# pavel-paulau/query

Measured on AMD Instinct MI355X. Metric: rows/sec filter+group-by on 100M synthetic JSON docs; achieved HBM GB/s, higher is better.
Workload: dtype int64/f64 tagged scalars (u8 tag + 8 B payload), u32 dictionary codes; 1 GPU; config2: SELECT cat, SUM(price) FROM default WHERE price > 50 GROUP BY cat @ 100000000 rows, K_cat=1000, columns resident in HBM; rows_per_gpu=100000000, groups=1000, rows_selected=49401294, agg_mode=2, spec_kernel=1

## Files before the change

### query_amd/build.py

```python
from __future__ import annotations

import os
import shutil
import subprocess
import sys

HERE = os.path.dirname(os.path.abspath(__file__))
CSRC = os.path.join(HERE, "csrc")
LIB = os.path.join(HERE, "libn1k.so")
SOURCES = ["n1k_kernels.hip", "n1k_bins.hip", "n1k_jsondev.hip", "n1k_matchtable.hip", "n1k_order.hip", "n1k_rowdistinct.hip", "n1k_order.cpp", "n1k_rowdistinct.cpp", "n1k_matchtable.cpp", "n1k_like.cpp", "n1k_coll.cpp", "n1k_in.cpp", "n1k_strfn.cpp", "n1k_jsonpush.cpp", "n1k_plan.cpp", "n1k_engine.cpp", "n1k_scan.cpp", "n1k_select.cpp", "n1k_partitioned.cpp", "n1k_distinct.cpp",
           "n1k_finish.cpp", "n1k_tail.cpp", "n1k_exchange.cpp", "n1k_jit.cpp", "n1k_json.cpp"]
HEADERS = ["n1k_types.h", "n1k_device.h", "n1k_tables.h", "n1k_scatter.h", "n1k_spec.h", "n1k_like.h", "n1k_coll.h", "n1k_in.h", "n1k_strfn.h", "n1k_order.h", "n1k_rowdistinct.h", "n1k_jit.h", "n1k_kernels.h", "n1k_plan.h", os.path.join("..", "..", "include", "n1k.h")]
HOST_HEADERS = ["n1k_engine.h", "n1k_buf.h", "n1k_wire.h"]
ARCH = "gfx950"


def _hipcc() -> str:
    for c in (os.environ.get("HIPCC"), shutil.which("hipcc"), "/opt/rocm/bin/hipcc"):
        if c and os.path.exists(c):
            return c
    raise RuntimeError("hipcc not found")


OBJDIR = os.path.join(CSRC, "build")
FLAGS = ["--offload-arch=" + ARCH, "-O3", "-std=c++17", "-fPIC", "-munsafe-fp-atomics", "-Wall", "-Wno-unused-function"]


def _stale(target: str, deps) -> bool:
    if not os.path.exists(target):
        return True
    mt = os.path.getmtime(target)
    return any(os.path.getmtime(d) > mt for d in deps)


def source_hash() -> str:
    import hashlib
    h = hashlib.sha1()
    for f in sorted([x for x in SOURCES if x.endswith(".hip")] + [x for x in HEADERS if not x.startswith("..")]):
        with open(os.path.join(CSRC, f), "rb") as fh:
            h.update(f.encode() + b"\0" + fh.read())
    return h.hexdigest()[:16]


def needs_build() -> bool:
    return _stale(LIB, [os.path.join(CSRC, f) for f in SOURCES + HEADERS + HOST_HEADERS] + [os.path.abspath(__file__)])


def build(force: bool = False, verbose: bool = False) -> str:
    if not force and not needs_build():
        return LIB
    from concurrent.futures import ThreadPoolExecutor
    os.makedirs(OBJDIR, exist_ok=True)
    hipcc = _hipcc()
    headers = [os.path.join(CSRC, f) for f in HEADERS + HOST_HEADERS] + [os.path.abspath(__file__)]

    def compile_one(src: str) -> str:
        obj = os.path.join(OBJDIR, src + ".o")
        path = os.path.join(CSRC, src)
        deps = headers if not src.endswith(".hip") else [os.path.join(CSRC, f) for f in HEADERS]
        if force or _stale(obj, [path] + deps):
            cmd = [hipcc] + FLAGS + ["-c", path, "-o", obj]
            if verbose:
                print(" ".join(cmd), file=sys.stderr)
            subprocess.check_call(cmd)
        return obj

    with ThreadPoolExecutor(max_workers=min(len(SOURCES), os.cpu_count() or 1)) as ex:
        objs = list(ex.map(compile_one, SOURCES))
    cmd = [hipcc, "--offload-arch=" + ARCH, "-shared", "-fPIC", "-o", LIB] + objs + ["-lhiprtc", "-lrccl", "-ldl", "-pthread"]
    if verbose:
        print(" ".join(cmd), file=sys.stderr)
    subprocess.check_call(cmd)
    return LIB


if __name__ == "__main__":
    print(build(force="--force" in sys.argv, verbose=True))
```

### query_amd/csrc/n1k_engine.cpp

```cpp
#include "n1k_engine.h"

using namespace n1k;
using namespace n1k_eng;

namespace n1k_eng {

thread_local std::string g_create_error;

n1k_status fail(n1k_handle* h, n1k_status st, const char* fmt, ...) {
    char buf[512];
    va_list ap;
    va_start(ap, fmt);
    vsnprintf(buf, sizeof buf, fmt, ap);
    va_end(ap);
    h->last_error = buf;
    return st;
}

uint32_t intern(n1k_handle* h, const std::string& s) {
    auto it = h->dict_index.find(s);
    if (it != h->dict_index.end()) return it->second;
    uint32_t code = (uint32_t)h->dict.size();
    h->dict.push_back(s);
    h->dict_index.emplace(s, code);
// ... 373 lines not shown
        tbits = (63 - n_dict * dbits) / n_tag;
    }
    uint32_t shift = 0;
    for (uint32_t k = 0; k < P.nkeys; k++) {
        KeySpec& ks = P.keys[k];
        ks.bits = ks.mode == KEYM_DICT ? dbits : tbits;
        ks.shift = shift;
        shift += ks.bits;
        if (ks.bits < (ks.mode == KEYM_DICT ? 4u : 8u)) return fail(h, N1K_UNSUPPORTED, "group key layout does not fit 63 bits");
    }
    P.wide_int = P.wide_flt = nullptr;
    P.wide_bits = 0;
    P.wide_count = h->groups.counters.p + CTR_WIDE_VALUES;
    if (n_tag && h->opt.wide_values) {
        uint32_t wb = 4;
        while ((1ull << wb) < h->opt.wide_values * 2 && wb < 30) wb++;
        wb = std::min(wb, tbits - 4);
        const size_t n = (size_t)1 << wb;
        HIP_TRY(h, h->groups.wide_int.ensure(n));
        HIP_TRY(h, h->groups.wide_flt.ensure(n));
        HIP_TRY(h, hipMemsetAsync(h->groups.wide_int.p, 0xFF, n * 8, h->stream));
        HIP_TRY(h, hipMemsetAsync(h->groups.wide_flt.p, 0xFF, n * 8, h->stream));
        P.wide_int = h->groups.wide_int.p;
        P.wide_flt = h->groups.wide_flt.p;
        P.wide_bits = wb;
    }
    {
        uint32_t total = 0;
        for (uint32_t k = 0; k < P.nkeys; k++) total += P.keys[k].bits;
        h->distinct.nw_key_bits = P.nkeys == 0 ? 1u : (total <= 34 ? total : 24u);
        h->distinct.nw_val_bits = 61 - h->distinct.nw_key_bits;
        for (uint32_t a = 0; a < P.naggs; a++)
            if (P.aggs[a].distinct)
                h->distinct.words[P.aggs[a].log_index] = h->opt.distinct_words && P.aggs[a].kind == AGG_COUNT;
    }
    h->layout_fixed = true;
    return N1K_OK;
}

n1k_status alloc_table(n1k_handle* h, uint64_t capacity, GlobalTable& t, DevBuf<uint64_t>& keys, DevBuf<uint64_t>& acc,
                       DevBuf<uint64_t>& rep) {
    HIP_TRY(h, keys.ensure(capacity));
    HIP_TRY(h, acc.ensure(capacity * h->prog.glob_words));
    if (h->prog.want_rep_row) HIP_TRY(h, rep.ensure(capacity));
    t.keys = keys.p;
    t.acc = acc.p;
    t.rep_row = h->prog.want_rep_row ? rep.p : nullptr;
    t.capacity = capacity;
    HIP_TRY(h, launch_init_table(h->prog, t, 0, capacity, nullptr, h->stream));
    return N1K_OK;
}

static n1k_status grow_table(n1k_handle* h, uint64_t cap) {
    if (cap <= h->groups.table.capacity) return N1K_OK;
    if (!h->groups.table.capacity) return alloc_table(h, cap, h->groups.table, h->groups.keys, h->groups.acc, h->groups.rep);
    GlobalTable nt{};
    DevBuf<uint64_t> nk, na, nr;
    ST_TRY(alloc_table(h, cap, nt, nk, na, nr));
    HIP_TRY(h, launch_rehash(h->prog, h->groups.table, nt, h->groups.errp, h->groups.counters.p + CTR_REHASH_SCRATCH, h->stream));
    HIP_TRY(h, hipStreamSynchronize(h->stream));
    h->groups.keys = std::move(nk);
    h->groups.acc = std::move(na);
    h->groups.rep = std::move(nr);
    h->groups.table = nt;
    return N1K_OK;
}

n1k_status ensure_table(n1k_handle* h, uint64_t incoming_rows) {
    uint64_t want_groups = std::min<uint64_t>(h->opt.max_groups, h->row_base + h->groups.merged_bound + incoming_rows);
    if (h->prog.nkeys == 0) want_groups = 1;
    else {
        bool all_dict = true;
        long double dom = 1;
        for (uint32_t k = 0; k < h->prog.nkeys; k++) {
            all_dict &= h->prog.keys[k].mode == KEYM_DICT;
            dom *= (long double)h->dict.size() + 2;
        }
        if (all_dict && dom < (long double)want_groups) want_groups = (uint64_t)dom;
    }
    return grow_table(h, next_pow2(std::max<uint64_t>(want_groups * 2, 1024)));
}

n1k_status ensure_table_groups(n1k_handle* h, uint64_t groups) {
    if (groups > h->opt.max_groups)
        return fail(h, N1K_OOM, "group table capacity exceeded: raise the max_groups option (now %llu)", (unsigned long long)h->opt.max_groups);
    return grow_table(h, next_pow2(std::max<uint64_t>(groups * 2, 1024)));
}

n1k_status ensure_pinned_counters(n1k_handle* h) {
    HIP_TRY(h, h->res.pin_counters.ensure(kCounters + kPinScratch));
    return N1K_OK;
}

hipEvent_t get_event(n1k_handle* h) {
    if (!h->timing.event_pool.empty()) {
        hipEvent_t e = h->timing.event_pool.back();
        h->timing.event_pool.pop_back();
        return e;
    }
    hipEvent_t e = nullptr;
    (void)hipEventCreate(&e);
    return e;
}

void drain_events(n1k_handle* h) {
    for (auto& pr : h->timing.events) {
        float ms = 0.f;
        if (pr.first && pr.second && hipEventElapsedTime(&ms, pr.first, pr.second) == hipSuccess) h->timing.stats.device_ms += ms;
        if (pr.first) h->timing.event_pool.push_back(pr.first);
        if (pr.second) h->timing.event_pool.push_back(pr.second);
    }
    h->timing.events.clear();
}

n1k_status validate_batch(n1k_handle* h, const n1k_batch* b) {
    if (!b) return fail(h, N1K_INVALID, "null batch");
    if (b->ncols != (uint32_t)h->plan.paths.size()) return fail(h, N1K_INVALID, "batch has %u columns, plan needs %u", b->ncols, (uint32_t)h->plan.paths.size());
    for (uint32_t c = 0; c < b->ncols; c++) {
        const n1k_col& col = b->cols[c];
        if (col.kind == N1K_COL_DICT32) {
            if (b->nrows && !col.codes) return fail(h, N1K_INVALID, "column %u: null codes", c);
        } else if (col.kind == N1K_COL_TAGGED64) {
            if (b->nrows && (!col.tags || !col.payload)) return fail(h, N1K_INVALID, "column %u: null tags/payload", c);
        } else
            return fail(h, N1K_INVALID, "column %u: unknown kind %u", c, col.kind);
        if (h->layout_fixed && col.kind != h->col_kinds[c])
            return fail(h, N1K_INVALID, "column %u changed kind between batches", c);
    }
    return N1K_OK;
}

uint64_t batch_bytes_per_row(const n1k_handle* h) {
    uint64_t b = 0;
    for (uint32_t c = 0; c < (uint32_t)h->plan.paths.size(); c++) b += h->col_kinds[c] == N1K_COL_DICT32 ? 4 : 9;
    return b;
}

void default_value(const AggDef& d, n1k_value& v, n1k_partial& p) {
    memset(&v, 0, sizeof v);
    memset(&p, 0, sizeof p);
    p.extreme.tag = N1K_T_NULL;
    if (d.kind == AGG_COUNT || d.kind == AGG_COUNTN) {
        v.tag = N1K_T_INT;
        v.v.i = 0;
    } else
        v.tag = N1K_T_NULL;
}

n1k_status reset_handle(n1k_handle* h, bool clear_stop) {
    if (clear_stop) h->stop_flag.store(0);
    h->failure_global = false;
    h->row_base = 0;
    h->groups.merged_bound = 0;
    h->filter.selected.clear();
    h->filter.has_sel32 = false;
    h->res.keys.clear();
    h->res.aggs.clear();
    h->res.parts.clear();
    h->res.rep.clear();
    memset(&h->timing.stats, 0, sizeof h->timing.stats);
    if (h->device_ready) {
        HIP_TRY(h, hipSetDevice(h->device));
        if (!h->timing.events.empty()) {
            HIP_TRY(h, hipStreamSynchronize(h->stream));
            drain_events(h);
        }
        h->timing.stats.device_ms = 0;
        h->part.groups_seen = 0;
        h->res.out_count_dirty = false;
        h->part.pending.count = 0;
        if (!h->timing.ev_q0) {
            (void)hipEventCreate(&h->timing.ev_q0);
            (void)hipEventCreate(&h->timing.ev_q1);
        }
        h->timing.q1_recorded = false;
        h->timing.q0_recorded = h->timing.ev_q0 && hipEventRecord(h->timing.ev_q0, h->stream) == hipSuccess;
        if (h->device_clean) return N1K_OK;
        h->device_clean = true;
        if (h->groups.table.capacity) HIP_TRY(h, launch_init_table(h->prog, h->groups.table, 0, h->groups.table.capacity, h->groups.counters.p, h->stream));
        else HIP_TRY(h, hipMemsetAsync(h->groups.counters.p, 0, kCounters * sizeof(unsigned long long), h->stream));
        if (h->distinct.word_hist.p) HIP_TRY(h, hipMemsetAsync(h->distinct.word_hist.p, 0, kMaxDistinct * 256 * sizeof(unsigned long long), h->stream));
        if (h->distinct.wcursor.p) HIP_TRY(h, hipMemsetAsync(h->distinct.wcursor.p, 0, kMaxDistinct * kWordSubs * kCursorStride * sizeof(unsigned long long), h->stream));
        h->distinct.wregion_used = false;
        if (h->prog.wide_int) {
            const size_t n = (size_t)1 << h->prog.wide_bits;
            HIP_TRY(h, hipMemsetAsync(h->groups.wide_int.p, 0xFF, n * 8, h->stream));
            HIP_TRY(h, hipMemsetAsync(h->groups.wide_flt.p, 0xFF, n * 8, h->stream));
        }
    }
    return N1K_OK;
}

}



extern "C" {

int n1k_abi_version(void) { return N1K_ABI_VERSION; }

int n1k_device_count(void) {
    int n = 0;
    if (hipGetDeviceCount(&n) != hipSuccess) return 0;
    return n;
}

const char* n1k_create_error(void) { return g_create_error.c_str(); }

uint64_t n1k_device_bytes_live(void) { return g_device_bytes_live.load(std::memory_order_relaxed); }

n1k_status n1k_create(const char* plan_json, size_t len, n1k_handle** out) {
    return guarded(nullptr, [&]() -> n1k_status {
    if (out) *out = nullptr;
    if (!plan_json || !out) {
        g_create_error = "null argument";
        return N1K_INVALID;
    }
    auto* h = new n1k_handle();
    PlanError err;
    if (!parse_plan_json(plan_json, len, h->plan, err) || !compile_plan(h, err)) {
        g_create_error = err.msg;
        n1k_status st = err.unsupported ? N1K_UNSUPPORTED : N1K_INVALID;
        delete h;
        return st;
    }
    if (h->plan.has_having) {
        std::string cond = h->plan.having_text;
        std::vector<std::pair<std::string, std::string>> subst;
        for (size_t a = 0; a < h->plan.aggs.size(); a++) subst.emplace_back(h->plan.aggs[a].text, "(`$g`.`a" + std::to_string(a) + "`)");
        for (size_t k = 0; k < h->plan.key_texts.size(); k++) subst.emplace_back(h->plan.key_texts[k], "(`$g`.`k" + std::to_string(k) + "`)");
        std::stable_sort(subst.begin(), subst.end(), [](const auto& x, const auto& y) { return x.first.size() > y.first.size(); });
        for (auto& sb : subst) {
            if (sb.first.empty()) continue;
            for (size_t pos = 0; (pos = cond.find(sb.first, pos)) != std::string::npos; pos += sb.second.size())
                cond.replace(pos, sb.first.size(), sb.second);
        }
        std::string js = "{\"#operator\":\"Filter\",\"condition\":\"";
        for (char c : cond) {
            if (c == '"' || c == '\\') js.push_back('\\');
            if ((unsigned char)c < 0x20) {
                char b[8];
                snprintf(b, sizeof b, "\\u%04x", (unsigned)c);
                js += b;
            } else
                js.push_back(c);
        }
        js += "\"}";
        n1k_status hst = n1k_create(js.c_str(), js.size(), &h->tail.having);
        if (hst != N1K_OK) {
            g_create_error = "HAVING: " + g_create_error;
            delete h;
            return hst;
        }
        for (const std::string& p : h->tail.having->plan.paths) {
            int idx = -1;
            char kind = 0;
            if (sscanf(p.c_str(), "(`$g`.`%c%d`)", &kind, &idx) != 2 || (kind != 'k' && kind != 'a') || idx < 0 ||
                (size_t)idx >= (kind == 'k' ? h->plan.key_texts.size() : h->plan.aggs.size())) {
                g_create_error = "HAVING refers to " + p + ", which is neither a group key nor an aggregate of the plan";
                n1k_destroy(h->tail.having);
                delete h;
                return N1K_UNSUPPORTED;
            }
            h->tail.having_cols.push_back(kind == 'k' ? idx : -idx - 1);
        }
    }
    if (h->plan.has_project) {
        n1k_status pst = build_projection(h);
        if (pst != N1K_OK) {
            if (h->tail.having) n1k_destroy(h->tail.having);
            h->tail.having = nullptr;
            delete h;
            return pst;
        }
    }
    g_create_error.clear();
    *out = h;
    return N1K_OK;
    });
}

static void destroy_handle(n1k_handle* h);
void n1k_destroy(n1k_handle* h) {
    if (!h) return;
    try {
        destroy_handle(h);
    } catch (...) {
    }
}
static void destroy_handle(n1k_handle* h) {
    if (h->timing.host_us[5] > 0)
        fprintf(stderr, "n1k host trace: %.0f one-call executions; per call: reset %.1f us, push %.1f us, finish %.1f us (of which waiting %.1f us, after the wait %.1f us)\n",
                h->timing.host_us[5], h->timing.host_us[0] / h->timing.host_us[5], h->timing.host_us[1] / h->timing.host_us[5], h->timing.host_us[2] / h->timing.host_us[5],
                h->timing.host_us[3] / h->timing.host_us[5], h->timing.host_us[4] / h->timing.host_us[5]);
    if (h->tail.having) n1k_destroy(h->tail.having);
    h->tail.having = nullptr;
    if (h->tail.project) n1k_destroy(h->tail.project);
    h->tail.project = nullptr;
    if (h->device_ready) {
        (void)hipSetDevice(h->device);
        if (h->stream) (void)hipStreamSynchronize(h->stream);
        if (h->stage.copy_stream) (void)hipStreamSynchronize(h->stage.copy_stream);
        drain_events(h);
        for (auto e : h->timing.event_pool) (void)hipEventDestroy(e);
        if (h->timing.ev_q0) (void)hipEventDestroy(h->timing.ev_q0);
        if (h->timing.ev_q1) (void)hipEventDestroy(h->timing.ev_q1);
// ... 36 lines not shown
}
const char* n1k_projection_alias(const n1k_handle* h, uint32_t i) {
    if (h && i < h->plan.row_distinct.size()) return h->plan.row_distinct[i].as.c_str();
    return (h && i < h->plan.project.size()) ? h->plan.project[i].as.c_str() : nullptr;
}

n1k_status n1k_dict_intern(n1k_handle* h, uint32_t n, const uint64_t* offsets, const char* bytes, uint32_t* out_codes) {
    return guarded(h, [&]() -> n1k_status {
    if (!h || (n && (!offsets || !bytes || !out_codes))) return N1K_INVALID;
    for (uint32_t i = 0; i < n; i++) {
        if (offsets[i + 1] < offsets[i]) return fail(h, N1K_INVALID, "dictionary offsets are not monotone");
        out_codes[i] = intern(h, std::string(bytes + offsets[i], (size_t)(offsets[i + 1] - offsets[i])));
    }
    if (h->dict.size() >= 0xFFFFFFF0ull) return fail(h, N1K_OOM, "dictionary too large");
    return N1K_OK;
    });
}

uint32_t n1k_dict_size(const n1k_handle* h) { return h ? (uint32_t)h->dict.size() : 0; }

n1k_status n1k_dict_get(const n1k_handle* h, uint32_t code, const char** ptr, size_t* len) {
    return guarded(h, [&]() -> n1k_status {
    if (!h || !ptr || !len || code >= h->dict.size()) return N1K_INVALID;
    *ptr = h->dict[code].data();
    *len = h->dict[code].size();
    return N1K_OK;
    });
}

n1k_status n1k_set_option(n1k_handle* h, const char* name, int64_t value) {
    return guarded(h, [&]() -> n1k_status {
    if (!h || !name) return N1K_INVALID;
    std::string n = name;
    if (n == "agg_mode") h->opt.agg_mode = value;
    else if (n == "max_groups") h->opt.max_groups = value > 0 ? (uint64_t)value : 1;
    else if (n == "grid_blocks") h->opt.grid_blocks = (uint32_t)std::max<int64_t>(0, value);
    else if (n == "fast") h->opt.fast = value ? 1 : 0;
    else if (n == "spec") h->opt.spec = value ? 1 : 0;
    else if (n == "wide") h->opt.wide = value ? 1 : 0;
    else if (n == "fuse_arith") h->opt.fuse_arith = value ? 1 : 0;
    else if (n == "lean_topk") h->opt.lean_topk = value ? 1 : 0;
    else if (n == "topk_sample") h->opt.topk_sample = value ? 1 : 0;
    else if (n == "distinct_fill_pct") h->opt.distinct_fill_pct = (uint32_t)std::min<int64_t>(std::max<int64_t>(value, 1), 75);
    else if (n == "dedupe_unroll") h->opt.dedupe_unroll = (uint32_t)value;
    else if (n == "agg_spec") h->opt.agg_spec = value ? 1 : 0;
    else if (n == "merge_chunks") h->opt.merge_chunks = (uint32_t)std::min<int64_t>(std::max<int64_t>(value, 0), 16);
    else if (n == "inject_failure") h->opt.inject_failure = (uint32_t)std::min<int64_t>(std::max<int64_t>(value, 0), 3);
    else if (n == "part_block") h->opt.part_block = value == 256 ? 256 : 512;
    else if (n == "part_subs") h->opt.part_subs = (uint32_t)std::min<int64_t>(std::max<int64_t>(value, 0), 2);
    else if (n == "part_per_cu") h->opt.part_per_cu = (uint32_t)std::min<int64_t>(std::max<int64_t>(value, 0), 8);
    else if (n == "jit") h->opt.jit = (uint32_t)std::min<int64_t>(std::max<int64_t>(value, 0), 2);
    else if (n == "jit_min_rows") h->opt.jit_min_rows = (uint64_t)std::max<int64_t>(value, 0);
    else if (n == "distinct_words") {
        if (h->layout_fixed) return fail(h, N1K_INVALID, "distinct_words must be set before the first batch");
        h->opt.distinct_words = value ? 1 : 0;
    } else if (n == "distinct_set_slots") {
        uint32_t v = 64;
        while (v < (uint32_t)std::min<int64_t>(std::max<int64_t>(value, 64), 8192)) v <<= 1;
        h->opt.distinct_set_slots = v;
    } else if (n == "records") {
        h->opt.records = value ? 1 : 0;
    } else if (n == "rec_slots") {
        h->opt.rec_slots = (uint32_t)std::min<int64_t>(std::max<int64_t>(value, 0), 8192);
    } else if (n == "rec_bins") {
        uint32_t v = 0;
        if (value > 0) for (v = 1; v < (uint32_t)std::min<int64_t>(value, 256); v <<= 1) {}
        h->opt.rec_bins = v;
    } else if (n == "rec_slices") {
        h->opt.rec_slices = (uint32_t)std::min<int64_t>(std::max<int64_t>(value, 0), 64);
    } else if (n == "rec_scan_per_cu") {
        h->opt.rec_scan_per_cu = (uint32_t)std::min<int64_t>(std::max<int64_t>(value, 0), 8);
    } else if (n == "rec_block") {
        h->opt.rec_block = value <= 0 ? 0u : (value <= 256 ? 256u : 512u);
    } else if (n == "rec_unroll") {
        h->opt.rec_unroll = (uint32_t)std::min<int64_t>(std::max<int64_t>(value, 0), 8);
    } else if (n == "distinct_region_cap") {
        h->opt.region_cap = (uint64_t)std::max<int64_t>(value, 0);
    } else if (n == "dedupe_block") {
        if ((value | 1) != 257 && (value | 1) != 513 && (value | 1) != 1025) return fail(h, N1K_INVALID, "dedupe_block must be 256, 512 or 1024 (+1: probe word by word)");
        h->opt.dedupe_block = (uint32_t)value;
    } else if (n == "json_device") {
        h->opt.json_device = value ? 1 : 0;
    } else if (n == "json_device_left_pct") {
        h->opt.json_device_left_pct = (uint32_t)std::min<int64_t>(std::max<int64_t>(value, 0), 100);
    } else if (n == "json_device_min_docs") {
        h->opt.json_device_min_docs = (uint64_t)std::max<int64_t>(value, 0);
    } else if (n == "json_threads") {
        h->opt.json_threads = (uint32_t)std::min<int64_t>(std::max<int64_t>(value, 0), 64);
    } else if (n == "partition_min_rows") {
        h->opt.partition_min_rows = (uint64_t)std::max<int64_t>(value, 1);
    } else if (n == "partition_probe_rows") {
        h->opt.partition_probe_rows = (uint64_t)std::max<int64_t>(value, 1);
    } else if (n == "partition_min_groups") {
        h->opt.partition_min_groups = (uint64_t)std::max<int64_t>(value, 1);
    } else if (n == "partition_sticky") {
        h->opt.partition_sticky = value ? 1 : 0;
        h->part.sticky.valid = false;
    } else if (n == "partition_levels") {
        h->opt.partition_levels = (int32_t)std::min<int64_t>(std::max<int64_t>(value, -1), 2);
    } else if (n == "topk_min_groups") {
        h->opt.topk_min_groups = (uint64_t)std::max<int64_t>(value, 1);
    } else if (n == "distinct_levels") {
        h->opt.distinct_levels = (int32_t)std::min<int64_t>(std::max<int64_t>(value, -1), 2);
    } else if (n == "wide_values") {
        if (h->layout_fixed) return fail(h, N1K_INVALID, "wide_values must be set before the first batch");
        h->opt.wide_values = (uint64_t)std::max<int64_t>(value, 0);
    }
    else if (n == "slabs") h->opt.slabs = (uint32_t)std::min<int64_t>(std::max<int64_t>(value, 0), 2);
    else if (n == "block") {
        if (value != 0 && value != 256 && value != 512 && value != 1024) return fail(h, N1K_INVALID, "block must be 0 (auto), 256, 512 or 1024");
        h->opt.block = (uint32_t)value;
    } else if (n == "rows_per_lane") {
        if (value != 2 && value != 4) return fail(h, N1K_INVALID, "rows_per_lane must be 2 or 4");
        h->opt.rows_per_lane = (uint32_t)value;
    }
    else if (n == "lds_bytes") h->opt.lds_bytes = (uint32_t)std::min<int64_t>(std::max<int64_t>(value, 1024), 64 * 1024);
    else if (n == "device") {
        if (h->device_ready) return fail(h, N1K_INVALID, "device must be chosen before the first push");
        h->device = (int)value;
    } else if (n == "stream") {
        if (h->device_ready) return fail(h, N1K_INVALID, "stream must be chosen before the first push");
        h->stream = (hipStream_t)(uintptr_t)value;
        h->own_stream = false;
    } else if (n == "rep_row") {
        if (h->layout_fixed) return fail(h, N1K_INVALID, "rep_row must be chosen before the first push");
        h->opt.rep_row = value ? 1 : 0;
        PlanError err;
        h->agg_names.clear();
        h->has_distinct = false;
        h->n_distinct = 0;
        if (!compile_plan(h, err)) return fail(h, N1K_INVALID, "%s", err.msg.c_str());
    } else if (!rowdistinct_option(h, n, value))
        return fail(h, N1K_INVALID, "unknown option %s", name);
    return N1K_OK;
    });
}

n1k_status n1k_push_device_batch(n1k_handle* h, const n1k_batch* batch) {
    return guarded(h, [&]() -> n1k_status {
    if (!h) return N1K_INVALID;
    ST_TRY(refuse_ordered_rows(h, "n1k_push_device_batch"));
    return push_device(h, batch);
    });
}

n1k_status n1k_run_device_batch(n1k_handle* h, const n1k_batch* batch, n1k_result* out) {
    if (!h || !batch || !out) return N1K_INVALID;
    if (h->plan.ordered_rows() || h->plan.has_row_distinct) return guarded(h, [&]() -> n1k_status { return refuse_ordered_rows(h, "n1k_run_device_batch"); });
    static const bool trace = getenv("N1K_HOST_TRACE") != nullptr;
    auto now = [] { return std::chrono::duration<double, std::micro>(std::chrono::steady_clock::now().time_since_epoch()).count(); };
    const double t0 = trace ? now() : 0;
    n1k_status st = n1k_reset(h);
    const double t1 = trace ? now() : 0;
    if (st == N1K_OK) st = n1k_push_device_batch(h, batch);
    const double t2 = trace ? now() : 0;
    if (st == N1K_OK) {
        h->clear_on_finish = true;
        st = n1k_finish(h, out);
        h->clear_on_finish = false;
    }
    if (trace) {
        h->timing.host_us[0] += t1 - t0;
        h->timing.host_us[1] += t2 - t1;
        h->timing.host_us[2] += now() - t2;
        h->timing.host_us[5] += 1;
    }
    return st;
}

n1k_status n1k_extract_json(n1k_handle* h, uint64_t ndocs, const uint64_t* offsets, const char* bytes, n1k_batch* out) {
    return guarded(h, [&]() -> n1k_status {
    if (!h || !out || (ndocs && (!offsets || !bytes))) return N1K_INVALID;
    if (h->json.paths_state == 0) {
        h->json.paths.resize(h->plan.paths.size());
        h->json.paths_state = 1;
        for (size_t c = 0; c < h->plan.paths.size(); c++)
            if (!parse_leaf_path(h->plan.paths[c], h->json.paths[c])) h->json.paths_state = -1;
    }
    if (h->json.paths_state < 0)
        return fail(h, N1K_UNSUPPORTED, "a leaf path of the plan is not a chain of field names: extract the columns yourself");
    const size_t np = h->json.paths.size();
    uint32_t nthreads = h->opt.json_threads ? h->opt.json_threads : std::min(16u, std::max(1u, std::thread::hardware_concurrency()));
    nthreads = (uint32_t)std::max<uint64_t>(1, std::min<uint64_t>(nthreads, ndocs / 2048 + 1));
    std::vector<JsonColumns> part(nthreads);
    std::vector<std::string> errs(nthreads);
    std::vector<long long> bad(nthreads, -1);
    std::vector<std::thread> workers;
    auto range = [&](uint32_t t) { return std::make_pair(ndocs * t / nthreads, ndocs * (t + 1) / nthreads); };
    std::vector<char> threw(nthreads, 0);
    auto work = [&](uint32_t t) {
        try {
            auto r = range(t);
            bad[t] = extract_json_range(h->json.paths, offsets, bytes, r.first, r.second, part[t], errs[t]);
        } catch (...) {
            threw[t] = 1;
        }
    };
    workers.reserve(nthreads);
    std::vector<uint32_t> inline_ranges{0};
    for (uint32_t t = 1; t < nthreads; t++) {
        try {
            workers.emplace_back(work, t);
        } catch (...) {
            inline_ranges.push_back(t);
        }
    }
    for (uint32_t t : inline_ranges) work(t);
    for (auto& w : workers) w.join();
    for (uint32_t t = 0; t < nthreads; t++)
        if (threw[t]) return fail(h, N1K_OOM, "out of host memory while scanning the documents");
    for (uint32_t t = 0; t < nthreads; t++)
        if (bad[t] >= 0) {
            if (errs[t].find("nested deeper than 256") != std::string::npos)
                return fail(h, N1K_UNSUPPORTED_DATA, "document %lld: %s", bad[t], errs[t].c_str());
            return fail(h, N1K_INVALID, "document %lld is not valid JSON: %s", bad[t], errs[t].c_str());
        }
    h->json.tags.assign(np, std::vector<uint8_t>());
    h->json.payload.assign(np, std::vector<uint64_t>());
    for (size_t c = 0; c < np; c++) {
        h->json.tags[c].resize(ndocs);
        h->json.payload[c].resize(ndocs);
    }
    for (uint32_t t = 0; t < nthreads; t++) {
        auto r = range(t);
        std::vector<uint64_t> code(part[t].strings.size());
        for (size_t i = 0; i < code.size(); i++) code[i] = intern(h, part[t].strings[i]);
        for (size_t c = 0; c < np; c++) {
            const size_t n = (size_t)(r.second - r.first);
            memcpy(h->json.tags[c].data() + r.first, part[t].tags[c].data(), n);
            uint64_t* dst = h->json.payload[c].data() + r.first;
            const uint64_t* src = part[t].payload[c].data();
            const uint8_t* tg = part[t].tags[c].data();
            for (size_t i = 0; i < n; i++) dst[i] = tg[i] >= N1K_T_STRING ? code[src[i]] : src[i];
        }
    }
    h->json.cols.assign(np, n1k_col{});
    for (size_t c = 0; c < np; c++) {
        h->json.cols[c].kind = N1K_COL_TAGGED64;
        h->json.cols[c].tags = h->json.tags[c].data();
        h->json.cols[c].payload = h->json.payload[c].data();
    }
    out->nrows = ndocs;
    out->ncols = (uint32_t)np;
    out->cols = h->json.cols.data();
    return N1K_OK;
    });
}

n1k_status n1k_push_json(n1k_handle* h, uint64_t ndocs, const uint64_t* offsets, const char* bytes) {
    return guarded(h, [&]() -> n1k_status {
    if (!h || (ndocs && (!offsets || !bytes))) return N1K_INVALID;
    ST_TRY(refuse_ordered_rows(h, "n1k_push_json"));
    if (h->stop_flag.load()) return fail(h, N1K_STOPPED, "operator was stopped");
    if (h->json.paths_state == 0) {
        h->json.paths.resize(h->plan.paths.size());
        h->json.paths_state = 1;
        for (size_t c = 0; c < h->plan.paths.size(); c++)
            if (!parse_leaf_path(h->plan.paths[c], h->json.paths[c])) h->json.paths_state = -1;
    }
    if (h->json.paths_state > 0 && ndocs) {
        bool done = false;
        n1k_status dst = push_json_device(h, ndocs, offsets, bytes, &done);
        if (dst != N1K_OK || done) return dst;
    }
    n1k_batch b{};
    n1k_status st = n1k_extract_json(h, ndocs, offsets, bytes, &b);
    if (st != N1K_OK) return st;
    return n1k_push_batch(h, &b);
    });
}

n1k_status n1k_push_batch(n1k_handle* h, const n1k_batch* batch) {
    return guarded(h, [&]() -> n1k_status {
    if (!h) return N1K_INVALID;
    ST_TRY(refuse_ordered_rows(h, "n1k_push_batch"));
    if (h->stop_flag.load()) return fail(h, N1K_STOPPED, "operator was stopped");
    n1k_status st = ensure_device(h);
    if (st != N1K_OK) return st;
    st = validate_batch(h, batch);
    if (st != N1K_OK) return st;
    std::vector<n1k_col> dcols;
    st = stage_host_batch(h, batch, dcols);
    if (st != N1K_OK) return st;
    n1k_batch db = *batch;
    db.cols = dcols.data();
    st = push_device(h, &db);
    n1k_status st2 = staged_batch_issued(h);
    return st != N1K_OK ? st : st2;
    });
}

n1k_status n1k_sync(n1k_handle* h) {
    return guarded(h, [&]() -> n1k_status {
    if (!h) return N1K_INVALID;
    if (!h->device_ready) return N1K_OK;
    HIP_TRY(h, hipSetDevice(h->device));
    unsigned long long counters[kCounters] = {0};
    HIP_TRY(h, hipMemcpyAsync(counters, h->groups.counters.p, sizeof counters, hipMemcpyDeviceToHost, h->stream));
    HIP_TRY(h, hipStreamSynchronize(h->stream));
    drain_events(h);
    if (h->plan.has_group && !h->device_clean) {
        h->timing.stats.rows_selected = counters[CTR_ROWS_SELECTED];
        h->timing.stats.groups_out = h->part.pending.count ? h->part.pending.count : counters[CTR_GROUPS];
    }
    if (!h->device_clean) h->timing.stats.wide_key_values = counters[CTR_WIDE_VALUES];
    return N1K_OK;
    });
}

n1k_status n1k_jit_check(n1k_handle* h, const uint32_t* col_kinds, uint32_t ncols, char* log, size_t loglen) {
    return guarded(h, [&]() -> n1k_status {
    if (!h || !col_kinds) return N1K_INVALID;
    if (log && loglen) log[0] = 0;
// ... 192 lines not shown
```

### query_amd/csrc/n1k_engine.h

```cpp
#pragma once
#include <hip/hip_runtime.h>

#include <algorithm>
#include <atomic>
#include <chrono>
#include <cmath>
#include <cstdarg>
#include <cstdio>
#include <cstring>
#include <functional>
#include <numeric>
#include <string>
#include <condition_variable>
#include <mutex>
#include <thread>
#include <unordered_map>
#include <vector>

#include "../../include/n1k.h"
#include "n1k_buf.h"
#include "n1k_jit.h"
#include "n1k_json.h"
#include "n1k_kernels.h"
#include "n1k_coll.h"
#include "n1k_in.h"
#include "n1k_like.h"
#include "n1k_order.h"
#include "n1k_plan.h"
#include "n1k_rowdistinct.h"
#include "n1k_strfn.h"


using namespace n1k;

static_assert(sizeof(n1k_value) == 16, "n1k_value layout");
static_assert(sizeof(OutValue) == sizeof(n1k_value), "OutValue must alias n1k_value");
static_assert(sizeof(Program) + sizeof(ScanArgs) + sizeof(GlobalTable) + 64 <= 4096, "kernel arguments exceed 4 KiB");

namespace n1k_eng {

extern thread_local std::string g_create_error;

struct MatchScratch {
    DevBuf<uint8_t> bytes;
    DevBuf<uint64_t> off;
    DevBuf<uint8_t> left;
    DevBuf<uint8_t> bits;
    DevBuf<uint8_t> progs;
    DevBuf<uint8_t> sprogs;
};

enum MatchKind { MK_LIKE, MK_COLL, MK_IN, MK_STRFN, MK_COUNT };

struct MatchTable {
    std::vector<LikePattern> patterns;
    std::vector<CollPred> preds;
    std::vector<InList> lists;
    uint32_t string_lists = 0;
    std::vector<StrFnPred> strfns;
    uint32_t strfn_first = 0;
    uint32_t coll_top = kMatchBits - 1;
    std::vector<double> in_numbers;
    InTableHost in_table;
    DevBuf<uint8_t> d_in_table;
    DevBuf<double> d_in_nums;
    bool in_uploaded = false;
    DevBuf<uint8_t> d_bits;
    size_t built_for = 0;
    MatchScratch scratch;
    struct { uint64_t dev = 0, host = 0; } counts[MK_COUNT];

    int add_like(const std::string& pattern, PlanError& err);
    int add_coll(const Expr* e, PlanError& err);
    int add_in(const Expr* e, PlanError& err);
    int add_strfn(const Expr* e, const Expr*& path, PlanError& err);
    void finalize_bits(Program& P);
    void clear_plan() {
        patterns.clear();
        preds.clear();
        lists.clear();
        strfns.clear();
        in_numbers.clear();
        string_lists = strfn_first = 0;
    }
};

inline uint32_t match_lds_bytes(const FastArgs& F) {
    for (uint32_t t = 0; t < F.nterms; t++)
        if (term_is_table_bit(F.terms[t].op)) return kMatchLdsBytes;
    return 0;
}

inline uint64_t next_pow2(uint64_t x) {
    uint64_t p = 1;
    while (p < x) p <<= 1;
    return p;
}
inline uint32_t ceil_log2(uint64_t x) {
    uint32_t b = 0;
    while ((1ull << b) < x) b++;
    return b;
}

n1k_status fail(n1k_handle* h, n1k_status st, const char* fmt, ...);

#define HIP_TRY(h, expr)                                                                                  \
    do {                                                                                                  \
        hipError_t _e = (expr);                                                                           \
        if (_e != hipSuccess)                                                                             \
            return fail(h, _e == hipErrorOutOfMemory ? N1K_OOM : N1K_DEVICE_ERROR, "%s failed: %s", #expr, \
                        hipGetErrorString(_e));                                                           \
    } while (0)

#define ST_TRY(expr) do { n1k_status _st = (expr); if (_st != N1K_OK) return _st; } while (0)

constexpr uint32_t kPinScratch = 16;
constexpr uint64_t kWordSubs = 256ull * kRecSubs;


struct Options {
    int64_t agg_mode = N1K_MODE_AUTO;
    uint64_t max_groups = 1ull << 26;
    uint32_t grid_blocks = 0;
    uint32_t fast = 1, spec = 1, wide = 1;
    uint32_t fuse_arith = 1;
    uint32_t lean_topk = 1;
    uint32_t topk_sample = 1;
    uint32_t distinct_fill_pct = 25;
    uint32_t dedupe_unroll = 0;
    uint32_t agg_spec = 1;
    uint32_t merge_chunks = 0;
    uint32_t inject_failure = 0;
    uint32_t part_block = 256;
    uint32_t part_subs = 1;
    uint32_t part_per_cu = 0;
    uint32_t jit = 1;
    uint64_t jit_min_rows = 4u << 20;
    uint32_t distinct_words = 1;
    uint32_t distinct_set_slots = 8192;
    uint32_t records = 1;
    uint32_t rec_slots = 0, rec_bins = 0, rec_slices = 0, rec_scan_per_cu = 0, rec_block = 0, rec_unroll = 0;
    uint64_t region_cap = 0;
    uint32_t dedupe_block = 1025;
    uint32_t json_device = 1;
    uint32_t json_device_left_pct = 12;
    uint64_t json_device_min_docs = 4096;
    uint32_t json_threads = 0;
    uint64_t partition_min_rows = 8u << 20, partition_probe_rows = 512u << 10, partition_min_groups = 4096;
    uint32_t partition_sticky = 1;
    int32_t partition_levels = -1;
    uint64_t topk_min_groups = 65536;
    int32_t distinct_levels = -1;
    uint64_t wide_values = 1u << 20;
    uint32_t slabs = 1;
    uint32_t block = 0, rows_per_lane = 4;
    uint32_t lds_bytes = 64 * 1024;
    uint32_t rep_row = 0;
    uint64_t rowdistinct_slots = 0;
    uint32_t rowdistinct_lds_slots = 0;
};

enum Counter : uint32_t {
    CTR_ROWS_SELECTED = 0,
    CTR_GROUPS = 1,
    CTR_OUT_COUNT = 2,
    CTR_FILTER_TOTAL = 3,
    CTR_REHASH_SCRATCH = 4,
    CTR_DISTINCT_REGION_WORDS = 5,
    CTR_PAIR_LOG_CURSORS = 8,
    CTR_ERR_FLAGS = 12,
    CTR_WIDE_VALUES = 13,
    CTR_WORD_LOG_CURSORS = 16,
    CTR_OPTIMISTIC_OVERFLOW = 20,
    CTR_PART_RECORDS = 21,
    CTR_SINGLETONS = 22,
    CTR_EXACT_OVERFLOW = 24,
    CTR_SAVED_ROWS_SELECTED = 25,
    CTR_REGION_GROUPS = 26,
    CTR_PEER_STATUS = 27,
    CTR_ROWDISTINCT_COUNT = 28,
    CTR_ROWDISTINCT_REACHED = 29
};
static_assert(CTR_ERR_FLAGS + kPeerStatusFromErr == CTR_PEER_STATUS, "the verdict kernel writes the peer status this far behind the flags");
static_assert(CTR_ROWDISTINCT_REACHED < kCounters && CTR_ROWDISTINCT_REACHED == CTR_ROWDISTINCT_COUNT + 1, "every counter word lies inside the buffer (CTR_ROWDISTINCT_REACHED is the last)");
static_assert(CTR_PAIR_LOG_CURSORS + kMaxDistinct <= CTR_ERR_FLAGS && CTR_WORD_LOG_CURSORS + kMaxDistinct <= CTR_OPTIMISTIC_OVERFLOW, "cursor words overlap their neighbours");

struct GroupTable {
    GlobalTable table{};
    DevBuf<uint64_t> keys, acc, rep;
    DevBuf<uint64_t> slabs;
    DevBuf<unsigned long long> block_sel;
    uint32_t* errp = nullptr;
    DevBuf<unsigned long long> counters;
    DevBuf<uint64_t> wide_int, wide_flt;
    uint64_t merged_bound = 0;
};
uint32_t intern(n1k_handle* h, const std::string& s);
uint32_t lookup_code(const n1k_handle* h, const char* s);
bool to_operand(n1k_handle* h, const Expr* e, Operand& o, PlanError& err);
bool compile_plan(n1k_handle* h, PlanError& err);
n1k_status ensure_device(n1k_handle* h);
n1k_status reset_handle(n1k_handle* h, bool clear_stop);
n1k_status ensure_rank(n1k_handle* h);
n1k_status fix_layout(n1k_handle* h, const n1k_batch* b);
n1k_status ensure_table(n1k_handle* h, uint64_t incoming_rows);
n1k_status ensure_table_groups(n1k_handle* h, uint64_t groups);
hipEvent_t get_event(n1k_handle* h);
n1k_status ensure_pinned_counters(n1k_handle* h);
void drain_events(n1k_handle* h);
n1k_status validate_batch(n1k_handle* h, const n1k_batch* b);
uint64_t batch_bytes_per_row(const n1k_handle* h);
void default_value(const AggDef& d, n1k_value& v, n1k_partial& p);

struct Timing {
    double host_us[6] = {0, 0, 0, 0, 0, 0};
    hipEvent_t ev_q0 = nullptr, ev_q1 = nullptr;
    bool q0_recorded = false, q1_recorded = false;
    n1k_stats stats{};
    std::vector<std::pair<hipEvent_t, hipEvent_t>> events;
    std::vector<hipEvent_t> event_pool;
};

struct Json {
    std::vector<JsonPath> paths;
    int paths_state = 0;
    std::vector<std::vector<uint8_t>> tags;
    std::vector<std::vector<uint64_t>> payload;
    std::vector<n1k_col> cols;
    DevBuf<char> d_bytes;
    DevBuf<uint64_t> d_offsets, d_new_first, d_patch_docs, d_patch_pay, d_tab;
    DevBuf<uint8_t> d_status, d_patch_tags;
    DevBuf<uint32_t> d_new_list, d_code_of, d_codes;
    std::vector<DevBuf<uint8_t>> d_tags;
    std::vector<DevBuf<uint64_t>> d_payload;
    std::vector<uint8_t> host_status;
};
n1k_status push_json_device(n1k_handle* h, uint64_t ndocs, const uint64_t* offsets, const char* bytes, bool* done);

n1k_status ensure_match_table(n1k_handle* h);

struct Staging {
    std::vector<DevBuf<uint8_t>> tags[2];
    std::vector<DevBuf<uint64_t>> payload[2];
    std::vector<DevBuf<uint32_t>> codes[2];
    hipStream_t copy_stream = nullptr;
    hipEvent_t free_ev[2] = {nullptr, nullptr};
    bool busy[2] = {false, false};
    hipEvent_t copied = nullptr;
    int cur = 0;
};
struct FilterOnly {
    DevBuf<uint64_t> tile_off, sel;
    std::vector<uint64_t> selected;
    DevBuf<uint32_t> sel32;
    bool has_sel32 = false;
    uint64_t sel32_count = 0, sel32_rows = 0;
    const uint32_t* sel32_out = nullptr;
};

struct RowOrder {
    DevBuf<uint64_t> key[kOrdHists];
    DevBuf<uint16_t> res[kOrdMaxTerms];
    DevBuf<uint64_t> kbuf[2];
    DevBuf<uint32_t> vbuf[2];
    DevBuf<uint32_t> hist, tile_hist;
    DevBuf<uint32_t> cand;
    DevBuf<char> state;
    DevBuf<uint32_t> rows_out;
    PinBuf<uint32_t> pin_hist;
    uint32_t passes = 0;
};
n1k_status order_selection(n1k_handle* h, const uint32_t* sel, uint64_t total, const uint32_t** out_rows, uint64_t* out_count);
n1k_status refuse_ordered_rows(n1k_handle* h, const char* call);

struct RowDistinct {
    DevBuf<uint32_t> table;
    DevBuf<uint32_t> slot_of;
    DevBuf<uint32_t> tile_count;
    DevBuf<uint32_t> rows_out;
    uint64_t stats[4] = {0, 0, 0, 0};
};
n1k_status distinct_selection(n1k_handle* h, const uint32_t* sel, uint64_t total, const uint32_t** out_rows, uint64_t* out_count);
bool rowdistinct_option(n1k_handle* h, const std::string& name, int64_t value);
bool filter_stream_fast(const n1k_handle* h);
uint32_t filter_stream_grid(const n1k_handle* h, uint64_t ntiles, bool fast);
bool build_fast_args(n1k_handle* h, uint32_t max_slots, FastArgs& F, bool fuse = false, bool partition_only = false);
template <class Col> inline void advance_cols(Col* cols, uint32_t n, uint64_t off) {
    for (uint32_t c = 0; c < n; c++) {
        if (cols[c].tags) cols[c].tags += off;
        if (cols[c].payload) cols[c].payload += off;
        if (cols[c].codes) cols[c].codes += off;
    }
}
template <class Col> inline bool cols_wide_aligned(const Col* cols, uint32_t n) {
    for (uint32_t c = 0; c < n; c++)
        if ((uintptr_t)cols[c].tags % 2 || (uintptr_t)cols[c].payload % 16 || (uintptr_t)cols[c].codes % 8) return false;
    return true;
}
enum class ShapeUse { Scan, Records, Partition };
struct ShapeKernel {
    const SpecEntry* spec = nullptr;
    const JitKernel* jit = nullptr;
    uint32_t stat = 0;
    explicit operator bool() const { return spec || jit; }
};
ShapeKernel shape_kernel(n1k_handle* h, const FastArgs& F, ShapeUse use, uint64_t nrows, size_t table_bytes = 0);
bool shape_compiles(const n1k_handle* h, const FastArgs& F, ShapeUse use, std::string* log);
n1k_status run_group_batch(n1k_handle* h, const n1k_batch* b);
n1k_status run_filter_batch(n1k_handle* h, const n1k_batch* b);
n1k_status bind_columns(n1k_handle* h, const n1k_batch* b, bool defer = false);
n1k_status materialize_derived(n1k_handle* h, const n1k_batch* b);
n1k_status push_device(n1k_handle* h, const n1k_batch* b);
n1k_status stage_host_batch(n1k_handle* h, const n1k_batch* batch, std::vector<n1k_col>& dcols);
n1k_status staged_batch_issued(n1k_handle* h);

struct Partitioned {
    DevBuf<uint64_t> rec_key[3], rec_pay[3][kRecOperands];
    DevBuf<uint8_t> rec_tag[3][kRecOperands];
    DevBuf<uint64_t> emit;
    DevBuf<uint64_t> rregion, rbins;
    DevBuf<unsigned long long> rcursor;
    struct { uint64_t count = 0, cap = 0; } pending;
    struct { bool valid = false; uint64_t rows = 0, groups_est = 0; } sticky;
    uint64_t groups_seen = 0;
};
struct PartitionPlan {
    Operand src[kRecOperands];
    uint32_t nsrc = 0;
    uint32_t agg_src[kMaxAggs];
};
bool partition_eligible(n1k_handle* h, PartitionPlan& pp);
bool small_key_domain(const n1k_handle* h);
n1k_status flush_pending(n1k_handle* h);
n1k_status run_group_partitioned(n1k_handle* h, const n1k_batch* b, const PartitionPlan& pp, uint64_t groups_est, bool may_keep_region);
n1k_status run_group_records(n1k_handle* h, const n1k_batch* b, const PartitionPlan& pp, uint64_t groups_est, bool may_keep_region, bool* done);

struct Distinct {
    DevBuf<uint64_t> log_key[kMaxDistinct], log_val[kMaxDistinct], regions, set_table;
    DevBuf<uint8_t> log_cls[kMaxDistinct];
    DevBuf<uint64_t> log_word[kMaxDistinct], part[2], seg[3], wtable;
    DevBuf<unsigned long long> hist, cursor, dcounts, word_hist;
    DevBuf<uint64_t> wregion[kMaxDistinct], woff, wgather;
    DevBuf<unsigned long long> wcursor;
    uint64_t wregion_cap = 0;
    bool wregion_used = false;
    uint32_t nw_key_bits = 0, nw_val_bits = 0;
    bool words[kMaxDistinct] = {false, false, false, false};
    uint32_t path = 0;
    uint64_t log_capacity = 0;
};
n1k_status distinct_grow_logs(n1k_handle* h, uint64_t nrows, ScanArgs& A);
n1k_status distinct_grow_regions(n1k_handle* h, const Program& P, uint64_t nrows, const ScanArgs& A, uint32_t dcache_slots, WordLogArgs& L);
n1k_status distinct_words_finish(n1k_handle* h, const AggSpec& ag, uint64_t nwords, bool hist_counted = true, const uint64_t* log = nullptr);
n1k_status distinct_regions_finish(n1k_handle* h, const AggSpec& ag, uint64_t nover, bool force_exact, bool* deferred);

struct TopK {
    DevBuf<uint64_t> images;
    DevBuf<uint32_t> cand;
    DevBuf<char> state, out2;
};
struct Results {
    std::vector<n1k_value> keys, aggs;
    std::vector<n1k_partial> parts;
    std::vector<uint64_t> rep;
    DevBuf<char> d_out;
    std::vector<char> out_host;
    std::vector<char> export_blob;
    bool out_count_dirty = true;
    PinBuf<char> pin_out;
    PinBuf<unsigned long long> pin_counters;
    PinBuf<char> pin_rows;
};

struct Tail {
    n1k_handle* project = nullptr;
    std::vector<int> project_cols;
    std::vector<Operand> project_ops;
    std::vector<n1k_value> r_proj;
    n1k_handle* having = nullptr;
    std::vector<int> having_cols;
    std::vector<uint32_t> having_codes;
};
n1k_status build_projection(n1k_handle* h);
n1k_status having_groups(n1k_handle* h, uint64_t& ng);
n1k_status project_groups(n1k_handle* h, uint64_t ng);
n1k_status order_groups(n1k_handle* h, uint64_t& ng);
n1k_status array_agg_groups(n1k_handle* h, uint64_t ng, const unsigned long long* counters);
void publish_result(n1k_handle* h, uint64_t ng, bool partials, n1k_result* out);

}

using namespace n1k_eng;

struct n1k_handle {
    ParsedPlan plan;
    std::string last_error;
    std::atomic<int> stop_flag{0};
    Options opt;
    bool failure_global = false;
    bool device_clean = false, clear_on_finish = false;
    std::string jit_log;
    int device = -1;
    bool device_ready = false;
    hipStream_t stream = nullptr;
    bool own_stream = false;
    int num_cus = 256;

    std::vector<std::string> dict;
    std::unordered_map<std::string, uint32_t> dict_index;
    bool need_rank = false;
    size_t rank_built_for = (size_t)-1;
    DevBuf<uint32_t> d_rank;

    MatchTable match;

    Program prog{};
    bool layout_fixed = false;
    uint32_t col_kinds[kMaxCols]{};
    std::vector<std::string> agg_names;
    bool has_distinct = false, has_minmax = false, has_array_agg = false;
    uint32_t n_distinct = 0;
    struct Derived { uint32_t op, nops; Operand ops[4]; };
    std::vector<Derived> derived;
    std::vector<std::string> const_strings;
    std::vector<DevBuf<uint8_t>> dv_tags;
    std::vector<DevBuf<uint64_t>> dv_payload;
    bool derived_ready = true;

    uint64_t row_base = 0;
    const unsigned long long* push_nrows_dev = nullptr;
    const unsigned long long* push_seg_counts = nullptr;
    uint32_t push_nseg = 0;
    uint64_t push_seg_rows = 0;

    GroupTable groups;
    Distinct distinct;
    Partitioned part;
    TopK topk;
    Tail tail;
    Json json;
    Staging stage;
    FilterOnly filter;
    RowDistinct rowdistinct;
    RowOrder order;
    Results res;
    Timing timing;
};

namespace n1k_eng {

template <class F>
n1k_status guarded(const n1k_handle* ch, F&& f) noexcept {
    n1k_handle* h = const_cast<n1k_handle*>(ch);
    try {
        return f();
    } catch (const std::bad_alloc&) {
        try { if (h) h->last_error = "out of host memory"; else g_create_error = "out of host memory"; } catch (...) {}
        return N1K_OOM;
    } catch (const std::exception& e) {
        try { if (h) h->last_error = std::string("internal error: ") + e.what(); else g_create_error = e.what(); } catch (...) {}
        return N1K_DEVICE_ERROR;
    } catch (...) {
        return N1K_DEVICE_ERROR;
    }
}

}
```

### query_amd/csrc/n1k_finish.cpp

```cpp
#include "n1k_engine.h"

using namespace n1k;
using namespace n1k_eng;

static void mark_query_end(n1k_handle* h) {
    if (h->timing.q0_recorded && h->timing.ev_q1 && hipEventRecord(h->timing.ev_q1, h->stream) == hipSuccess) h->timing.q1_recorded = true;
}

struct OutLayout {
    size_t aggs, parts, rep, total;
    OutLayout(uint64_t groups = 0, size_t nk = 0, size_t na = 0)
        : aggs(groups * nk * sizeof(OutValue)), parts(aggs + groups * na * sizeof(OutValue)), rep(parts + groups * na * sizeof(OutPartial)), total(rep + groups * 8) {}
    OutValue* k(char* b) const { return (OutValue*)b; }
    OutValue* a(char* b) const { return (OutValue*)(b + aggs); }
    OutPartial* p(char* b) const { return (OutPartial*)(b + parts); }
    uint64_t* r(char* b) const { return (uint64_t*)(b + rep); }
};

struct Finish {
    unsigned long long counters[kCounters] = {0};
    uint32_t err_flags = 0;
    uint64_t ng = 0;
    uint64_t spec_groups = 0;
    char* d_rows = nullptr;
    char* rows = nullptr;
    OutLayout lay;
    bool sets_exact = false;
    bool sets_deferred = false, vetoed = false;
    std::chrono::steady_clock::time_point wait_end{};
};

enum : uint32_t { PIN_NCAND = kCounters, PIN_ERR_FLAGS, PIN_VETO };

static uint64_t speculative_groups(const n1k_handle* h) {
    const ParsedPlan& pl = h->plan;
    const bool topk_forced = pl.has_order && pl.limit >= 0 && !pl.has_having && h->opt.topk_min_groups < 4096;
    if (!pl.has_group || h->has_distinct || !h->groups.table.capacity || h->groups.table.capacity > (1u << 20) || topk_forced || h->part.pending.count)
        return 0;
    return std::min<uint64_t>(h->groups.table.capacity, 4096);
}

static n1k_status zero_out_count(n1k_handle* h) {
    if (h->res.out_count_dirty) HIP_TRY(h, hipMemsetAsync(h->groups.counters.p + CTR_OUT_COUNT, 0, sizeof(unsigned long long), h->stream));
    h->res.out_count_dirty = true;
    return N1K_OK;
}

static n1k_status read_counters(n1k_handle* h, Finish& F) {
    if (!h->device_ready) return h->timing.stats.rows_in == 0 ? ensure_device(h) : N1K_OK;
    HIP_TRY(h, hipSetDevice(h->device));
    ST_TRY(ensure_pinned_counters(h));
    F.spec_groups = speculative_groups(h);
    if (F.spec_groups) {
        F.lay = OutLayout(F.spec_groups, h->plan.keys.size(), h->plan.aggs.size());
        HIP_TRY(h, h->res.pin_out.ensure(F.lay.total + kCounters * sizeof(unsigned long long)));
        char* d = F.rows = h->res.pin_out.p;
        unsigned long long* host_counters = (unsigned long long*)(d + F.lay.total);
        if (h->groups.table.capacity <= 8192) {
            const bool clear = h->clear_on_finish && !h->prog.wide_int;
            HIP_TRY(h, launch_finalize_small(h->prog, h->groups.table, F.lay.k(d), F.lay.a(d), F.lay.p(d), F.lay.r(d), h->groups.counters.p,
                                             host_counters, F.spec_groups, h->groups.errp, clear, h->stream));
            h->res.out_count_dirty = !clear;
            h->device_clean = clear;
        } else {
            ST_TRY(zero_out_count(h));
            HIP_TRY(h, launch_finalize(h->prog, h->groups.table, F.lay.k(d), F.lay.a(d), F.lay.p(d), F.lay.r(d),
                                       h->groups.counters.p + CTR_OUT_COUNT, F.spec_groups, h->groups.errp, h->stream));
            HIP_TRY(h, launch_publish_counters(h->groups.counters.p, host_counters, kCounters, h->stream));
        }
        mark_query_end(h);
        const auto w0 = std::chrono::steady_clock::now();
        HIP_TRY(h, hipStreamSynchronize(h->stream));
        F.wait_end = std::chrono::steady_clock::now();
        h->timing.host_us[3] += std::chrono::duration<double, std::micro>(F.wait_end - w0).count();
        memcpy(F.counters, host_counters, sizeof F.counters);
    } else {
        HIP_TRY(h, hipMemcpyAsync(h->res.pin_counters.p, h->groups.counters.p, sizeof F.counters, hipMemcpyDeviceToHost, h->stream));
        mark_query_end(h);
        HIP_TRY(h, hipStreamSynchronize(h->stream));
        memcpy(F.counters, h->res.pin_counters.p, sizeof F.counters);
    }
    F.err_flags = (uint32_t)F.counters[CTR_ERR_FLAGS];
    drain_events(h);
    return N1K_OK;
}

static n1k_status build_distinct_sets(n1k_handle* h, Finish& F) {
    h->distinct.path = 0;
    if (h->distinct.wregion_used) HIP_TRY(h, hipMemsetAsync(h->groups.counters.p + CTR_OPTIMISTIC_OVERFLOW, 0, 8, h->stream));
    for (size_t a = 0; a < h->plan.aggs.size(); a++) {
        const AggSpec& ag = h->prog.aggs[a];
        if (!ag.distinct || ag.kind == AGG_ARRAY) continue;
        const uint64_t npairs = std::min<uint64_t>(F.counters[CTR_PAIR_LOG_CURSORS + ag.log_index], h->distinct.log_capacity);
        const uint64_t nwords = h->distinct.words[ag.log_index] ? std::min<uint64_t>(F.counters[CTR_WORD_LOG_CURSORS + ag.log_index], h->distinct.log_capacity) : 0;
        DistinctArgs D{};
        D.log_key = h->distinct.log_key[ag.log_index].p;
        D.log_val = h->distinct.log_val[ag.log_index].p;
        D.log_cls = h->distinct.log_cls[ag.log_index].p;
        D.npairs = npairs;
        D.glob_off = ag.glob_off;
        D.kind = ag.kind;
        D.total_words = h->groups.counters.p + CTR_DISTINCT_REGION_WORDS;
        HIP_TRY(h, h->distinct.regions.ensure(h->groups.table.capacity * 6));
        D.regions = h->distinct.regions.p;
        HIP_TRY(h, hipMemsetAsync(D.total_words, 0, sizeof(unsigned long long), h->stream));
        HIP_TRY(h, launch_distinct_layout(h->prog, h->groups.table, D, h->stream));
        if (npairs) {
            unsigned long long words = 0;
            HIP_TRY(h, hipMemcpyAsync(&words, D.total_words, sizeof words, hipMemcpyDeviceToHost, h->stream));
            HIP_TRY(h, hipStreamSynchronize(h->stream));
            HIP_TRY(h, h->distinct.set_table.ensure(std::max<uint64_t>(words, 1)));
            D.set_table = h->distinct.set_table.p;
            if (words) HIP_TRY(h, hipMemsetAsync(h->distinct.set_table.p, 0xFF, words * 8, h->stream));
            HIP_TRY(h, launch_distinct_insert(h->prog, h->groups.table, D, h->groups.errp, h->stream));
            h->distinct.path |= 1u;
        }
        if (h->distinct.wregion_used && h->distinct.words[ag.log_index]) ST_TRY(distinct_regions_finish(h, ag, nwords, F.sets_exact, &F.sets_deferred));
        else if (nwords) ST_TRY(distinct_words_finish(h, ag, nwords));
    }
    h->timing.stats.distinct_path = h->distinct.path;
    return N1K_OK;
}

struct TopKPlan { bool on = false, lean = false; uint64_t keep = 0; };

static TopKPlan plan_topk(const n1k_handle* h, uint64_t ng) {
    const ParsedPlan& pl = h->plan;
    TopKPlan t;
    t.keep = pl.limit >= 0 ? (uint64_t)pl.offset + (uint64_t)pl.limit : ng;
    t.on = pl.has_order && pl.limit >= 0 && !pl.has_having && pl.order[0].proj_index < 0 && t.keep > 0 && t.keep < ng &&
           ng >= h->opt.topk_min_groups && ng < (1ull << 32);
    t.lean = t.on && h->part.pending.count && h->opt.lean_topk;
    return t;
}

static n1k_status sized_final_group(n1k_handle* h, Finish& F, bool lean) {
    F.lay = OutLayout(F.ng, h->plan.keys.size(), h->plan.aggs.size());
    HIP_TRY(h, h->res.d_out.ensure((lean ? F.ng * sizeof(OutValue) : F.lay.total) + 16));
    char* d = F.d_rows = h->res.d_out.p;
    ST_TRY(zero_out_count(h));
    if (lean) {
        const OrderTerm& t0 = h->plan.order[0];
        HIP_TRY(h, h->topk.images.ensure(F.ng));
        ST_TRY(ensure_rank(h));
        HIP_TRY(h, launch_finalize_region(h->prog, h->part.emit.p, h->part.pending.cap, F.ng, nullptr, nullptr, nullptr, nullptr, h->groups.errp,
                                          h->stream, nullptr, nullptr, t0.key_index >= 0,
                                          (uint32_t)(t0.key_index >= 0 ? t0.key_index : t0.agg_index), h->topk.images.p, t0.desc));
    } else if (h->part.pending.count)
        HIP_TRY(h, launch_finalize_region(h->prog, h->part.emit.p, h->part.pending.cap, F.ng, F.lay.k(d), F.lay.a(d), F.lay.p(d), F.lay.r(d),
                                          h->groups.errp, h->stream));
    else
        HIP_TRY(h, launch_finalize(h->prog, h->groups.table, F.lay.k(d), F.lay.a(d), F.lay.p(d), F.lay.r(d), h->groups.counters.p + CTR_OUT_COUNT,
                                   F.ng, h->groups.errp, h->stream));
    return N1K_OK;
}

static n1k_status select_topk(n1k_handle* h, Finish& F, const TopKPlan& tk) {
    const OrderTerm& t0 = h->plan.order[0];
    const uint32_t nk = (uint32_t)h->plan.keys.size(), na = (uint32_t)h->plan.aggs.size();
    HIP_TRY(h, h->topk.images.ensure(F.ng));
    HIP_TRY(h, h->topk.cand.ensure(topk_cand_entries(F.ng)));
    HIP_TRY(h, h->topk.state.ensure(topk_state_bytes()));
    ST_TRY(ensure_rank(h));
    char* d = F.d_rows;
    const OutLayout all = F.lay;
    const bool by_key = t0.key_index >= 0;
    const OutValue* vals = tk.lean || by_key ? all.k(d) : all.a(d);
    const uint32_t stride = tk.lean ? 1u : (by_key ? nk : na), index = tk.lean ? 0u : (uint32_t)(by_key ? t0.key_index : t0.agg_index);
    const bool sampled = h->opt.topk_sample && topk_can_sample(F.ng, tk.keep);
    unsigned long long ncand = 0;
    for (int attempt = sampled ? 0 : 1; attempt < 2; attempt++) {
        HIP_TRY(h, launch_topk_select(h->prog, vals, stride, index, F.ng, t0.desc, tk.keep, h->topk.images.p, h->topk.state.p, h->topk.cand.p,
                                      h->stream, attempt == 0, tk.lean || (attempt == 1 && sampled)));
        HIP_TRY(h, hipMemcpyAsync(h->res.pin_counters.p + PIN_NCAND, h->topk.state.p + topk_ncand_offset(), sizeof ncand, hipMemcpyDeviceToHost, h->stream));
        HIP_TRY(h, hipStreamSynchronize(h->stream));
        ncand = h->res.pin_counters.p[PIN_NCAND];
        if (ncand >= tk.keep) break;
    }
    F.lay = OutLayout(ncand, nk, na);
    HIP_TRY(h, h->topk.out2.ensure(F.lay.total + 16));
    char* c = F.d_rows = h->topk.out2.p;
    if (tk.lean)
        HIP_TRY(h, launch_finalize_region(h->prog, h->part.emit.p, h->part.pending.cap, ncand, F.lay.k(c), F.lay.a(c), F.lay.p(c), F.lay.r(c),
                                          h->groups.errp, h->stream, h->topk.cand.p));
    else
        HIP_TRY(h, launch_topk_compact(h->topk.cand.p, ncand, nk, na, all.k(d), all.a(d), all.p(d), all.r(d), F.lay.k(c), F.lay.a(c), F.lay.p(c),
                                       F.lay.r(c), h->stream));
    h->timing.stats.topk_candidates = ncand;
    F.ng = ncand;
    return N1K_OK;
}

static n1k_status land_rows(n1k_handle* h, Finish& F) {
    const size_t bytes = F.lay.total;
    const bool pinned_rows = bytes <= (8u << 20);
    if (pinned_rows && h->res.pin_rows.n < bytes) HIP_TRY(h, h->res.pin_rows.ensure(std::max<size_t>(bytes, 64u << 10)));
    if (!pinned_rows) h->res.out_host.resize(bytes);
    F.rows = pinned_rows ? h->res.pin_rows.p : h->res.out_host.data();
    unsigned long long* const pin = h->res.pin_counters.p;
    HIP_TRY(h, hipMemcpyAsync(F.rows, F.d_rows, bytes, hipMemcpyDeviceToHost, h->stream));
    HIP_TRY(h, hipMemcpyAsync(pin + PIN_ERR_FLAGS, h->groups.errp, 4, hipMemcpyDeviceToHost, h->stream));
    if (F.sets_deferred) HIP_TRY(h, hipMemcpyAsync(pin + PIN_VETO, h->groups.counters.p + CTR_OPTIMISTIC_OVERFLOW, 8, hipMemcpyDeviceToHost, h->stream));
    mark_query_end(h);
    HIP_TRY(h, hipStreamSynchronize(h->stream));
    memcpy(&F.err_flags, pin + PIN_ERR_FLAGS, 4);
    F.vetoed = F.sets_deferred && pin[PIN_VETO] != 0;
    return N1K_OK;
}

static void unpack_rows(n1k_handle* h, const Finish& F) {
    const size_t nk = h->plan.keys.size(), na = h->plan.aggs.size(), ng = F.ng;
    h->res.keys.assign((const n1k_value*)F.lay.k(F.rows), (const n1k_value*)F.lay.k(F.rows) + ng * nk);
    h->res.aggs.assign((const n1k_value*)F.lay.a(F.rows), (const n1k_value*)F.lay.a(F.rows) + ng * na);
    h->res.rep.assign(F.lay.r(F.rows), F.lay.r(F.rows) + ng);
    const OutPartial* parts = F.lay.p(F.rows);
    h->res.parts.resize(ng * na);
    for (size_t i = 0; i < ng * na; i++) {
        n1k_partial& p = h->res.parts[i];
        memset(&p, 0, sizeof p);
        p.count = parts[i].count;
        p.isum = parts[i].isum;
        p.fsum = parts[i].fsum;
        p.int_exact = parts[i].flags & 1u;
        p.has_float = (parts[i].flags >> 1) & 1u;
        p.extreme.tag = (uint8_t)parts[i].ext_tag;
        p.extreme.v.code = parts[i].ext_payload;
        p.distinct = parts[i].distinct;
    }
// ... 104 lines not shown
```

### query_amd/csrc/n1k_kernels.h

```cpp
#pragma once
#include <hip/hip_runtime.h>
#include <vector>
#include "n1k_types.h"

namespace n1k {

constexpr int kFilterStreamTile = 8192;

struct OutValue {
    uint64_t tag;
    uint64_t payload;
};

struct OutPartial {
    int64_t count;
    int64_t isum;
    double fsum;
    uint32_t flags;
    uint32_t ext_tag;
    uint64_t ext_payload;
    int64_t distinct;
};

struct SynthArgs {
    uint64_t seed, first_row, nrows, total_rows;
    uint32_t k_cat, pad;
    const double* cat_cdf;
    uint32_t* cat_codes;
    uint8_t* price_tags;
    uint64_t* price_payload;
    uint8_t* user_tags;
    uint64_t* user_payload;
    uint8_t* region_tags;
    uint64_t* region_payload;
};

hipError_t launch_init_table(const Program& P, const GlobalTable& G, uint64_t first, uint64_t count,
                             unsigned long long* counters, hipStream_t st);
hipError_t launch_restamp_ranks(const Program& P, const GlobalTable& G, hipStream_t st);
hipError_t launch_rehash(const Program& P, const GlobalTable& oldt, const GlobalTable& newt, uint32_t* err_flags,
                         unsigned long long* ngroups_scratch, hipStream_t st);
hipError_t launch_scan_group(const Program& P, const ScanArgs& A, const GlobalTable& G, unsigned long long* ngroups,
                             uint32_t grid, uint32_t block, uint32_t rows_per_lane, bool direct, hipStream_t st);
hipError_t launch_scan_fast(const Program& P, const FastArgs& F, const GlobalTable& G, unsigned long long* ngroups,
                            uint32_t grid, uint32_t block, uint32_t rows_per_lane, hipStream_t st);
hipError_t launch_merge_slabs(const Program& P, const FastArgs& F, const GlobalTable& G, uint32_t nblocks,
                              unsigned long long* ngroups, hipStream_t st, uint32_t ychunks_opt = 0);
hipError_t launch_finalize_region(const Program& P, const uint64_t* region, uint64_t cap, uint64_t count, OutValue* out_keys,
                                  OutValue* out_aggs, OutPartial* out_parts, uint64_t* out_rep, uint32_t* err_flags, hipStream_t st,
                                  const uint32_t* cand = nullptr, OutValue* ord = nullptr, bool ord_is_key = false, uint32_t ord_index = 0,
                                  uint64_t* images = nullptr, bool desc = false);
hipError_t launch_add_counter(unsigned long long* p, unsigned long long v, hipStream_t st);
hipError_t launch_probe_keys(const Program& P, uint64_t nrows, const GlobalTable& G, uint32_t* err_flags, unsigned long long* ngroups,
                             uint32_t grid, hipStream_t st);
hipError_t launch_project_records(const Program& P, const ProjectArgs& A, uint32_t grid, hipStream_t st);
hipError_t launch_agg_bins(const Program& P, const BinAggArgs& A, const GlobalTable& G, unsigned long long* ngroups, uint32_t grid,
                           hipStream_t st);
size_t topk_state_bytes();
size_t topk_ncand_offset();
hipError_t launch_topk_select(const Program& P, const OutValue* vals, uint32_t stride, uint32_t index, uint64_t n, bool desc,
                              uint64_t keep, uint64_t* images, void* state, uint32_t* cand, hipStream_t st, bool sampled = false, bool images_done = false);
hipError_t launch_topk_select_images(const uint64_t* images, uint64_t n, uint64_t keep, void* state, uint32_t* cand, hipStream_t st, bool sampled);
bool topk_can_sample(uint64_t n, uint64_t keep);
uint64_t topk_cand_entries(uint64_t n);
hipError_t launch_topk_compact(const uint32_t* cand, uint64_t ncand, uint32_t nk, uint32_t na, const OutValue* keys,
                               const OutValue* aggs, const OutPartial* parts, const uint64_t* rep, OutValue* okeys, OutValue* oaggs,
                               OutPartial* oparts, uint64_t* orep, hipStream_t st);
hipError_t launch_distinct_layout(const Program& P, const GlobalTable& G, const DistinctArgs& D, hipStream_t st);
hipError_t launch_radix_pass(const RadixArgs& A, uint32_t slices, hipStream_t st, bool have_hist = false);
hipError_t launch_distinct_dedupe(const Program& P, const GlobalTable& G, const DedupeArgs& D, uint32_t grid, uint32_t block, hipStream_t st);
size_t distinct_dedupe_lds(const DedupeArgs& D);
hipError_t launch_compact_regions(const uint64_t* region, uint32_t nreg, uint64_t cap, const unsigned long long* count, const uint64_t* off,
                                  uint64_t* dst, hipStream_t st);
hipError_t launch_regrow_regions(const uint64_t* src, uint32_t nreg, uint64_t src_cap, uint64_t* dst, uint64_t dst_cap,
                                 unsigned long long* count, hipStream_t st);
hipError_t launch_distinct_words_global(const GlobalTable& G, const uint64_t* words, uint64_t n, uint64_t* table, uint64_t mask,
                                        uint32_t key_shift, unsigned long long* counts, uint32_t* err_flags, uint32_t grid,
                                        hipStream_t st);
hipError_t launch_distinct_add_counts(const Program& P, const GlobalTable& G, const unsigned long long* counts, uint32_t glob_off,
                                      hipStream_t st, const uint32_t* veto = nullptr);
hipError_t launch_distinct_insert(const Program& P, const GlobalTable& G, const DistinctArgs& D, uint32_t* err_flags,
                                  hipStream_t st);
hipError_t launch_export_partials(const Program& P, const GlobalTable& G, uint32_t nparts, uint64_t cap, uint64_t* out,
                                  uint64_t region_words, uint32_t* err_flags, hipStream_t st);
hipError_t launch_merge_partials(const Program& P, const GlobalTable& G, uint32_t nregions, uint64_t cap, const uint64_t* in,
                                 uint64_t region_words, uint32_t* err_flags, unsigned long long* ngroups, hipStream_t st,
                                 uint64_t limit = 0, bool unique_keys = false);
hipError_t launch_arith(const ArithArgs& A, hipStream_t st);
hipError_t launch_publish_counters(const unsigned long long* src, unsigned long long* dst, uint32_t n, hipStream_t st);
hipError_t launch_partition(const Program& P, const PartArgs& A, uint32_t grid, hipStream_t st);
struct HeaderList { unsigned long long* h[kMaxParts]; };
hipError_t launch_exchange_verdict(const HeaderList& H, uint32_t nregions, uint32_t* err_flags, hipStream_t st);
hipError_t launch_stamp_verdict(unsigned long long* headers, uint32_t nregions, uint64_t stride_words, const uint32_t* err_flags,
                                uint32_t host_status, hipStream_t st);
hipError_t launch_dense_to_segments(unsigned long long* headers, uint32_t nregions, uint64_t stride_words, uint64_t sub_rows, hipStream_t st,
                                    const uint32_t* dest_cap = nullptr);
struct SpecEntry {
    const char* name;
    SpecSig sig;
    hipError_t (*launch)(const Program& P, const FastArgs& F, const GlobalTable& G, unsigned long long* ngroups,
                         uint32_t grid, uint32_t block, bool wide, const WordLogArgs& L, hipStream_t st);
    hipError_t (*launch_records)(const Program& P, const FastArgs& F, uint32_t grid, bool wide, const WordLogArgs& L, hipStream_t st);
};
size_t spec_records_lds_bytes();
hipError_t launch_radix_scatter16(const RadixArgs& A, uint32_t wpr, uint32_t bins_per_region, hipStream_t st);
hipError_t launch_radix_scatter_words(const RadixArgs& A, uint32_t wpr, uint32_t bins_per_region, hipStream_t st);
size_t agg_bins16_lds_bytes(const Program& P, uint32_t slots);
hipError_t launch_agg_bins16(const Program& P, const BinAggArgs& A, uint32_t grid, uint32_t block, uint32_t per_thread, hipStream_t st,
                             bool specialise = true);
const std::vector<SpecEntry>& spec_registry();
hipError_t launch_finalize(const Program& P, const GlobalTable& G, OutValue* out_keys, OutValue* out_aggs,
                           OutPartial* out_parts, uint64_t* out_rep, unsigned long long* out_count, uint64_t max_out,
                           uint32_t* err_flags, hipStream_t st);
hipError_t launch_finalize_small(const Program& P, const GlobalTable& G, OutValue* out_keys, OutValue* out_aggs, OutPartial* out_parts,
                                 uint64_t* out_rep, unsigned long long* counters, unsigned long long* host_counters, uint64_t max_out,
                                 uint32_t* err_flags, bool clear, hipStream_t st);
hipError_t launch_filter_stream(const Program& P, uint64_t nrows, uint64_t row_base, uint64_t* out_rows, unsigned long long* tile_state,
                                unsigned long long* tile_counter, unsigned long long* total, uint32_t* err_flags, uint32_t grid,
                                hipStream_t st, bool fast = false);
hipError_t launch_filter_stream(const Program& P, uint64_t nrows, uint32_t* out_rows, unsigned long long* tile_state,
                                unsigned long long* tile_counter, unsigned long long* total, uint32_t* err_flags, uint32_t grid,
                                hipStream_t st, bool fast);
constexpr uint32_t kGatherMaxCols = 16;
struct GatherCol {
    uint32_t kind, pad;
    const uint8_t* src_tags;
    const uint64_t* src_payload;
    const uint32_t* src_codes;
    uint8_t* dst_tags;
    uint64_t* dst_payload;
    uint32_t* dst_codes;
};
struct GatherArgs {
    const uint32_t* rows;
    uint64_t n;
    uint32_t ncols, pad;
    GatherCol cols[kGatherMaxCols];
};
hipError_t launch_gather_rows(const GatherArgs& A, hipStream_t st);
constexpr uint32_t kJsonMaxSteps = 4;
struct JsonDevPath {
    uint32_t nsteps;
    uint32_t name_off[kJsonMaxSteps], name_len[kJsonMaxSteps];
};
struct JsonDevArgs {
    const uint8_t* bytes;
    const uint64_t* offsets;
    uint64_t base, ndocs;
    uint32_t npaths, tab_bits;
    JsonDevPath paths[kMaxCols];
    char names[1024];
    uint8_t* out_tags[kMaxCols];
    uint64_t* out_payload[kMaxCols];
    uint8_t* status;
    unsigned long long* tab_hash;
    unsigned long long* tab_first;
    uint32_t* new_list;
    unsigned long long* new_count;
    uint32_t new_cap;
};
hipError_t launch_json_extract(const JsonDevArgs& A, uint32_t num_cus, hipStream_t st);
hipError_t launch_json_remap(const JsonDevArgs& A, const uint32_t* code_of, hipStream_t st);
hipError_t launch_json_gather_first(const JsonDevArgs& A, uint64_t n, unsigned long long* out, hipStream_t st);
hipError_t launch_json_scatter_codes(const uint32_t* new_list, const uint32_t* codes, uint64_t n, uint32_t* code_of, hipStream_t st);
hipError_t launch_json_patch(const JsonDevArgs& A, const uint64_t* docs, const uint8_t* tags, const uint64_t* payload, uint64_t n, hipStream_t st);
hipError_t launch_synth(const SynthArgs& a, hipStream_t st);

}
```

### query_amd/csrc/n1k_kernels.hip

```cpp
#include <hip/hip_runtime.h>
#include "n1k_device.h"
#include "n1k_tables.h"
#include "n1k_scatter.h"
#include "n1k_kernels.h"
#include <algorithm>
#include <vector>

namespace n1k {


template <int R>
N1K_DEV void load_operand(const Program& P, const Operand& o, const uint64_t (&row)[R], const bool (&valid)[R],
                          uint32_t (&tag)[R], uint64_t (&pay)[R]) {
    if (o.is_const) {
#pragma unroll
        for (int j = 0; j < R; j++) {
            tag[j] = o.ctag;
            pay[j] = o.cpayload;
        }
        return;
    }
    const DevCol& c = P.cols[o.col];
    if (c.kind == COLK_DICT32) {
        const uint32_t* codes = c.codes;
#pragma unroll
        for (int j = 0; j < R; j++) {
            uint32_t code = valid[j] ? codes[row[j]] : 0xFFFFFFFFu;
            tag[j] = code == 0xFFFFFFFFu ? T_MISSING : (code == 0xFFFFFFFEu ? T_NULL : T_STRING);
            pay[j] = code;
        }
    } else {
        const uint8_t* tags = c.tags;
        const uint64_t* payload = c.payload;
#pragma unroll
        for (int j = 0; j < R; j++) {
            tag[j] = valid[j] ? (uint32_t)tags[row[j]] : (uint32_t)T_MISSING;
            pay[j] = valid[j] ? payload[row[j]] : 0ull;
        }
    }
}

template <int R>
N1K_DEV void eval_term(const Program& P, const Term& t, const uint64_t (&row)[R], const bool (&valid)[R],
                       uint32_t (&out)[R], uint32_t& unsupported) {
    uint32_t ta[R];
    uint64_t pa[R];
    load_operand<R>(P, t.a, row, valid, ta, pa);
    switch (t.op) {
        case TERM_EQ:
        case TERM_LT:
        case TERM_LE: {
            uint32_t tb[R];
            uint64_t pb[R];
            load_operand<R>(P, t.b, row, valid, tb, pb);
#pragma unroll
            for (int j = 0; j < R; j++) {
                if (t.op == TERM_EQ) {
                    out[j] = equals_l(ta[j], pa[j], tb[j], pb[j], &unsupported);
                } else {
                    int c = compare(ta[j], pa[j], tb[j], pb[j], P.str_rank, &unsupported);
                    out[j] = c == CMP_MISSING ? L_MISSING
                                              : (c == CMP_NULL ? L_NULL : ((t.op == TERM_LT ? c < 0 : c <= 0) ? L_TRUE : L_FALSE));
                }
            }
            break;
        }
        case TERM_BETWEEN: {
            uint32_t tb[R], tc[R];
            uint64_t pb[R], pc[R];
            load_operand<R>(P, t.b, row, valid, tb, pb);
            load_operand<R>(P, t.c, row, valid, tc, pc);
#pragma unroll
            for (int j = 0; j < R; j++) {
                int lo = compare(ta[j], pa[j], tb[j], pb[j], P.str_rank, &unsupported);
                int hi = compare(ta[j], pa[j], tc[j], pc[j], P.str_rank, &unsupported);
                uint32_t r;
                if (lo == CMP_MISSING || hi == CMP_MISSING) r = L_MISSING;
                else if (lo == CMP_NULL || hi == CMP_NULL) r = L_NULL;
                else r = (lo >= 0 && hi <= 0) ? L_TRUE : L_FALSE;
                out[j] = r;
            }
            break;
        }
        case TERM_IS_NULL:
#pragma unroll
            for (int j = 0; j < R; j++) out[j] = ta[j] == T_NULL ? L_TRUE : (ta[j] == T_MISSING ? L_MISSING : L_FALSE);
            break;
        case TERM_IS_NOT_NULL:
#pragma unroll
            for (int j = 0; j < R; j++) out[j] = ta[j] == T_NULL ? L_FALSE : (ta[j] == T_MISSING ? L_MISSING : L_TRUE);
            break;
        case TERM_IS_MISSING:
#pragma unroll
            for (int j = 0; j < R; j++) out[j] = ta[j] == T_MISSING ? L_TRUE : L_FALSE;
            break;
        case TERM_IS_NOT_MISSING:
#pragma unroll
            for (int j = 0; j < R; j++) out[j] = ta[j] == T_MISSING ? L_FALSE : L_TRUE;
            break;
        case TERM_IS_VALUED:
#pragma unroll
            for (int j = 0; j < R; j++) out[j] = ta[j] <= T_NULL ? L_FALSE : L_TRUE;
            break;
        case TERM_IS_NOT_VALUED:
#pragma unroll
            for (int j = 0; j < R; j++) out[j] = ta[j] <= T_NULL ? L_TRUE : L_FALSE;
            break;
        case TERM_TRUTH:
#pragma unroll
            for (int j = 0; j < R; j++) out[j] = truth_l(ta[j], pa[j], P.empty_str_code, P.empty_arr_code, P.empty_obj_code);
            break;
        case TERM_LIKE:
        case TERM_STRFN:
        case TERM_COLL: {
            const uint32_t bit = 1u << (uint32_t)t.b.cpayload;
            const uint32_t want = term_table_tag(t.op);
#pragma unroll
            for (int j = 0; j < R; j++) {
                const uint32_t code = (uint32_t)pa[j];
                const bool hit = ta[j] == want && code < P.match_n && (P.match_bits[code] & bit) != 0;
                out[j] = ta[j] == T_MISSING ? L_MISSING : (ta[j] != want ? L_NULL : (hit ? L_TRUE : L_FALSE));
            }
            break;
        }
        case TERM_IN: {
            const uint32_t flags = (uint32_t)t.b.cpayload, mask = flags & 0xFFu;
            const uint32_t begin = (uint32_t)t.c.cpayload, end = (uint32_t)(t.c.cpayload >> 32);
#pragma unroll
            for (int j = 0; j < R; j++) {
                const uint32_t code = (uint32_t)pa[j];
                const bool str_hit = ta[j] == T_STRING && mask && code < P.match_n && (P.match_bits[code] & mask) != 0;
                out[j] = in_term_l(flags, P.in_nums + begin, end - begin, ta[j], pa[j], str_hit);
            }
            break;
        }
        default: {
            const uint32_t ct = t.b.ctag;
            const uint64_t cp = t.b.cpayload;
            const double cf = num_actual(ct, cp);
#pragma unroll
            for (int j = 0; j < R; j++) {
                uint32_t tg = ta[j];
                int c;
                if (tg == T_INT && ct == T_INT) {
                    int64_t x = (int64_t)pa[j], y = (int64_t)cp;
                    c = x < y ? -1 : (x > y ? 1 : 0);
                } else if (tg == T_INT || tg == T_FLOAT) {
                    c = collate_f64(num_actual(tg, pa[j]), cf);
                } else {
                    c = tg < T_INT ? -1 : 1;
                }
                bool r = t.op == TERM_NUM_LT ? c < 0 : t.op == TERM_NUM_LE ? c <= 0 : t.op == TERM_NUM_GT ? c > 0
                         : t.op == TERM_NUM_GE ? c >= 0 : (c == 0 && (tg == T_INT || tg == T_FLOAT));
                out[j] = tg == T_MISSING ? L_MISSING : (tg == T_NULL ? L_NULL : (r ? L_TRUE : L_FALSE));
            }
// ... 1004 lines not shown

template <class Spec>
static hipError_t launch_spec_records(const Program& P, const FastArgs& F, uint32_t grid, bool wide, const WordLogArgs& L, hipStream_t st) {
    const size_t shmem = sizeof(ScatterLds<Rec16, 512, 4>);
    if (wide) {
        auto k = scan_spec_records_kernel<Spec, 2, 512, true>;
        (void)hipFuncSetAttribute((const void*)k, hipFuncAttributeMaxDynamicSharedMemorySize, (int)shmem);
        hipLaunchKernelGGL(k, dim3(grid), dim3(512), shmem, st, P, F, L);
    } else {
        auto k = scan_spec_records_kernel<Spec, 4, 512, false>;
        (void)hipFuncSetAttribute((const void*)k, hipFuncAttributeMaxDynamicSharedMemorySize, (int)shmem);
        hipLaunchKernelGGL(k, dim3(grid), dim3(512), shmem, st, P, F, L);
    }
    return hipGetLastError();
}
size_t spec_records_lds_bytes() { return sizeof(ScatterLds<Rec16, 512, 4>); }

const std::vector<SpecEntry>& spec_registry() {
    static const std::vector<SpecEntry> reg = {
#define N1K_REG(S) SpecEntry{#S, make_sig<S>(), &launch_spec<S>, &launch_spec_records<S>}
        N1K_REG(Spec_gt_sum), N1K_REG(Spec_lt_sum), N1K_REG(Spec_gtf_sum), N1K_REG(Spec_gt_all), N1K_REG(Spec_gt_count),
        N1K_REG(Spec_sum), N1K_REG(Spec_avg), N1K_REG(Spec_count), N1K_REG(Spec_gt_nokey_count), N1K_REG(Spec_2k_sum),
        N1K_REG(Spec_ik_count), N1K_REG(Spec_ik_sum), N1K_REG(Spec_dik_sum), N1K_REG(Spec_cd_avg), N1K_REG(Spec_cd),
#undef N1K_REG
    };
    return reg;
}

__global__ void init_table_kernel(const Program P, const GlobalTable G, uint64_t first, uint64_t count,
                                  unsigned long long* counters) {
    uint64_t i = (uint64_t)blockIdx.x * blockDim.x + threadIdx.x;
    if (counters && i < kCounters) counters[i] = 0;
    if (i >= count) return;
    uint64_t s = first + i;
    G.keys[s] = kEmptyKey;
    if (G.rep_row) G.rep_row[s] = ~0ull;
    glob_row_init(P, &G.acc[(size_t)s * P.glob_words]);
}

template <int R, int BLOCK>
__global__ __launch_bounds__(BLOCK) void partition_kernel(const Program P, const PartArgs A) {
    const uint32_t tid = threadIdx.x, lane = tid & 63;
    uint32_t unsupported = 0, unpackable = 0;
    __shared__ uint32_t s_cnt[kMaxParts];
    __shared__ unsigned long long s_base[kMaxParts];
    for (uint32_t d = tid; d < kMaxParts; d += BLOCK) s_cnt[d] = 0;
    __syncthreads();
    const uint64_t tile_rows = (uint64_t)BLOCK * R;
    const uint64_t ntiles = (A.nrows + tile_rows - 1) / tile_rows;
    for (uint64_t tile = blockIdx.x; tile < ntiles; tile += gridDim.x) {
        uint64_t row[R];
        bool valid[R], pass[R];
#pragma unroll
        for (int j = 0; j < R; j++) {
            row[j] = tile * tile_rows + (uint64_t)j * BLOCK + tid;
            valid[j] = row[j] < A.nrows;
        }
        eval_predicate<R>(P, row, valid, pass, unsupported);
        uint64_t key[R];
#pragma unroll
        for (int j = 0; j < R; j++) key[j] = 0;
        for (uint32_t k = 0; k < P.nkeys; k++) {
            const KeySpec& ks = P.keys[k];
            uint32_t kt[R];
            uint64_t kp[R];
            load_operand<R>(P, ks.src, row, pass, kt, kp);
#pragma unroll
            for (int j = 0; j < R; j++) {
                uint64_t f = 0, canon = 0;
                if (pass[j] && !pack_key_field(P, ks, kt[j], kp[j], f, canon)) {
                    unpackable = 1;
                    pass[j] = false;
                }
                key[j] = mix64(key[j] ^ canon) + k;
            }
        }
        uint64_t pos[R];
        uint32_t dest[R];
#pragma unroll
        for (int j = 0; j < R; j++) {
            dest[j] = (uint32_t)(((key[j] >> 32) * (uint64_t)A.nparts) >> 32);
            pos[j] = 0;
            for (uint32_t d = 0; d < A.nparts; d++) {
                unsigned long long m = __ballot(pass[j] && dest[j] == d);
                if (m == 0ull) continue;
                int leader = __ffsll((long long)m) - 1;
                uint32_t base = 0;
                if ((int)lane == leader) base = atomicAdd(&s_cnt[d], (uint32_t)__popcll(m));
                base = __shfl(base, leader, 64);
                if (pass[j] && dest[j] == d) pos[j] = base + (uint32_t)__popcll(m & ((1ull << lane) - 1ull));
            }
        }
        __syncthreads();
        for (uint32_t d = tid; d < A.nparts; d += BLOCK) {
            uint32_t n = s_cnt[d];
            s_base[d] = n ? atomicAdd(&A.counts[(size_t)d * (A.count_stride ? A.count_stride : 1u)], (unsigned long long)n) : 0ull;
        }
        __syncthreads();
#pragma unroll
        for (int j = 0; j < R; j++) {
            if (!pass[j]) continue;
            uint64_t r = s_base[dest[j]] + pos[j];
            if (r >= (A.per_dest ? (uint64_t)A.dest_cap[dest[j]] : A.capacity)) {
                if (!(atomicOr(A.err_flags, (uint32_t)ERR_TABLE_FULL) & ERR_TABLE_FULL) && A.region_bytes)
                    for (uint32_t q = 0; q < A.nparts; q++)
                        atomicOr(&A.counts[(size_t)q * A.count_stride + 1], 1ull);
                pass[j] = false;
            }
            pos[j] = A.region_bytes ? r : (uint64_t)dest[j] * A.capacity + r;
        }
        __syncthreads();
        for (uint32_t d = tid; d < A.nparts; d += BLOCK) s_cnt[d] = 0;
        uint64_t roff[R];
#pragma unroll
        for (int j = 0; j < R; j++) roff[j] = A.hdr_bytes;
        for (uint32_t c = 0; c < A.ncopy; c++) {
            Operand o{};
            o.is_const = 0;
            o.col = c;
            uint32_t vt[R];
            uint64_t vp[R];
            load_operand<R>(P, o, row, pass, vt, vp);
#pragma unroll
            for (int j = 0; j < R; j++) {
                if (!pass[j]) continue;
                if (A.per_dest) {
                    char* const reg = (char*)A.counts + (size_t)dest[j] * A.region_bytes;
                    const uint64_t capd = A.dest_cap[dest[j]];
                    if (P.cols[c].kind == COLK_DICT32) {
                        ((uint32_t*)(reg + roff[j]))[pos[j]] = (uint32_t)vp[j];
                        roff[j] = part_region_next(roff[j], capd, 4);
                    } else {
                        ((uint64_t*)(reg + roff[j]))[pos[j]] = vp[j];
                        roff[j] = part_region_next(roff[j], capd, 8);
                        ((uint8_t*)(reg + roff[j]))[pos[j]] = (uint8_t)vt[j];
                        roff[j] = part_region_next(roff[j], capd, 1);
                    }
                    continue;
                }
                const size_t shift = (size_t)dest[j] * A.region_bytes;
                if (P.cols[c].kind == COLK_DICT32) {
                    ((uint32_t*)((char*)A.out_codes[c] + shift))[pos[j]] = (uint32_t)vp[j];
                } else {
                    ((uint8_t*)((char*)A.out_tags[c] + shift))[pos[j]] = (uint8_t)vt[j];
                    ((uint64_t*)((char*)A.out_payload[c] + shift))[pos[j]] = vp[j];
                }
            }
        }
    }
    if (unsupported) atomicOr(A.err_flags, (uint32_t)ERR_UNSUPPORTED_VALUE);
    if (unpackable) atomicOr(A.err_flags, (uint32_t)ERR_UNPACKABLE_KEY);
}

enum { RED_ADD_U64, RED_ADD_F64, RED_OR, RED_MIN_I64, RED_MAX_I64, RED_MIN_U64, RED_MAX_U64 };

template <int OP>
N1K_DEV uint64_t reduce_over_y(uint64_t (*red)[64], uint64_t v) {
    const uint32_t tx = threadIdx.x, ty = threadIdx.y;
    red[ty][tx] = v;
    __syncthreads();
    for (uint32_t off = 8; off > 0; off >>= 1) {
        if (ty < off) {
            uint64_t a = red[ty][tx], b = red[ty + off][tx], r;
            if (OP == RED_ADD_U64) r = a + b;
            else if (OP == RED_ADD_F64) r = f64_bits(as_f64(a) + as_f64(b));
            else if (OP == RED_OR) r = a | b;
            else if (OP == RED_MIN_I64) r = (int64_t)a < (int64_t)b ? a : b;
            else if (OP == RED_MAX_I64) r = (int64_t)a > (int64_t)b ? a : b;
            else if (OP == RED_MIN_U64) r = a < b ? a : b;
            else r = a > b ? a : b;
            red[ty][tx] = r;
        }
        __syncthreads();
    }
    uint64_t out = red[0][tx];
    __syncthreads();
    return out;
}

__global__ __launch_bounds__(1024) void merge_slabs_kernel(const Program P, const FastArgs F, const GlobalTable G,
                                                          uint32_t nblocks_total, unsigned long long* ngroups) {
    __shared__ uint64_t red[16][64];
    const uint32_t S = F.lds_slots;
    const uint32_t s = blockIdx.x * 64 + threadIdx.x;
    const bool in_range = s < S;
    if (blockIdx.x == 0 && blockIdx.y == 0 && threadIdx.y == 0) {
        unsigned long long c = 0;
        for (uint32_t b = threadIdx.x; b < nblocks_total; b += 64) c += F.block_selected[b];
        for (int off = 32; off > 0; off >>= 1) c += __shfl_down(c, off, 64);
        if (threadIdx.x == 0 && c) atomicAdd(F.rows_selected, c);
    }
    const uint32_t Y = 16 * gridDim.y, y = blockIdx.y * 16 + threadIdx.y;
    const size_t slab_words = (size_t)P.lds_words * S * Y;
    const uint32_t nblocks = (in_range && y < nblocks_total) ? (nblocks_total - y + Y - 1) / Y : 0;
    const uint64_t* base = F.slabs + (size_t)y * P.lds_words * S + (in_range ? s : 0);
    uint64_t touched = 0;
#pragma unroll 8
    for (uint32_t b = 0; b < nblocks; b++) touched |= base[b * slab_words] ^ kEmptyKey;
    touched = reduce_over_y<RED_OR>(red, touched);
    const bool leader = threadIdx.y == 0 && in_range && touched != 0;
    long long g = -1;
    if (leader) g = global_find_or_insert(G, fast_slot_key(F, s), F.err_flags, ngroups);
    uint64_t* grow = g >= 0 ? &G.acc[(size_t)g * P.glob_words] : nullptr;
    for (uint32_t a = 0; a < P.naggs; a++) {
        const AggSpec& ag = P.aggs[a];
        if (ag.distinct) continue;
        const uint64_t* l = base + (size_t)ag.lds_off * S;
        unsigned long long* w = grow ? (unsigned long long*)(grow + ag.glob_off) : nullptr;
        switch (ag.kind) {
            case AGG_COUNT:
            case AGG_COUNTN: {
                unsigned long long c = 0;
#pragma unroll 8
                for (uint32_t b = 0; b < nblocks; b++) c += l[b * slab_words];
                c = reduce_over_y<RED_ADD_U64>(red, c);
                if (w && c) atomicAdd(&w[0], c);
                break;
            }
            case AGG_SUM:
            case AGG_AVG: {
                unsigned long long lo = 0, hi = 0, fl = 0, n = 0;
                double fs = 0.0;
                const bool avg = ag.kind == AGG_AVG;
#pragma unroll 4
                for (uint32_t b = 0; b < nblocks; b++) {
                    const uint64_t* lb = l + b * slab_words;
                    int64_t x = (int64_t)lb[0];
                    double f = as_f64(lb[(size_t)S]);
                    fl |= lb[2 * (size_t)S];
                    lo += (unsigned long long)(uint32_t)x;
                    hi += (unsigned long long)(x >> 32);
                    fs += f;
                    if (avg) n += lb[3 * (size_t)S];
                }
                lo = reduce_over_y<RED_ADD_U64>(red, lo);
                hi = reduce_over_y<RED_ADD_U64>(red, hi);
                fs = as_f64(reduce_over_y<RED_ADD_F64>(red, f64_bits(fs)));
                fl = reduce_over_y<RED_OR>(red, fl);
                if (avg) n = reduce_over_y<RED_ADD_U64>(red, n);
                if (!w || !fl) break;
                if (fl & (SF_NONNEG_INT | SF_NEG_INT)) { atomicAdd(&w[0], lo); atomicAdd(&w[1], hi); }
                if (fl & SF_FLOAT) atomicAdd((double*)&w[2], fs);
                atomicOr(&w[3], fl);
                if (avg) atomicAdd(&w[4], n);
                break;
            }
            default: {
                const bool mn = ag.kind == AGG_MIN;
                unsigned long long fl = 0;
                long long iv = mn ? INT64_MAX : INT64_MIN;
                unsigned long long fv = mn ? ~0ull : 0ull, sv = mn ? ~0ull : 0ull;
#pragma unroll 4
                for (uint32_t b = 0; b < nblocks; b++) {
                    const uint64_t* lb = l + b * slab_words;
                    fl |= lb[0];
                    long long x = (long long)lb[(size_t)S];
                    unsigned long long yv = lb[2 * (size_t)S], z = lb[3 * (size_t)S];
                    iv = mn ? (x < iv ? x : iv) : (x > iv ? x : iv);
                    fv = mn ? (yv < fv ? yv : fv) : (yv > fv ? yv : fv);
                    sv = mn ? (z < sv ? z : sv) : (z > sv ? z : sv);
                }
                fl = reduce_over_y<RED_OR>(red, fl);
                if (mn) {
                    iv = (long long)reduce_over_y<RED_MIN_I64>(red, (uint64_t)iv);
                    fv = reduce_over_y<RED_MIN_U64>(red, fv);
                    sv = reduce_over_y<RED_MIN_U64>(red, sv);
                } else {
                    iv = (long long)reduce_over_y<RED_MAX_I64>(red, (uint64_t)iv);
                    fv = reduce_over_y<RED_MAX_U64>(red, fv);
                    sv = reduce_over_y<RED_MAX_U64>(red, sv);
                }
                if (!w || !fl) break;
                atomicOr(&w[0], fl);
                if (fl & MM_INT) { if (mn) atomicMin((long long*)&w[1], iv); else atomicMax((long long*)&w[1], iv); }
                if (fl & MM_FLOAT) { if (mn) atomicMin(&w[2], fv); else atomicMax(&w[2], fv); }
                if (fl & MM_STRING) { if (mn) atomicMin(&w[3], sv); else atomicMax(&w[3], sv); }
                break;
            }
        }
    }
}

__global__ void export_partials_kernel(const Program P, const GlobalTable G, uint32_t nparts, uint64_t cap,
                                       uint64_t* out, uint64_t region_words, uint32_t* err_flags) {
    uint64_t s = (uint64_t)blockIdx.x * blockDim.x + threadIdx.x;
    if (s == 0 && P.wide_count && *P.wide_count)
        for (uint32_t r = 0; r < nparts; r++) atomicOr((unsigned long long*)&out[(size_t)r * region_words + 1], 2ull);
    const uint64_t key = s < G.capacity ? G.keys[s] : kEmptyKey;
    const bool used = key != kEmptyKey;
    const uint32_t d = used ? (uint32_t)(((mix64(key) >> 32) * (uint64_t)nparts) >> 32) : 0xFFFFFFFFu;
    unsigned long long pos = 0;
    unsigned long long todo = __ballot(used);
    const uint32_t lane = threadIdx.x & 63;
    while (todo) {
        const int leader = __ffsll((long long)todo) - 1;
        const uint32_t dl = __shfl(d, leader, 64);
        const unsigned long long same = __ballot(used && d == dl);
        unsigned long long base = 0;
        if ((int)lane == leader) base = atomicAdd((unsigned long long*)&out[(size_t)dl * region_words], (unsigned long long)__popcll(same));
        base = __shfl(base, leader, 64);
        if (used && d == dl) pos = base + (unsigned long long)__popcll(same & ((1ull << lane) - 1ull));
        todo &= ~same;
    }
    if (!used) return;
    uint64_t* region = out + (size_t)d * region_words;
    if (pos >= cap) {
        if (!(atomicOr(err_flags, (uint32_t)ERR_TABLE_FULL) & ERR_TABLE_FULL))
            for (uint32_t r = 0; r < nparts; r++) atomicOr((unsigned long long*)&out[(size_t)r * region_words + 1], 1ull);
        return;
    }
    region[2 + pos] = key;
    uint64_t* acc = region + 2 + cap + pos * P.glob_words;
    for (uint32_t w = 0; w < P.glob_words; w++) acc[w] = G.acc[(size_t)s * P.glob_words + w];
}

N1K_DEV void merge_partial_record(const Program& P, const GlobalTable& G, uint64_t key, const uint64_t* l, uint32_t* err_flags,
                                  bool& fresh, bool unique_keys) {
    long long g = global_find_or_insert_quiet(G, key, err_flags, fresh);
    if (g < 0) return;
    if (fresh && unique_keys) {
        uint64_t* w = &G.acc[(size_t)g * P.glob_words];
        for (uint32_t i = 0; i < P.glob_words; i++) w[i] = l[i];
        return;
    }
    for (uint32_t a = 0; a < P.naggs; a++) {
        const AggSpec& ag = P.aggs[a];
        const uint64_t* p = l + ag.glob_off;
        unsigned long long* w = (unsigned long long*)&G.acc[(size_t)g * P.glob_words + ag.glob_off];
        if (ag.distinct) {
            atomicOr(err_flags, (uint32_t)ERR_UNSUPPORTED_VALUE);
            continue;
        }
        switch (ag.kind) {
            case AGG_COUNT:
            case AGG_COUNTN:
                if (p[0]) atomicAdd(&w[0], (unsigned long long)p[0]);
                break;
            case AGG_SUM:
            case AGG_AVG:
                if (!p[3]) break;
                atomicAdd(&w[0], (unsigned long long)p[0]);
                atomicAdd(&w[1], (unsigned long long)p[1]);
                if (p[3] & SF_FLOAT) atomicAdd((double*)&w[2], as_f64(p[2]));
                atomicOr(&w[3], (unsigned long long)p[3]);
                if (ag.kind == AGG_AVG) atomicAdd(&w[4], (unsigned long long)p[4]);
                break;
            default: {
                if (!p[0]) break;
                bool mn = ag.kind == AGG_MIN;
                atomicOr(&w[0], (unsigned long long)p[0]);
                if (p[0] & MM_INT) { if (mn) atomicMin((long long*)&w[1], (long long)p[1]); else atomicMax((long long*)&w[1], (long long)p[1]); }
                if (p[0] & MM_FLOAT) { if (mn) atomicMin(&w[2], (unsigned long long)p[2]); else atomicMax(&w[2], (unsigned long long)p[2]); }
                if (p[0] & MM_STRING) { if (mn) atomicMin(&w[3], (unsigned long long)p[3]); else atomicMax(&w[3], (unsigned long long)p[3]); }
                break;
            }
        }
    }
}

N1K_DEV void raise_verdict(uint64_t verdict, uint32_t* err_flags) {
    uint32_t f = 0;
    if (verdict & VD_OVERFLOW) f |= ERR_EXCHANGE_OVERFLOW;
    if (verdict & VD_WIDE) f |= ERR_EXCHANGE_WIDE;
    if (verdict & VD_UNPACKABLE) f |= ERR_PEER_UNPACKABLE;
    if (verdict & VD_UNSUPPORTED) f |= ERR_PEER_UNSUPPORTED;
    if (verdict >> VD_STATUS_SHIFT) f |= ERR_PEER_FAILED;
    atomicOr(err_flags, f);
}

__global__ void merge_partials_kernel(const Program P, const GlobalTable G, uint32_t nregions, uint64_t cap,
                                      const uint64_t* in, uint64_t region_words, uint32_t* err_flags,
                                      unsigned long long* ngroups, uint32_t unique_keys) {
    uint64_t i = (uint64_t)blockIdx.x * blockDim.x + threadIdx.x;
    uint32_t r = (uint32_t)(i / cap);
    uint64_t pos = i % cap;
    if (r >= nregions) return;
    uint64_t verdict = 0, status = 0;
    for (uint32_t q = 0; q < nregions; q++) {
        const uint64_t v = in[(size_t)q * region_words + 1];
        verdict |= v;
        status = (v >> VD_STATUS_SHIFT) > status ? (v >> VD_STATUS_SHIFT) : status;
    }
    if (verdict) {
        if (i == 0) {
            raise_verdict(verdict, err_flags);
            if (status) atomicMax((unsigned long long*)err_flags + kPeerStatusFromErr, (unsigned long long)(status & 0xFF));
        }
        return;
    }
    const uint64_t* region = in + (size_t)r * region_words;
    uint64_t count = region[0] < cap ? region[0] : cap;
    bool fresh = false;
    if (pos < count) merge_partial_record(P, G, region[2 + pos], region + 2 + cap + pos * P.glob_words, err_flags, fresh, unique_keys != 0);
    const unsigned long long m = __ballot(fresh);
    if ((threadIdx.x & 63) == 0 && m) atomicAdd(ngroups, (unsigned long long)__popcll(m));
}

__global__ void restamp_ranks_kernel(const Program P, const GlobalTable G) {
    uint64_t s = (uint64_t)blockIdx.x * blockDim.x + threadIdx.x;
    if (s >= G.capacity || G.keys[s] == kEmptyKey) return;
    for (uint32_t a = 0; a < P.naggs; a++) {
        const AggSpec& ag = P.aggs[a];
        if (ag.distinct || (ag.kind != AGG_MIN && ag.kind != AGG_MAX)) continue;
        uint64_t* w = &G.acc[s * P.glob_words + ag.glob_off];
        if (w[0] & MM_STRING) {
            const uint32_t code = (uint32_t)w[3];
            w[3] = ((uint64_t)P.str_rank[code] << 32) | code;
        }
    }
}

hipError_t launch_restamp_ranks(const Program& P, const GlobalTable& G, hipStream_t st) {
    if (!G.capacity) return hipSuccess;
    hipLaunchKernelGGL(restamp_ranks_kernel, dim3((uint32_t)((G.capacity + 255) / 256)), dim3(256), 0, st, P, G);
    return hipGetLastError();
}

__global__ void rehash_kernel(const Program P, const GlobalTable oldt, const GlobalTable newt, uint32_t* err_flags,
                              unsigned long long* scratch) {
    uint64_t s = (uint64_t)blockIdx.x * blockDim.x + threadIdx.x;
    if (s >= oldt.capacity) return;
    uint64_t key = oldt.keys[s];
    if (key == kEmptyKey) return;
    bool fresh = false;
    long long g = global_find_or_insert_quiet(newt, key, err_flags, fresh);
    if (g < 0) return;
    for (uint32_t w = 0; w < P.glob_words; w++) newt.acc[(size_t)g * P.glob_words + w] = oldt.acc[(size_t)s * P.glob_words + w];
    if (newt.rep_row && oldt.rep_row) newt.rep_row[g] = oldt.rep_row[s];
}


// ... 11 lines not shown
        put_value(fin, T_NULL, 0);
        *part = pt;
        return;
    }
    if (ag.distinct) {
        pt.distinct = (int64_t)w[0];
        if (ag.kind == AGG_COUNT || ag.kind == AGG_COUNTN) {
            put_value(fin, T_INT, w[0]);
        } else if (w[0] == 0) {
            put_value(fin, T_NULL, 0);
        } else {
            uint64_t fl = w[8];
            __int128 tot = ((__int128)(int64_t)w[6] << 32) + (__int128)(unsigned __int128)w[5];
            bool fits = tot >= (__int128)INT64_MIN && tot <= (__int128)INT64_MAX;
            bool int_exact = !(fl & SF_FLOAT) && !(fl & SF_NEG_INT) && fits;
            double itot = fits ? (double)(int64_t)tot : (double)(int64_t)w[6] * 4294967296.0 + (double)w[5];
            double fsum = as_f64(w[7]);
            pt.isum = int_exact ? (int64_t)tot : 0;
            pt.fsum = int_exact ? 0.0 : fsum + itot;
            pt.flags = (int_exact ? 1u : 0u) | ((fl & SF_FLOAT) ? 2u : 0u);
            if (ag.kind == AGG_SUM) {
                if (int_exact) put_value(fin, T_INT, (uint64_t)(int64_t)tot);
                else put_value(fin, T_FLOAT, f64_bits(fsum + itot));
            } else {
                double avg = (int_exact ? (double)(int64_t)tot : fsum + itot) / (double)w[0];
                if (is_int_f64(avg)) put_value(fin, T_INT, (uint64_t)go_f2i(avg));
                else put_value(fin, T_FLOAT, f64_bits(avg));
            }
        }
        *part = pt;
        return;
    }
    switch (ag.kind) {
        case AGG_COUNT:
        case AGG_COUNTN:
            pt.count = (int64_t)w[0];
            put_value(fin, T_INT, w[0]);
            break;
        case AGG_SUM:
        case AGG_AVG: {
            uint64_t fl = w[3];
            bool has_nn = fl & SF_NONNEG_INT, has_ng = fl & SF_NEG_INT, has_f = fl & SF_FLOAT;
            __int128 tot = ((__int128)(int64_t)w[1] << 32) + (__int128)(unsigned __int128)w[0];
            bool fits = tot >= (__int128)INT64_MIN && tot <= (__int128)INT64_MAX;
            bool int_exact = !has_f && !(has_nn && has_ng) && fits;
            double itot = (double)(int64_t)w[1] * 4294967296.0 + (double)w[0];
            if (fits) itot = (double)(int64_t)tot;
            double fsum = as_f64(w[2]);
            uint64_t n = ag.kind == AGG_AVG ? w[4] : 0;
            pt.count = (int64_t)n;
            pt.isum = int_exact ? (int64_t)tot : 0;
            pt.fsum = int_exact ? fsum : fsum + itot;
            pt.flags = (int_exact ? 1u : 0u) | (has_f ? 2u : 0u);
            if (fl == 0) {
                put_value(fin, T_NULL, 0);
            } else if (ag.kind == AGG_SUM) {
                if (int_exact) put_value(fin, T_INT, (uint64_t)(int64_t)tot);
                else put_value(fin, T_FLOAT, f64_bits(fsum + itot));
            } else {
                double sm = int_exact ? (double)(int64_t)tot : fsum + itot;
                double avg = sm / (double)n;
                if (is_int_f64(avg)) put_value(fin, T_INT, (uint64_t)go_f2i(avg));
                else put_value(fin, T_FLOAT, f64_bits(avg));
            }
            break;
        }
        default: {
            uint64_t fl = w[0];
            bool mn = ag.kind == AGG_MIN;
            uint32_t tag = T_NULL;
            uint64_t p = 0;
            bool has_num = fl & (MM_INT | MM_FLOAT);
            bool has_bool = fl & (MM_FALSE | MM_TRUE);
            int which = 0;
            if (mn) which = has_bool ? 1 : (has_num ? 2 : ((fl & MM_STRING) ? 3 : ((fl & MM_OTHER) ? 4 : 0)));
            else which = (fl & MM_OTHER) ? 4 : ((fl & MM_STRING) ? 3 : (has_num ? 2 : (has_bool ? 1 : 0)));
            if (which == 1) {
                tag = mn ? ((fl & MM_FALSE) ? T_FALSE : T_TRUE) : ((fl & MM_TRUE) ? T_TRUE : T_FALSE);
            } else if (which == 2) {
                bool hi = fl & MM_INT, hf = fl & MM_FLOAT;
                double f = f64_unsortable(w[2]);
                int64_t iv = (int64_t)w[1];
                bool pick_int = hi;
                if (hi && hf) {
                    int c = collate_f64((double)iv, f);
                    pick_int = mn ? c <= 0 : c >= 0;
                }
                if (pick_int) { tag = T_INT; p = (uint64_t)iv; }
                else { tag = T_FLOAT; p = f64_bits(f); }
            } else if (which == 3) {
                tag = T_STRING;
                p = w[3] & 0xFFFFFFFFull;
            } else if (which == 4) {
                atomicOr(err_flags, (uint32_t)ERR_UNSUPPORTED_VALUE);
            }
            pt.ext_tag = tag;
            pt.ext_payload = p;
            put_value(fin, tag, p);
            break;
        }
    }
    *part = pt;
}

constexpr uint32_t kFinalizeChunkMax = 16384;
__global__ __launch_bounds__(256) void finalize_kernel(const Program P, const GlobalTable G, OutValue* out_keys, OutValue* out_aggs,
                                                       OutPartial* out_parts, uint64_t* out_rep, unsigned long long* out_count,
                                                       uint64_t max_out, uint32_t* err_flags, uint32_t chunk) {
    __shared__ uint32_t wave_cnt[4];
    __shared__ unsigned long long chunk_base;
    const uint32_t tid = threadIdx.x, lane = tid & 63, wave = tid >> 6;
    const uint64_t lo = (uint64_t)blockIdx.x * chunk;
    const uint64_t hi = lo + chunk < G.capacity ? lo + chunk : G.capacity;
    uint32_t mine = 0;
    for (uint64_t s = lo + tid; s < hi; s += 256) mine += G.keys[s] != kEmptyKey ? 1u : 0u;
    for (int off = 32; off > 0; off >>= 1) mine += __shfl_down(mine, off, 64);
    if (lane == 0) wave_cnt[wave] = mine;
    __syncthreads();
    if (tid == 0) {
        const uint32_t total = wave_cnt[0] + wave_cnt[1] + wave_cnt[2] + wave_cnt[3];
        chunk_base = total ? atomicAdd(out_count, (unsigned long long)total) : 0ull;
    }
    __syncthreads();
    unsigned long long next = chunk_base;
    for (uint64_t s0 = lo; s0 < hi; s0 += 256) {
        const uint64_t s = s0 + tid;
        const uint64_t key = s < hi ? G.keys[s] : kEmptyKey;
        const bool used = key != kEmptyKey;
        const unsigned long long m = __ballot(used);
        __syncthreads();
        if (lane == 0) wave_cnt[wave] = (uint32_t)__popcll(m);
        __syncthreads();
        uint32_t before = 0;
        for (uint32_t w = 0; w < wave; w++) before += wave_cnt[w];
        const uint32_t step_total = wave_cnt[0] + wave_cnt[1] + wave_cnt[2] + wave_cnt[3];
        const unsigned long long idx = next + before + (uint32_t)__popcll(m & ((1ull << lane) - 1ull));
        next += step_total;
        if (!used || idx >= max_out) continue;
        for (uint32_t k = 0; k < P.nkeys; k++) {
            const KeySpec& ks = P.keys[k];
            uint64_t field = ks.bits >= 64 ? key : ((key >> ks.shift) & ((1ull << ks.bits) - 1ull));
            uint32_t tag;
            uint64_t p;
            unpack_key_field(P, ks.mode, field, tag, p);
            put_value(&out_keys[idx * P.nkeys + k], tag, p);
        }
        const uint64_t* g = &G.acc[(size_t)s * P.glob_words];
        for (uint32_t a = 0; a < P.naggs; a++)
            finalize_agg(P, P.aggs[a], g, &out_aggs[idx * P.naggs + a], &out_parts[idx * P.naggs + a], err_flags);
        if (out_rep) out_rep[idx] = P.emit_packed_key ? key : (G.rep_row ? G.rep_row[s] : ~0ull);
    }
}

constexpr uint32_t kFinalizeSmallMax = 8192;
__global__ __launch_bounds__(1024) void finalize_small_kernel(const Program P, const GlobalTable G, OutValue* out_keys, OutValue* out_aggs,
                                                             OutPartial* out_parts, uint64_t* out_rep, unsigned long long* counters,
                                                             unsigned long long* host_counters, uint64_t max_out, uint32_t* err_flags,
                                                             uint32_t clear) {
    __shared__ uint32_t wave_cnt[16];
    const uint32_t tid = threadIdx.x, lane = tid & 63, wave = tid >> 6;
    unsigned long long next = 0;
    for (uint64_t s0 = 0; s0 < G.capacity; s0 += 1024) {
        const uint64_t s = s0 + tid;
        const uint64_t key = s < G.capacity ? G.keys[s] : kEmptyKey;
        const bool used = key != kEmptyKey;
        const unsigned long long m = __ballot(used);
        __syncthreads();
        if (lane == 0) wave_cnt[wave] = (uint32_t)__popcll(m);
        __syncthreads();
        uint32_t before = 0, step_total = 0;
        for (uint32_t w = 0; w < 16; w++) {
            before += w < wave ? wave_cnt[w] : 0u;
            step_total += wave_cnt[w];
        }
        const unsigned long long idx = next + before + (uint32_t)__popcll(m & ((1ull << lane) - 1ull));
        next += step_total;
        if (!used) continue;
        uint64_t* g = &G.acc[(size_t)s * P.glob_words];
        if (idx < max_out) {
            for (uint32_t k = 0; k < P.nkeys; k++) {
                const KeySpec& ks = P.keys[k];
                uint64_t field = ks.bits >= 64 ? key : ((key >> ks.shift) & ((1ull << ks.bits) - 1ull));
                uint32_t tag;
                uint64_t p;
                unpack_key_field(P, ks.mode, field, tag, p);
                put_value(&out_keys[idx * P.nkeys + k], tag, p);
            }
            for (uint32_t a = 0; a < P.naggs; a++)
                finalize_agg(P, P.aggs[a], g, &out_aggs[idx * P.naggs + a], &out_parts[idx * P.naggs + a], err_flags);
            if (out_rep) out_rep[idx] = P.emit_packed_key ? key : (G.rep_row ? G.rep_row[s] : ~0ull);
        }
        if (clear) {
            G.keys[s] = kEmptyKey;
            if (G.rep_row) G.rep_row[s] = ~0ull;
            glob_row_init(P, g);
        }
    }
    __syncthreads();
    if (tid == 0) counters[2] = next;
    __syncthreads();
    if (tid < kCounters) {
        host_counters[tid] = __hip_atomic_load(&counters[tid], __ATOMIC_RELAXED, __HIP_MEMORY_SCOPE_AGENT);
        if (clear) counters[tid] = 0;
    }
}

hipError_t launch_finalize_small(const Program& P, const GlobalTable& G, OutValue* out_keys, OutValue* out_aggs, OutPartial* out_parts,
                                 uint64_t* out_rep, unsigned long long* counters, unsigned long long* host_counters, uint64_t max_out,
                                 uint32_t* err_flags, bool clear, hipStream_t st) {
    if (G.capacity > kFinalizeSmallMax) return hipErrorInvalidValue;
    hipLaunchKernelGGL(finalize_small_kernel, dim3(1), dim3(1024), 0, st, P, G, out_keys, out_aggs, out_parts, out_rep, counters,
                       host_counters, max_out, err_flags, clear ? 1u : 0u);
    return hipGetLastError();
}

N1K_DEV uint64_t order_image(const Program& P, uint64_t tag, uint64_t p, bool desc);
__global__ void finalize_region_kernel(const Program P, const uint64_t* region, uint64_t cap, uint64_t count, OutValue* out_keys,
                                       OutValue* out_aggs, OutPartial* out_parts, uint64_t* out_rep, uint32_t* err_flags,
                                       const uint32_t* cand, OutValue* ord, uint32_t ord_is_key, uint32_t ord_index, uint64_t* images,
                                       uint32_t desc) {
    const uint64_t j = (uint64_t)blockIdx.x * blockDim.x + threadIdx.x;
    if (j >= count) return;
    const uint64_t i = cand ? (uint64_t)cand[j] : j;
    const uint64_t key = region[2 + i];
    const uint64_t* g = region + 2 + cap + i * P.glob_words;
    if (ord || images) {
        OutValue v, term;
        OutPartial part;
        term.tag = T_MISSING;
        term.payload = 0;
        for (uint32_t a = 0; a < P.naggs; a++) {
            finalize_agg(P, P.aggs[a], g, &v, &part, err_flags);
            if (!ord_is_key && a == ord_index) term = v;
        }
        if (ord_is_key) {
            const KeySpec& ks = P.keys[ord_index];
            uint64_t field = ks.bits >= 64 ? key : ((key >> ks.shift) & ((1ull << ks.bits) - 1ull));
            uint32_t tag;
            uint64_t p;
            unpack_key_field(P, ks.mode, field, tag, p);
            put_value(&term, tag, p);
        }
        if (images) images[i] = order_image(P, term.tag, term.payload, desc != 0);
        else ord[i] = term;
        return;
    }
    for (uint32_t k = 0; k < P.nkeys; k++) {
        const KeySpec& ks = P.keys[k];
        uint64_t field = ks.bits >= 64 ? key : ((key >> ks.shift) & ((1ull << ks.bits) - 1ull));
        uint32_t tag;
        uint64_t p;
        unpack_key_field(P, ks.mode, field, tag, p);
        put_value(&out_keys[j * P.nkeys + k], tag, p);
    }
    for (uint32_t a = 0; a < P.naggs; a++)
        finalize_agg(P, P.aggs[a], g, &out_aggs[j * P.naggs + a], &out_parts[j * P.naggs + a], err_flags);
    if (out_rep) out_rep[j] = ~0ull;
}

template <int R, int BLOCK>
__global__ __launch_bounds__(BLOCK) void project_records_kernel(const Program P, const ProjectArgs A) {
    __shared__ uint32_t wave_cnt[BLOCK / 64];
    __shared__ unsigned long long tile_base;
    __shared__ uint32_t s_hist[256];
    const uint32_t tid = threadIdx.x;
    for (uint32_t i = tid; i < 256; i += BLOCK) s_hist[i] = 0;
    __syncthreads();
    uint32_t unsupported = 0, unpackable = 0;
    const uint64_t tile_rows = (uint64_t)BLOCK * R;
    const uint64_t ntiles = (A.nrows + tile_rows - 1) / tile_rows;
    for (uint64_t tile = blockIdx.x; tile < ntiles; tile += gridDim.x) {
        uint64_t row[R];
        bool valid[R], pass[R];
#pragma unroll
        for (int j = 0; j < R; j++) {
            row[j] = tile * tile_rows + (uint64_t)j * BLOCK + tid;
            valid[j] = row[j] < A.nrows;
        }
        eval_predicate<R>(P, row, valid, pass, unsupported);
        uint64_t key[R];
#pragma unroll
        for (int j = 0; j < R; j++) key[j] = 0;
        for (uint32_t k = 0; k < P.nkeys; k++) {
            const KeySpec& ks = P.keys[k];
            uint32_t kt[R];
            uint64_t kp[R];
            load_operand<R>(P, ks.src, row, pass, kt, kp);
#pragma unroll
            for (int j = 0; j < R; j++) {
                uint64_t f = 0, canon = 0;
                if (pass[j] && !pack_key_field(P, ks, kt[j], kp[j], f, canon)) {
                    unpackable = 1;
                    pass[j] = false;
                }
                key[j] |= f << ks.shift;
            }
        }
        uint32_t mine = 0;
#pragma unroll
        for (int j = 0; j < R; j++) {
            mine += pass[j] ? 1u : 0u;
            if (pass[j] && A.hist) atomicAdd(&s_hist[radix_bin(key[j], 56)], 1u);
        }
        unsigned long long pos = tile_reserve<BLOCK>(mine, A.cursor, wave_cnt, &tile_base, tid);
        unsigned long long q = pos;
#pragma unroll
        for (int j = 0; j < R; j++)
            if (pass[j] && q < A.capacity) A.out.key[q++] = key[j];
        for (uint32_t e = 0; e < A.nsrc; e++) {
            uint32_t vt[R];
            uint64_t vp[R];
            load_operand<R>(P, A.src[e], row, pass, vt, vp);
            q = pos;
#pragma unroll
            for (int j = 0; j < R; j++)
                if (pass[j] && q < A.capacity) {
                    A.out.pay[e][q] = vp[j];
                    A.out.tag[e][q] = (uint8_t)vt[j];
                    q++;
                }
        }
        if (pos + mine > A.capacity) atomicOr(A.err_flags, (uint32_t)ERR_TABLE_FULL);
        __syncthreads();
    }
    if (unsupported) atomicOr(A.err_flags, (uint32_t)ERR_UNSUPPORTED_VALUE);
    if (unpackable) atomicOr(A.err_flags, (uint32_t)ERR_UNPACKABLE_KEY);
    __syncthreads();
    if (A.hist)
        for (uint32_t i = tid; i < 256; i += BLOCK)
            if (s_hist[i]) atomicAdd(&A.hist[i], (unsigned long long)s_hist[i]);
}

template <int R, int BLOCK>
__global__ __launch_bounds__(BLOCK) void probe_keys_kernel(const Program P, uint64_t nrows, const GlobalTable G, uint32_t* err_flags,
                                                          unsigned long long* ngroups) {
    const uint32_t tid = threadIdx.x;
    uint32_t unsupported = 0, fresh = 0;
    const uint64_t tile_rows = (uint64_t)BLOCK * R;
    const uint64_t ntiles = (nrows + tile_rows - 1) / tile_rows;
    for (uint64_t tile = blockIdx.x; tile < ntiles; tile += gridDim.x) {
        uint64_t row[R];
        bool valid[R], pass[R];
#pragma unroll
        for (int j = 0; j < R; j++) {
            row[j] = tile * tile_rows + (uint64_t)j * BLOCK + tid;
            valid[j] = row[j] < nrows;
        }
        eval_predicate<R>(P, row, valid, pass, unsupported);
        uint64_t key[R];
#pragma unroll
        for (int j = 0; j < R; j++) key[j] = 0;
        for (uint32_t k = 0; k < P.nkeys; k++) {
            const KeySpec& ks = P.keys[k];
            uint32_t kt[R];
            uint64_t kp[R];
            load_operand<R>(P, ks.src, row, pass, kt, kp);
#pragma unroll
            for (int j = 0; j < R; j++) {
                uint64_t f = 0, canon = 0;
                if (pass[j] && !pack_key_field(P, ks, kt[j], kp[j], f, canon)) pass[j] = false;
                key[j] |= f << ks.shift;
            }
        }
#pragma unroll
        for (int j = 0; j < R; j++) {
// ... 1138 lines not shown
```

### query_amd/csrc/n1k_scan.cpp

```cpp
#include "n1k_engine.h"

using namespace n1k;
using namespace n1k_eng;

namespace n1k_eng {

bool build_fast_args(n1k_handle* h, uint32_t max_slots, FastArgs& F, bool fuse, bool partition_only) {
    const Program& P = h->prog;
    memset(&F, 0, sizeof F);
    const uint32_t ni = (uint32_t)h->plan.paths.size(), nd = (uint32_t)h->derived.size();
    if (fuse) {
        if (nd == 0 || nd > (uint32_t)kFastDerived || ni == 0 || ni > (uint32_t)kFastCols) return false;
        for (uint32_t d = 0; d < nd; d++)
            for (uint32_t k = 0; k < h->derived[d].nops; k++) {
                const Operand& o = h->derived[d].ops[k];
                if (h->derived[d].op >= AR_GREATEST) return false;
                if (!o.is_const && o.col >= ni + d) return false;
                if (o.is_const) F.dconst[d][k] = o.cpayload;
            }
        F.nderived = nd;
    }
    if (h->opt.fast == 0 || P.want_rep_row || P.ncols == 0 || (!fuse && P.ncols > (uint32_t)kFastCols)) return false;
    if (P.nkeys > (uint32_t)kFastKeys || (!partition_only && (P.naggs > (uint32_t)kFastAggs || P.naggs == 0))) return false;
    uint32_t term_ix[2] = {0, 0};
// ... 76 lines not shown
}

static SpecSig make_plan_sig(const n1k_handle* h, const FastArgs& F, ShapeUse use) {
    const Program& P = h->prog;
    SpecSig g{};
    g.ncols = (int)F.ncols; g.nterms = (int)F.nterms; g.nkeys = (int)F.nkeys; g.naggs = (int)F.naggs;
    g.hashed = (int)F.hashed;
    for (uint32_t c = 0; c < F.ncols; c++) g.col_kind[c] = F.cols[c].kind;
    for (uint32_t t = 0; t < F.nterms; t++) {
        g.terms[t].op = F.terms[t].op;
        g.terms[t].col = F.terms[t].col;
        bool num = F.terms[t].op >= TERM_NUM_LT && F.terms[t].op <= TERM_NUM_EQ;
        g.terms[t].const_int = num && F.terms[t].ctag == T_INT ? 1u : 0u;
    }
    for (uint32_t k = 0; k < F.nkeys; k++) g.key_col[k] = F.keys[k].col;
    for (uint32_t a = 0; a < F.naggs; a++) {
        g.aggs[a].kind = P.aggs[a].kind;
        g.aggs[a].has_operand = P.aggs[a].has_operand;
        g.aggs[a].col = P.aggs[a].has_operand ? F.agg_col[a] : 0u;
        g.aggs[a].distinct = P.aggs[a].distinct ? 1u : 0u;
    }
    g.nderived = (int)F.nderived;
    for (uint32_t d = 0; d < F.nderived; d++) {
        g.derived[d].op = h->derived[d].op;
        g.derived[d].nops = h->derived[d].nops;
        for (uint32_t k = 0; k < h->derived[d].nops; k++) {
            const Operand& o = h->derived[d].ops[k];
            g.derived[d].ops[k].is_const = o.is_const ? 1u : 0u;
            g.derived[d].ops[k].v = o.is_const ? o.ctag : o.col;
        }
    }
    if (use == ShapeUse::Scan) g.seg = h->push_nseg > 1 ? 1 : 0;
    if (use == ShapeUse::Partition) {
        g.mode = 1;
        g.hashed = 0;
    }
    return g;
}

bool shape_compiles(const n1k_handle* h, const FastArgs& F, ShapeUse use, std::string* log) {
    return jit_compile_check(make_plan_sig(h, F, use), log);
}

ShapeKernel shape_kernel(n1k_handle* h, const FastArgs& F, ShapeUse use, uint64_t nrows, size_t table_bytes) {
    if (!h->opt.spec) return {};
    const SpecSig g = make_plan_sig(h, F, use);
    if (use != ShapeUse::Partition && !g.seg)
        for (const SpecEntry& e : spec_registry())
            if (memcmp(&e.sig, &g, sizeof g) == 0) return {&e, nullptr, 1u};
    bool build = h->opt.jit && (use == ShapeUse::Records || h->opt.jit == 2 || nrows >= h->opt.jit_min_rows);
    if (use == ShapeUse::Scan) {
        bool key_kinds_hashed = false;
        for (uint32_t k = 0; k < F.nkeys; k++) key_kinds_hashed |= F.keys[k].col >= F.ncols || F.cols[F.keys[k].col].kind != COLK_DICT32;
        build = build && table_bytes <= 64 * 1024 && key_kinds_hashed == (F.hashed != 0);
    } else if (use == ShapeUse::Partition) {
        size_t lds = 2048 + 2048 + 4096;
        for (uint32_t c = 0; c < F.ncols; c++) lds += 2048u * (F.cols[c].kind == COLK_DICT32 ? 4u : 9u);
        build = build && lds + match_lds_bytes(F) <= 60 * 1024;
    }
    if (!build) return {};
    const JitKernel* k = jit_get(g);
    if (k->failed || !(use == ShapeUse::Scan ? k->wide : (use == ShapeUse::Records ? k->rec_wide : k->part_wide))) {
        h->jit_log = k->log;
        return {};
    }
    return {nullptr, k, F.nderived ? 3u : 2u};
}

struct ScanChoice {
    bool interpreter = true;
    bool shaped = false;
    bool fuse = false;
    ShapeKernel kernel;
    FastArgs F;
    uint32_t ndist = 0;
    Program compact;
    uint32_t fblock = 0, per_cu = 0, grid_cap = 0;
    bool use_slabs = false;
    uint32_t table_bytes = 0, scatter_bytes = 0, match_lds = 0, dcache_slots = 0, lds_total = 0;
    uint32_t max_slots = 0, slots = 0, block = 0, rpl = 0, direct_stride[kMaxKeys] = {}, direct_radix[kMaxKeys] = {};
    bool direct = false;
};

static ScanChoice choose_scan(n1k_handle* h, uint64_t nrows) {
    const Program& P = h->prog;
    ScanChoice c;
    FastArgs& F = c.F;
    c.block = h->opt.block ? h->opt.block : 1024;
    c.rpl = c.block == 1024 ? h->opt.rows_per_lane : 4;
    c.max_slots = (uint32_t)std::min<uint64_t>(h->opt.lds_bytes / (P.lds_words * 8), 1u << 15);
    if (c.max_slots < 2) return c;
    const uint32_t direct_max_slots = (uint32_t)std::min<uint64_t>((156u * 1024u) / (P.lds_words * 8), 1u << 15);
    for (uint32_t a = 0; a < P.naggs; a++) c.ndist += P.aggs[a].distinct ? 1u : 0u;
    if (c.ndist) {
        c.compact = P;
        uint32_t w = 1;
        for (uint32_t a = 0; a < c.compact.naggs; a++) {
            AggSpec& ag = c.compact.aggs[a];
            ag.lds_off = w;
            if (ag.distinct) ag.lds_n = 0;
            else w += (ag.kind == AGG_COUNT || ag.kind == AGG_COUNTN) ? 1u : (ag.kind == AGG_SUM ? kLdsWordsSum : (ag.kind == AGG_AVG ? kLdsWordsAvg : kWordsMinMax));
        }
        c.compact.lds_words = w;
    }
    const uint32_t ndist = c.ndist, lds_words = ndist ? c.compact.lds_words : P.lds_words;
    if (h->opt.agg_mode != N1K_MODE_LDS_HASH) {
        if (!h->derived_ready && h->opt.fuse_arith && build_fast_args(h, direct_max_slots, F, true)) {
            c.kernel = shape_kernel(h, F, ShapeUse::Scan, nrows, (size_t)F.lds_slots * P.lds_words * 8);
            c.fuse = c.shaped = (bool)c.kernel;
        }
        if (!c.fuse && (c.shaped = build_fast_args(h, direct_max_slots, F, false)))
            c.kernel = shape_kernel(h, F, ShapeUse::Scan, nrows, (size_t)F.lds_slots * lds_words * 8);
    }
    c.interpreter = !c.shaped || (!c.kernel && (F.hashed || ndist || h->push_nrows_dev || h->push_nseg));
    if (c.interpreter) {
        c.direct = h->opt.agg_mode != N1K_MODE_LDS_HASH;
        uint64_t domain = 1;
        for (uint32_t k = 0; k < P.nkeys && c.direct; k++) {
            if (P.keys[k].mode != KEYM_DICT) c.direct = false;
            uint64_t radix = (uint64_t)h->dict.size() + 2;
            c.direct_stride[k] = (uint32_t)domain;
            c.direct_radix[k] = (uint32_t)std::min<uint64_t>(radix, 0xFFFFFFFFull);
            domain *= radix;
            if (domain > c.max_slots) c.direct = false;
        }
        c.slots = c.direct ? (uint32_t)std::max<uint64_t>(domain, 2) : c.max_slots;
        if (P.nkeys == 0) c.slots = 2;
        return c;
    }
    c.table_bytes = F.lds_slots * lds_words * 8;
    c.match_lds = match_lds_bytes(F);
    c.scatter_bytes = ndist * (2048u * 8u + 2u * 256u * 4u + 256u * 4u + 256u * 8u + 2048u) + (ndist ? 64u : 0u);
    if (ndist) {
        const uint32_t without = c.table_bytes + c.scatter_bytes + c.match_lds;
        const uint32_t share = 160u * 1024u / std::max(1u, std::min(3u, 160u * 1024u / (without + 512u)));
        for (uint32_t sl = 4096; sl >= 64; sl >>= 1)
            if (without + ndist * sl * 8u + 512u <= share) { c.dcache_slots = sl; break; }
    }
    c.lds_total = c.table_bytes + c.scatter_bytes + ndist * c.dcache_slots * 8u + c.match_lds;
    c.fblock = h->opt.block == 1024 || h->opt.block == 512 ? h->opt.block : (c.table_bytes <= 72 * 1024 ? 512u : 1024u);
    if (ndist) c.fblock = 512;
    c.per_cu = c.fblock == 512 ? (c.lds_total <= 48 * 1024 ? 3u : (c.lds_total <= 72 * 1024 ? 2u : 1u))
                               : (c.lds_total <= 72 * 1024 ? 2u : 1u);
    if (ndist) c.per_cu = std::max(1u, std::min(3u, 160u * 1024u / (c.lds_total + 512u)));
    if (c.kernel.jit && c.fblock != 512) {
        c.fblock = 512;
        c.per_cu = c.table_bytes + c.match_lds <= 48 * 1024 ? 3u : 2u;
    }
    c.grid_cap = h->opt.grid_blocks ? h->opt.grid_blocks : (uint32_t)(h->num_cus * c.per_cu);
    c.use_slabs = !F.hashed && (h->opt.slabs == 1 ? c.table_bytes >= 4096 : h->opt.slabs == 2);
    return c;
}

static n1k_status launch_chunk(n1k_handle* h, const ScanChoice& c, const Program& P, FastArgs& F, const WordLogArgs& L, uint64_t off, uint64_t n) {
    unsigned long long* ngroups = h->groups.counters.p + CTR_GROUPS;
    auto launch = [&](uint32_t g, bool wide) {
        if (c.kernel.spec) return c.kernel.spec->launch(P, F, h->groups.table, ngroups, g, c.fblock, wide, L, h->stream);
        if (c.kernel.jit) return jit_launch(c.kernel.jit, P, F, h->groups.table, ngroups, g, wide, L, c.ndist, h->stream);
        return launch_scan_fast(P, F, h->groups.table, ngroups, g, c.fblock, h->opt.rows_per_lane, h->stream);
    };
    F.row_base = h->row_base + off;
    std::copy_n(P.cols, F.ncols, F.cols);
    advance_cols(F.cols, F.ncols, off);
    const bool wide = c.kernel && cols_wide_aligned(F.cols, F.ncols) && h->opt.wide && n >= 2;
    const uint64_t n_main = wide && !h->push_nrows_dev && !h->push_nseg ? (n & ~1ull) : n;
    F.nrows = (uint32_t)n_main;
    const uint64_t items = wide ? (n_main + 1) / 2 : n_main;
    const uint32_t rpl = !c.kernel ? h->opt.rows_per_lane : (wide ? 2 : 4);
    uint64_t tiles = (items + (uint64_t)c.fblock * rpl - 1) / ((uint64_t)c.fblock * rpl);
    if (c.ndist) tiles = (tiles + 3) / 4;
    const uint32_t g = (uint32_t)std::max<uint64_t>(1, std::min<uint64_t>(c.grid_cap, tiles));
    if (c.use_slabs && g > 1) {
        HIP_TRY(h, h->groups.slabs.ensure((size_t)g * P.lds_words * F.lds_slots));
        HIP_TRY(h, h->groups.block_sel.ensure(g));
        F.slabs = h->groups.slabs.p;
        F.block_selected = h->groups.block_sel.p;
    }
    HIP_TRY(h, launch(g, wide));
    if (F.slabs) HIP_TRY(h, launch_merge_slabs(P, F, h->groups.table, g, ngroups, h->stream, h->opt.merge_chunks));
    F.slabs = nullptr;
    if (n_main < n) {
        advance_cols(F.cols, F.ncols, n_main);
        F.nrows = (uint32_t)(n - n_main);
        F.row_base += n_main;
        HIP_TRY(h, launch(1, false));
    }
    return N1K_OK;
}

static n1k_status run_shaped(n1k_handle* h, ScanChoice& c, const ScanArgs& A, uint64_t nrows) {
    const Program& P = c.ndist ? c.compact : h->prog;
    FastArgs& F = c.F;
    F.err_flags = h->groups.errp;
    F.rows_selected = h->groups.counters.p + CTR_ROWS_SELECTED;
    F.nrows_dev = h->push_nrows_dev;
    if (h->push_nseg > 1) {
        if (h->push_nseg > kMaxSegments || nrows >= (1ull << 31)) return fail(h, N1K_INVALID, "segmented batch too large");
        F.nseg = h->push_nseg;
        F.seg_rows = (uint32_t)h->push_seg_rows;
        F.seg_count_stride = kCursorStride;
        F.seg_counts = h->push_seg_counts;
    }
    WordLogArgs L{};
    if (c.ndist) {
        n1k_status st = distinct_grow_regions(h, P, nrows, A, c.dcache_slots, L);
        if (st != N1K_OK) return st;
    }
    hipEvent_t e0 = get_event(h), e1 = get_event(h);
    if (e0) (void)hipEventRecord(e0, h->stream);
    const uint64_t chunk = 1ull << 31;
    for (uint64_t off = 0; off < nrows; off += chunk) {
        n1k_status st = launch_chunk(h, c, P, F, L, off, std::min<uint64_t>(chunk, nrows - off));
        if (st != N1K_OK) return st;
    }
    if (e1) (void)hipEventRecord(e1, h->stream);
    h->timing.events.emplace_back(e0, e1);
    h->timing.stats.agg_mode = F.hashed ? N1K_MODE_LDS_HASH : N1K_MODE_LDS_DIRECT;
    return N1K_OK;
}

static n1k_status run_interpreter(n1k_handle* h, const ScanChoice& c, ScanArgs& A, uint64_t nrows) {
    const Program& P = h->prog;
    memcpy(A.direct_stride, c.direct_stride, sizeof A.direct_stride);
    memcpy(A.direct_radix, c.direct_radix, sizeof A.direct_radix);
    A.lds_slots = c.slots;
    A.lds_max_fill = std::max(1u, (uint32_t)((uint64_t)c.slots * 5 / 8));
    A.err_flags = h->groups.errp;
    A.rows_selected = h->groups.counters.p + CTR_ROWS_SELECTED;
    uint64_t tile_rows = (uint64_t)c.block * c.rpl;
    uint64_t ntiles = (nrows + tile_rows - 1) / tile_rows;
    uint32_t per_cu = c.block == 1024 ? 1 : (c.block == 512 ? 2 : 4);
    uint32_t grid = h->opt.grid_blocks ? h->opt.grid_blocks : (uint32_t)(h->num_cus * per_cu);
    grid = (uint32_t)std::max<uint64_t>(1, std::min<uint64_t>(grid, ntiles));
    hipEvent_t e0 = get_event(h), e1 = get_event(h);
    if (e0) (void)hipEventRecord(e0, h->stream);
    if (h->push_nseg > 1) {
        Program Ps = P;
        for (uint32_t sg = 0; sg < h->push_nseg; sg++) {
            std::copy_n(P.cols, P.ncols, Ps.cols);
            advance_cols(Ps.cols, P.ncols, (uint64_t)sg * h->push_seg_rows);
            ScanArgs As = A;
            As.nrows = h->push_seg_rows;
            As.nrows_dev = h->push_seg_counts + (size_t)sg * kCursorStride;
            const uint64_t nt = (h->push_seg_rows + tile_rows - 1) / tile_rows;
            const uint32_t g = (uint32_t)std::max<uint64_t>(1, std::min<uint64_t>(grid, nt));
            HIP_TRY(h, launch_scan_group(Ps, As, h->groups.table, h->groups.counters.p + CTR_GROUPS, g, c.block, c.rpl, c.direct, h->stream));
        }
    } else
        HIP_TRY(h, launch_scan_group(P, A, h->groups.table, h->groups.counters.p + CTR_GROUPS, grid, c.block, c.rpl, c.direct, h->stream));
    if (e1) (void)hipEventRecord(e1, h->stream);
    h->timing.events.emplace_back(e0, e1);
    h->timing.stats.agg_mode = c.direct ? N1K_MODE_LDS_DIRECT : N1K_MODE_LDS_HASH;
    return N1K_OK;
}

n1k_status run_group_batch(n1k_handle* h, const n1k_batch* b) {
    n1k_status st = ensure_table(h, b->nrows);
    if (st != N1K_OK) return st;
    ScanArgs A{};
    A.nrows = b->nrows;
    A.nrows_dev = h->push_nrows_dev;
    A.row_base = h->row_base;
    if (h->has_distinct) {
        st = distinct_grow_logs(h, b->nrows, A);
        if (st != N1K_OK) return st;
    }
    ScanChoice c = choose_scan(h, b->nrows);
    if (c.max_slots < 2) return fail(h, N1K_UNSUPPORTED, "accumulator row too wide for LDS");
    if (!c.fuse) {
        st = materialize_derived(h, b);
        if (st != N1K_OK) return st;
        if (c.ndist) std::copy_n(h->prog.cols, h->prog.ncols, c.compact.cols);
    }
    if (c.shaped) h->timing.stats.spec_kernel = c.kernel.stat;
    return c.interpreter ? run_interpreter(h, c, A, b->nrows) : run_shaped(h, c, A, b->nrows);
}

bool filter_stream_fast(const n1k_handle* h) {
    const Program& P = h->prog;
    if (!(h->opt.wide && P.nlogic == 1 && P.logic[0].op == LOGIC_PUSH)) return false;
    const Term& t = P.terms[P.logic[0].arg];
    return t.op >= TERM_NUM_LT && t.op <= TERM_NUM_EQ && !t.a.is_const && t.a.col < (uint32_t)h->plan.paths.size() &&
           P.cols[t.a.col].kind == COLK_TAGGED64 && (uintptr_t)P.cols[t.a.col].payload % 16 == 0 && (uintptr_t)P.cols[t.a.col].tags % 2 == 0;
}

uint32_t filter_stream_grid(const n1k_handle* h, uint64_t ntiles, bool fast) {
    if (fast)
        return (uint32_t)std::min<uint64_t>(ntiles, (uint64_t)h->num_cus * (h->opt.grid_blocks ? h->opt.grid_blocks : 5));
    return (uint32_t)std::min<uint64_t>(ntiles, (uint64_t)h->num_cus * 4);
}

n1k_status run_filter_batch(n1k_handle* h, const n1k_batch* b) {
    Program& P = h->prog;
    if (b->nrows == 0) return N1K_OK;
    hipEvent_t e0 = get_event(h), e1 = get_event(h);
    unsigned long long total = 0;
    const uint64_t ntiles = (b->nrows + kFilterStreamTile - 1) / kFilterStreamTile;
    HIP_TRY(h, h->filter.tile_off.ensure(ntiles + 1));
    HIP_TRY(h, h->filter.sel.ensure(b->nrows));
    const bool fast = filter_stream_fast(h);
    const uint32_t grid = filter_stream_grid(h, ntiles, fast);
    if (e0) (void)hipEventRecord(e0, h->stream);
    HIP_TRY(h, launch_filter_stream(P, b->nrows, h->row_base, h->filter.sel.p, (unsigned long long*)h->filter.tile_off.p,
                                    (unsigned long long*)h->filter.tile_off.p + ntiles, h->groups.counters.p + CTR_FILTER_TOTAL, h->groups.errp, grid, h->stream, fast));
    h->timing.stats.spec_kernel = fast ? 1u : 0u;
    if (e1) (void)hipEventRecord(e1, h->stream);
    HIP_TRY(h, hipMemcpyAsync(&total, h->groups.counters.p + CTR_FILTER_TOTAL, sizeof total, hipMemcpyDeviceToHost, h->stream));
    HIP_TRY(h, hipStreamSynchronize(h->stream));
    if (total) {
        size_t old = h->filter.selected.size();
        h->filter.selected.resize(old + total);
        HIP_TRY(h, hipMemcpyAsync(h->filter.selected.data() + old, h->filter.sel.p, total * 8, hipMemcpyDeviceToHost, h->stream));
    }
    h->timing.events.emplace_back(e0, e1);
    HIP_TRY(h, hipStreamSynchronize(h->stream));
    h->timing.stats.rows_selected += total;
    return N1K_OK;
}

n1k_status bind_columns(n1k_handle* h, const n1k_batch* b, bool defer) {
    Program& P = h->prog;
    auto resolve = [&](Operand& o) {
        if (o.is_const && o.ctag == T_STRING && o.pad == 1) {
            o.cpayload = intern(h, h->const_strings[(size_t)o.cpayload]);
            o.pad = 0;
        }
    };
    for (uint32_t t = 0; t < P.nterms; t++) { resolve(P.terms[t].a); resolve(P.terms[t].b); resolve(P.terms[t].c); }
    for (uint32_t k = 0; k < P.nkeys; k++) resolve(P.keys[k].src);
    for (uint32_t a = 0; a < P.naggs; a++) resolve(P.aggs[a].src);
    for (auto& d : h->derived)
        for (uint32_t k = 0; k < d.nops; k++) resolve(d.ops[k]);
    const uint32_t ni = (uint32_t)h->plan.paths.size();
    for (uint32_t c = 0; c < ni; c++) {
        P.cols[c].kind = b->cols[c].kind == N1K_COL_DICT32 ? COLK_DICT32 : COLK_TAGGED64;
        P.cols[c].tags = b->cols[c].tags;
        P.cols[c].payload = b->cols[c].payload;
        P.cols[c].codes = b->cols[c].codes;
    }
    bool tagged_key = false;
    for (uint32_t k = 0; k < P.nkeys; k++) tagged_key |= P.keys[k].mode == KEYM_TAGGED;
    if (tagged_key) {
        P.nan_code = intern(h, "NaN");
        P.pinf_code = intern(h, "+Infinity");
        P.ninf_code = intern(h, "-Infinity");
    }
    P.dict_size = (uint32_t)h->dict.size();
    P.empty_str_code = lookup_code(h, "");
    P.empty_arr_code = lookup_code(h, "[]");
    P.empty_obj_code = lookup_code(h, "{}");
    h->derived_ready = h->derived.empty();
    if (h->derived_ready) return N1K_OK;
    for (size_t i = 0; i < h->derived.size(); i++) {
        DevCol& d = P.cols[ni + i];
        d.kind = COLK_TAGGED64;
        d.tags = nullptr;
        d.payload = nullptr;
        d.codes = nullptr;
    }
    return defer ? N1K_OK : materialize_derived(h, b);
}

n1k_status materialize_derived(n1k_handle* h, const n1k_batch* b) {
    Program& P = h->prog;
    if (h->derived_ready) return N1K_OK;
    const uint32_t ni = (uint32_t)h->plan.paths.size();
    for (const auto& d : h->derived)
        if (d.op >= AR_GREATEST) {
            n1k_status rst = ensure_rank(h);
            if (rst != N1K_OK) return rst;
            break;
        }
    h->dv_tags.resize(h->derived.size());
    h->dv_payload.resize(h->derived.size());
    for (size_t i = 0; i < h->derived.size(); i++) {
        if (h->dv_tags[i].n < b->nrows) HIP_TRY(h, hipStreamSynchronize(h->stream));
        HIP_TRY(h, h->dv_tags[i].ensure(std::max<uint64_t>(b->nrows, 1)));
        HIP_TRY(h, h->dv_payload[i].ensure(std::max<uint64_t>(b->nrows, 1)));
        ArithArgs A{};
        A.op = h->derived[i].op;
        A.nops = h->derived[i].nops;
        for (uint32_t k = 0; k < A.nops; k++) A.ops[k] = h->derived[i].ops[k];
        for (uint32_t c = 0; c < ni + i; c++) A.cols[c] = P.cols[c];
        A.nrows = b->nrows;
        A.out_tags = h->dv_tags[i].p;
        A.out_payload = h->dv_payload[i].p;
        A.str_rank = h->d_rank.p;
        A.err_flags = h->groups.errp;
        HIP_TRY(h, launch_arith(A, h->stream));
        DevCol& d = P.cols[ni + i];
        d.kind = COLK_TAGGED64;
        d.tags = A.out_tags;
        d.payload = A.out_payload;
        d.codes = nullptr;
    }
    h->derived_ready = true;
    return N1K_OK;
}

n1k_status push_device(n1k_handle* h, const n1k_batch* b) {
    if (h->stop_flag.load()) return fail(h, N1K_STOPPED, "operator was stopped");
    h->device_clean = false;
    n1k_status st = ensure_device(h);
    if (st != N1K_OK) return st;
    st = validate_batch(h, b);
    if (st != N1K_OK) return st;
    if (!h->layout_fixed) {
        st = fix_layout(h, b);
        if (st != N1K_OK) return st;
    }
    st = flush_pending(h);
    if (st != N1K_OK) return st;
    const bool first_rows = h->row_base == 0 && h->groups.merged_bound == 0;
    PartitionPlan pp;
    const bool can_partition = h->plan.has_group && !h->push_nrows_dev && !h->push_nseg && partition_eligible(h, pp);
    uint64_t head = b->nrows;
    bool decide = false;
    if (can_partition && h->opt.agg_mode == N1K_MODE_PARTITIONED) head = 0;
    else if (can_partition && h->opt.agg_mode == N1K_MODE_AUTO && b->nrows >= h->opt.partition_min_rows && !small_key_domain(h)) {
        head = std::min<uint64_t>(b->nrows, h->opt.partition_probe_rows);
        decide = true;
    }
    auto view = [&](uint64_t off, uint64_t n, std::vector<n1k_col>& cols, n1k_batch& v) {
        cols.assign(b->cols, b->cols + b->ncols);
        advance_cols(cols.data(), b->ncols, off);
        v.nrows = n;
        v.ncols = b->ncols;
        v.cols = cols.data();
    };
    std::vector<n1k_col> cols;
    n1k_batch v{};
    view(0, b->nrows, cols, v);
    const bool defer = h->plan.has_group && !decide && !(can_partition && head == 0);
    st = bind_columns(h, &v, defer);
    if (st != N1K_OK) return st;
    st = ensure_rank(h);
    if (st != N1K_OK) return st;
    st = ensure_match_table(h);
    if (st != N1K_OK) return st;
    bool partition = can_partition && head == 0 && b->nrows > 0;
    uint64_t groups_est = b->nrows;
    if (decide && first_rows && h->opt.partition_sticky && h->part.sticky.valid && b->nrows >= h->part.sticky.rows / 2 && b->nrows <= h->part.sticky.rows * 2) {
        decide = false;
        partition = true;
        groups_est = std::min<uint64_t>(b->nrows, h->part.sticky.groups_est * b->nrows / std::max<uint64_t>(h->part.sticky.rows, 1) + 1024);
    }
    if (decide) {
        st = ensure_table(h, head);
        if (st != N1K_OK) return st;
        unsigned long long before = 0, after = 0;
        HIP_TRY(h, hipMemcpyAsync(&before, h->groups.counters.p + CTR_GROUPS, sizeof before, hipMemcpyDeviceToHost, h->stream));
        const uint32_t grid = (uint32_t)std::max<uint64_t>(1, std::min<uint64_t>((uint64_t)h->num_cus * 4, (head + 1023) / 1024));
        HIP_TRY(h, launch_probe_keys(h->prog, head, h->groups.table, h->groups.errp, h->groups.counters.p + CTR_GROUPS, grid, h->stream));
        HIP_TRY(h, hipMemcpyAsync(&after, h->groups.counters.p + CTR_GROUPS, sizeof after, hipMemcpyDeviceToHost, h->stream));
        HIP_TRY(h, hipStreamSynchronize(h->stream));
        const uint64_t fresh = after > before ? after - before : 0;
        partition = fresh >= h->opt.partition_min_groups;
        const double m = (double)head, d = (double)std::max<uint64_t>(1, fresh);
        if (d < 0.98 * m) {
            double lo = d, hi = 1e18;
            for (int it = 0; it < 200; it++) {
                const double U = std::sqrt(lo * hi);
                if (U * (1.0 - std::exp(-m / U)) < d) lo = U; else hi = U;
            }
            const double U = lo, nn = (double)b->nrows;
            groups_est = std::min<uint64_t>(groups_est, (uint64_t)(2.0 * U * (1.0 - std::exp(-nn / U))) + 1024);
        }
        if (partition && first_rows && h->groups.table.capacity) {
            HIP_TRY(h, launch_init_table(h->prog, h->groups.table, 0, h->groups.table.capacity, nullptr, h->stream));
            HIP_TRY(h, hipMemsetAsync(h->groups.counters.p + CTR_GROUPS, 0, sizeof(unsigned long long), h->stream));
        }
    }
    if (b->nrows) {
        if (!h->plan.has_group) st = run_filter_batch(h, &v);
        else if (partition) {
            bool done = false;
            st = run_group_records(h, &v, pp, groups_est, first_rows, &done);
            h->part.sticky.valid = st == N1K_OK && done && first_rows && h->opt.agg_mode == N1K_MODE_AUTO;
            h->part.sticky.rows = b->nrows;
            h->part.sticky.groups_est = groups_est;
            if (st == N1K_OK && !done) st = run_group_partitioned(h, &v, pp, groups_est, first_rows);
        } else
            st = run_group_batch(h, &v);
        if (st != N1K_OK) return st;
    }
    h->row_base += b->nrows;
    h->timing.stats.rows_in += b->nrows;
    h->timing.stats.batches += 1;
    h->timing.stats.bytes_scanned += b->nrows * batch_bytes_per_row(h);
    return N1K_OK;
}

n1k_status stage_host_batch(n1k_handle* h, const n1k_batch* batch, std::vector<n1k_col>& dcols) {
    uint32_t nc = batch->ncols;
    const int set = h->stage.cur;
    auto& s_tags = h->stage.tags[set];
    auto& s_payload = h->stage.payload[set];
    auto& s_codes = h->stage.codes[set];
    s_tags.resize(std::max<size_t>(s_tags.size(), nc));
    s_payload.resize(std::max<size_t>(s_payload.size(), nc));
    s_codes.resize(std::max<size_t>(s_codes.size(), nc));
    if (!h->stage.copy_stream) {
        HIP_TRY(h, hipStreamCreateWithFlags(&h->stage.copy_stream, hipStreamNonBlocking));
        HIP_TRY(h, hipEventCreateWithFlags(&h->stage.copied, hipEventDisableTiming));
        for (int i = 0; i < 2; i++) HIP_TRY(h, hipEventCreateWithFlags(&h->stage.free_ev[i], hipEventDisableTiming));
    }
    if (h->stage.busy[set]) HIP_TRY(h, hipStreamWaitEvent(h->stage.copy_stream, h->stage.free_ev[set], 0));
    dcols.assign(nc, n1k_col{});
    uint64_t n = batch->nrows;
    for (uint32_t c = 0; c < nc; c++) {
        const n1k_col& col = batch->cols[c];
        dcols[c] = col;
        if (col.kind == N1K_COL_DICT32) {
            HIP_TRY(h, s_codes[c].ensure(n));
            if (n) HIP_TRY(h, hipMemcpyAsync(s_codes[c].p, col.codes, n * 4, hipMemcpyHostToDevice, h->stage.copy_stream));
            dcols[c].codes = s_codes[c].p;
        } else {
            HIP_TRY(h, s_tags[c].ensure(n));
            HIP_TRY(h, s_payload[c].ensure(n));
            if (n) {
                HIP_TRY(h, hipMemcpyAsync(s_tags[c].p, col.tags, n, hipMemcpyHostToDevice, h->stage.copy_stream));
                HIP_TRY(h, hipMemcpyAsync(s_payload[c].p, col.payload, n * 8, hipMemcpyHostToDevice, h->stage.copy_stream));
            }
            dcols[c].tags = s_tags[c].p;
            dcols[c].payload = s_payload[c].p;
        }
    }
    HIP_TRY(h, hipEventRecord(h->stage.copied, h->stage.copy_stream));
    HIP_TRY(h, hipStreamWaitEvent(h->stream, h->stage.copied, 0));
    HIP_TRY(h, hipEventSynchronize(h->stage.copied));
    return N1K_OK;
}

n1k_status staged_batch_issued(n1k_handle* h) {
    const int set = h->stage.cur;
    HIP_TRY(h, hipEventRecord(h->stage.free_ev[set], h->stream));
    h->stage.busy[set] = true;
    h->stage.cur ^= 1;
    return N1K_OK;
}

}
```

Baseline: 325.1 billion rows/s.

## Fold per-block slabs directly into result rows, skipping merge into global table

When a single-chunk device query runs from a clean table with small key domain, the slab merge is deferred from the scan and replaced at finish time by a fused fold_rows kernel. That kernel reduces the per-block LDS slabs, joins with any existing global-table entries, finalizes output rows, and copies the counters out via a last-block ticket. This removes the separate merge_slabs and finalize_small launches and the global-table atomic round trip. In exchange it adds a new code path with complex eligibility conditions and extra handle state (pending slabs, clean_at_push) that must stay consistent across reset and finish.

```diff
diff --git a/query_amd/build.py b/query_amd/build.py
--- a/query_amd/build.py
+++ b/query_amd/build.py
@@ -10,7 +10,7 @@
 LIB = os.path.join(HERE, "libn1k.so")
 SOURCES = ["n1k_kernels.hip", "n1k_bins.hip", "n1k_jsondev.hip", "n1k_matchtable.hip", "n1k_order.hip", "n1k_rowdistinct.hip", "n1k_order.cpp", "n1k_rowdistinct.cpp", "n1k_matchtable.cpp", "n1k_like.cpp", "n1k_coll.cpp", "n1k_in.cpp", "n1k_strfn.cpp", "n1k_jsonpush.cpp", "n1k_plan.cpp", "n1k_engine.cpp", "n1k_scan.cpp", "n1k_select.cpp", "n1k_partitioned.cpp", "n1k_distinct.cpp",
            "n1k_finish.cpp", "n1k_tail.cpp", "n1k_exchange.cpp", "n1k_jit.cpp", "n1k_json.cpp"]
-HEADERS = ["n1k_types.h", "n1k_device.h", "n1k_tables.h", "n1k_scatter.h", "n1k_spec.h", "n1k_like.h", "n1k_coll.h", "n1k_in.h", "n1k_strfn.h", "n1k_order.h", "n1k_rowdistinct.h", "n1k_jit.h", "n1k_kernels.h", "n1k_plan.h", os.path.join("..", "..", "include", "n1k.h")]
+HEADERS = ["n1k_types.h", "n1k_device.h", "n1k_tables.h", "n1k_fold.h", "n1k_scatter.h", "n1k_spec.h", "n1k_like.h", "n1k_coll.h", "n1k_in.h", "n1k_strfn.h", "n1k_order.h", "n1k_rowdistinct.h", "n1k_jit.h", "n1k_kernels.h", "n1k_plan.h", os.path.join("..", "..", "include", "n1k.h")]
 HOST_HEADERS = ["n1k_engine.h", "n1k_buf.h", "n1k_wire.h"]
 ARCH = "gfx950"
 
diff --git a/query_amd/csrc/n1k_engine.cpp b/query_amd/csrc/n1k_engine.cpp
--- a/query_amd/csrc/n1k_engine.cpp
+++ b/query_amd/csrc/n1k_engine.cpp
@@ -549,6 +549,8 @@
     h->failure_global = false;
     h->row_base = 0;
     h->groups.merged_bound = 0;
+    h->groups.pending.grid = 0;
+    h->groups.pending.clean_at_push = false;
     h->filter.selected.clear();
     h->filter.has_sel32 = false;
     h->res.keys.clear();
@@ -891,13 +893,12 @@
     const double t0 = trace ? now() : 0;
     n1k_status st = n1k_reset(h);
     const double t1 = trace ? now() : 0;
+    h->clear_on_finish = true;
     if (st == N1K_OK) st = n1k_push_device_batch(h, batch);
     const double t2 = trace ? now() : 0;
-    if (st == N1K_OK) {
-        h->clear_on_finish = true;
-        st = n1k_finish(h, out);
-        h->clear_on_finish = false;
-    }
+    if (st == N1K_OK) st = n1k_finish(h, out);
+    h->clear_on_finish = false;
+    h->groups.pending.grid = 0;
     if (trace) {
         h->timing.host_us[0] += t1 - t0;
         h->timing.host_us[1] += t2 - t1;
diff --git a/query_amd/csrc/n1k_engine.h b/query_amd/csrc/n1k_engine.h
--- a/query_amd/csrc/n1k_engine.h
+++ b/query_amd/csrc/n1k_engine.h
@@ -167,6 +167,7 @@
     CTR_FILTER_TOTAL = 3,
     CTR_REHASH_SCRATCH = 4,
     CTR_DISTINCT_REGION_WORDS = 5,
+    CTR_TAIL_TICKET = 6,
     CTR_PAIR_LOG_CURSORS = 8,
     CTR_ERR_FLAGS = 12,
     CTR_WIDE_VALUES = 13,
@@ -183,6 +184,8 @@
 };
 static_assert(CTR_ERR_FLAGS + kPeerStatusFromErr == CTR_PEER_STATUS, "the verdict kernel writes the peer status this far behind the flags");
 static_assert(CTR_ROWDISTINCT_REACHED < kCounters && CTR_ROWDISTINCT_REACHED == CTR_ROWDISTINCT_COUNT + 1, "every counter word lies inside the buffer (CTR_ROWDISTINCT_REACHED is the last)");
+static_assert(CTR_ROWS_SELECTED == 0 && CTR_GROUPS == 1 && CTR_OUT_COUNT == 2 && CTR_TAIL_TICKET > CTR_DISTINCT_REGION_WORDS && CTR_TAIL_TICKET < CTR_PAIR_LOG_CURSORS,
+              "the query's last kernels (finalize_small_kernel, fold_rows_kernel) write words [0], [1] and [2] by number");
 static_assert(CTR_PAIR_LOG_CURSORS + kMaxDistinct <= CTR_ERR_FLAGS && CTR_WORD_LOG_CURSORS + kMaxDistinct <= CTR_OPTIMISTIC_OVERFLOW, "cursor words overlap their neighbours");
 
 struct GroupTable {
@@ -194,6 +197,11 @@
     DevBuf<unsigned long long> counters;
     DevBuf<uint64_t> wide_int, wide_flt;
     uint64_t merged_bound = 0;
+    struct PendingSlabs {
+        bool clean_at_push = false;
+        uint32_t grid = 0;
+        FastArgs F{};
+    } pending;
 };
 uint32_t intern(n1k_handle* h, const std::string& s);
 uint32_t lookup_code(const n1k_handle* h, const char* s);
@@ -386,6 +394,7 @@
 n1k_status project_groups(n1k_handle* h, uint64_t ng);
 n1k_status order_groups(n1k_handle* h, uint64_t& ng);
 n1k_status array_agg_groups(n1k_handle* h, uint64_t ng, const unsigned long long* counters);
+bool slabs_to_rows(const n1k_handle* h, const FastArgs& F, uint32_t g, bool only_chunk, bool whole);
 void publish_result(n1k_handle* h, uint64_t ng, bool partials, n1k_result* out);
 
 }
diff --git a/query_amd/csrc/n1k_finish.cpp b/query_amd/csrc/n1k_finish.cpp
--- a/query_amd/csrc/n1k_finish.cpp
+++ b/query_amd/csrc/n1k_finish.cpp
@@ -40,6 +40,15 @@
     return std::min<uint64_t>(h->groups.table.capacity, 4096);
 }
 
+namespace n1k_eng {
+bool slabs_to_rows(const n1k_handle* h, const FastArgs& F, uint32_t g, bool only_chunk, bool whole) {
+    if (!h->clear_on_finish || !h->groups.pending.clean_at_push || !only_chunk || !whole || h->push_nrows_dev || h->push_nseg) return false;
+    if (!F.slabs || F.hashed || g <= 1 || h->opt.merge_chunks != 0 || h->prog.wide_int || h->has_array_agg) return false;
+    const uint64_t spec = speculative_groups(h), cap = h->groups.table.capacity;
+    return spec && cap <= kFinalizeSmallMax && F.lds_slots <= std::min<uint64_t>(std::min<uint64_t>(cap, spec), h->opt.max_groups);
+}
+}
+
 static n1k_status zero_out_count(n1k_handle* h) {
     if (h->res.out_count_dirty) HIP_TRY(h, hipMemsetAsync(h->groups.counters.p + CTR_OUT_COUNT, 0, sizeof(unsigned long long), h->stream));
     h->res.out_count_dirty = true;
@@ -50,13 +59,25 @@
     if (!h->device_ready) return h->timing.stats.rows_in == 0 ? ensure_device(h) : N1K_OK;
     HIP_TRY(h, hipSetDevice(h->device));
     ST_TRY(ensure_pinned_counters(h));
+    GroupTable::PendingSlabs& ps = h->groups.pending;
+    const bool fold = ps.grid && slabs_to_rows(h, ps.F, ps.grid, true, true);
+    if (ps.grid && !fold) {
+        HIP_TRY(h, launch_merge_slabs(h->prog, ps.F, h->groups.table, ps.grid, h->groups.counters.p + CTR_GROUPS, h->stream, h->opt.merge_chunks));
+        ps.grid = 0;
+    }
     F.spec_groups = speculative_groups(h);
     if (F.spec_groups) {
         F.lay = OutLayout(F.spec_groups, h->plan.keys.size(), h->plan.aggs.size());
         HIP_TRY(h, h->res.pin_out.ensure(F.lay.total + kCounters * sizeof(unsigned long long)));
         char* d = F.rows = h->res.pin_out.p;
         unsigned long long* host_counters = (unsigned long long*)(d + F.lay.total);
-        if (h->groups.table.capacity <= 8192) {
+        if (fold) {
+            HIP_TRY(h, launch_fold_rows(h->prog, ps.F, h->groups.table, ps.grid, F.lay.k(d), F.lay.a(d), F.lay.p(d), F.lay.r(d), h->groups.counters.p, CTR_TAIL_TICKET,
+                                        host_counters, F.spec_groups, h->stream));
+            ps.grid = 0;
+            h->res.out_count_dirty = false;
+            h->device_clean = true;
+        } else if (h->groups.table.capacity <= kFinalizeSmallMax) {
             const bool clear = h->clear_on_finish && !h->prog.wide_int;
             HIP_TRY(h, launch_finalize_small(h->prog, h->groups.table, F.lay.k(d), F.lay.a(d), F.lay.p(d), F.lay.r(d), h->groups.counters.p,
                                              host_counters, F.spec_groups, h->groups.errp, clear, h->stream));
@@ -74,6 +95,10 @@
         F.wait_end = std::chrono::steady_clock::now();
         h->timing.host_us[3] += std::chrono::duration<double, std::micro>(F.wait_end - w0).count();
         memcpy(F.counters, host_counters, sizeof F.counters);
+        if (fold && F.counters[CTR_TAIL_TICKET]) {
+            h->device_clean = false;
+            F.counters[CTR_TAIL_TICKET] = 0;
+        }
     } else {
         HIP_TRY(h, hipMemcpyAsync(h->res.pin_counters.p, h->groups.counters.p, sizeof F.counters, hipMemcpyDeviceToHost, h->stream));
         mark_query_end(h);
diff --git a/query_amd/csrc/n1k_fold.h b/query_amd/csrc/n1k_fold.h
--- /dev/null
+++ b/query_amd/csrc/n1k_fold.h
@@ -0,0 +1,97 @@
+#pragma once
+#include <stdint.h>
+#include "n1k_types.h"
+
+namespace n1k {
+
+#if defined(__HIP__)
+#define N1K_HD __host__ __device__ inline
+#else
+#define N1K_HD inline
+#endif
+
+enum : uint32_t { FOLD_ADD_U64 = 0, FOLD_ADD_F64, FOLD_OR, FOLD_MIN_I64, FOLD_MAX_I64, FOLD_MIN_U64, FOLD_MAX_U64 };
+constexpr uint32_t kFoldMaxWords = 5;
+
+N1K_HD constexpr uint64_t fold_word(uint32_t op, uint64_t a, uint64_t b) {
+    switch (op) {
+        case FOLD_ADD_U64: return a + b;
+        case FOLD_ADD_F64: return __builtin_bit_cast(uint64_t, __builtin_bit_cast(double, a) + __builtin_bit_cast(double, b));
+        case FOLD_OR: return a | b;
+        case FOLD_MIN_I64: return (int64_t)a < (int64_t)b ? a : b;
+        case FOLD_MAX_I64: return (int64_t)a > (int64_t)b ? a : b;
+        case FOLD_MIN_U64: return a < b ? a : b;
+        default: return a > b ? a : b;
+    }
+}
+
+N1K_HD constexpr uint32_t fold_slab_words(uint32_t kind) {
+    return (kind == AGG_COUNT || kind == AGG_COUNTN) ? 1u : (kind == AGG_SUM ? kLdsWordsSum : (kind == AGG_AVG ? kLdsWordsAvg : kWordsMinMax));
+}
+N1K_HD constexpr uint32_t fold_acc_words(uint32_t kind) {
+    return (kind == AGG_COUNT || kind == AGG_COUNTN) ? 1u : (kind == AGG_SUM ? kGlobWordsSum : (kind == AGG_AVG ? kGlobWordsAvg : kWordsMinMax));
+}
+
+N1K_HD constexpr uint32_t fold_word_op(uint32_t kind, uint32_t i) {
+    switch (kind) {
+        case AGG_COUNT:
+        case AGG_COUNTN: return FOLD_ADD_U64;
+        case AGG_SUM:
+        case AGG_AVG: return i == 2 ? FOLD_ADD_F64 : (i == 3 ? FOLD_OR : FOLD_ADD_U64);
+        case AGG_MIN: return i == 0 ? FOLD_OR : (i == 1 ? FOLD_MIN_I64 : FOLD_MIN_U64);
+        default: return i == 0 ? FOLD_OR : (i == 1 ? FOLD_MAX_I64 : FOLD_MAX_U64);
+    }
+}
+
+N1K_HD constexpr uint64_t fold_identity(uint32_t kind, uint32_t i) {
+    if (kind == AGG_MIN) return i == 0 ? 0ull : (i == 1 ? (uint64_t)INT64_MAX : ~0ull);
+    if (kind == AGG_MAX) return i == 1 ? (uint64_t)INT64_MIN : 0ull;
+    return 0ull;
+}
+
+N1K_HD constexpr uint64_t fold_slab_identity(uint32_t kind, uint32_t i) { return (kind == AGG_MIN || kind == AGG_MAX) ? fold_identity(kind, i) : 0ull; }
+
+N1K_HD constexpr uint32_t fold_flags_word(uint32_t kind) { return (kind == AGG_SUM || kind == AGG_AVG) ? 3u : 0u; }
+
+N1K_HD constexpr bool fold_word_live(uint32_t kind, uint32_t i, uint64_t flags) {
+    switch (kind) {
+        case AGG_COUNT:
+        case AGG_COUNTN: return flags != 0;
+        case AGG_SUM:
+        case AGG_AVG: return i < 2 ? (flags & (SF_NONNEG_INT | SF_NEG_INT)) != 0 : (i == 2 ? (flags & SF_FLOAT) != 0 : flags != 0);
+        default: return i == 0 ? flags != 0 : (i == 1 ? (flags & MM_INT) != 0 : (i == 2 ? (flags & MM_FLOAT) != 0 : (flags & MM_STRING) != 0));
+    }
+}
+
+N1K_HD void fold_slab(uint32_t kind, uint64_t* acc, const uint64_t* l) {
+    if (kind == AGG_SUM || kind == AGG_AVG) {
+        const int64_t x = (int64_t)l[0];
+        acc[0] += (uint64_t)(uint32_t)x;
+        acc[1] += (uint64_t)(x >> 32);
+        acc[2] = fold_word(FOLD_ADD_F64, acc[2], l[1]);
+        acc[3] |= l[2];
+        if (kind == AGG_AVG) acc[4] += l[3];
+        return;
+    }
+    const uint32_t n = fold_acc_words(kind);
+    for (uint32_t i = 0; i < kFoldMaxWords; i++)
+        if (i < n) acc[i] = fold_word(fold_word_op(kind, i), acc[i], l[i]);
+}
+
+N1K_HD void fold_init(uint32_t kind, uint64_t* acc) {
+    for (uint32_t i = 0; i < kFoldMaxWords; i++) acc[i] = fold_identity(kind, i);
+}
+
+N1K_HD void fold_join(uint32_t kind, uint64_t* acc, const uint64_t* other) {
+    const uint32_t n = fold_acc_words(kind);
+    for (uint32_t i = 0; i < kFoldMaxWords; i++)
+        if (i < n) acc[i] = fold_word(fold_word_op(kind, i), acc[i], other[i]);
+}
+
+N1K_HD void fold_row(uint32_t kind, const uint64_t* acc, uint64_t* row) {
+    const uint32_t n = fold_acc_words(kind);
+    for (uint32_t i = 0; i < kFoldMaxWords; i++)
+        if (i < n) row[i] = acc[i];
+}
+
+}
diff --git a/query_amd/csrc/n1k_kernels.h b/query_amd/csrc/n1k_kernels.h
--- a/query_amd/csrc/n1k_kernels.h
+++ b/query_amd/csrc/n1k_kernels.h
@@ -6,6 +6,7 @@
 namespace n1k {
 
 constexpr int kFilterStreamTile = 8192;
+constexpr uint32_t kFinalizeSmallMax = 8192;
 
 struct OutValue {
     uint64_t tag;
@@ -115,6 +116,9 @@
 hipError_t launch_finalize_small(const Program& P, const GlobalTable& G, OutValue* out_keys, OutValue* out_aggs, OutPartial* out_parts,
                                  uint64_t* out_rep, unsigned long long* counters, unsigned long long* host_counters, uint64_t max_out,
                                  uint32_t* err_flags, bool clear, hipStream_t st);
+hipError_t launch_fold_rows(const Program& P, const FastArgs& F, const GlobalTable& G, uint32_t nslabs, OutValue* out_keys, OutValue* out_aggs,
+                            OutPartial* out_parts, uint64_t* out_rep, unsigned long long* counters, uint32_t ticket_word,
+                            unsigned long long* host_counters, uint64_t max_out, hipStream_t st);
 hipError_t launch_filter_stream(const Program& P, uint64_t nrows, uint64_t row_base, uint64_t* out_rows, unsigned long long* tile_state,
                                 unsigned long long* tile_counter, unsigned long long* total, uint32_t* err_flags, uint32_t grid,
                                 hipStream_t st, bool fast = false);
diff --git a/query_amd/csrc/n1k_kernels.hip b/query_amd/csrc/n1k_kernels.hip
--- a/query_amd/csrc/n1k_kernels.hip
+++ b/query_amd/csrc/n1k_kernels.hip
@@ -1,6 +1,7 @@
 #include <hip/hip_runtime.h>
 #include "n1k_device.h"
 #include "n1k_tables.h"
+#include "n1k_fold.h"
 #include "n1k_scatter.h"
 #include "n1k_kernels.h"
 #include <algorithm>
@@ -1311,30 +1312,50 @@
     if (unpackable) atomicOr(A.err_flags, (uint32_t)ERR_UNPACKABLE_KEY);
 }
 
-enum { RED_ADD_U64, RED_ADD_F64, RED_OR, RED_MIN_I64, RED_MAX_I64, RED_MIN_U64, RED_MAX_U64 };
-
-template <int OP>
-N1K_DEV uint64_t reduce_over_y(uint64_t (*red)[64], uint64_t v) {
+N1K_DEV uint64_t reduce_over_y(uint64_t (*red)[64], uint64_t v, uint32_t op) {
     const uint32_t tx = threadIdx.x, ty = threadIdx.y;
     red[ty][tx] = v;
     __syncthreads();
     for (uint32_t off = 8; off > 0; off >>= 1) {
-        if (ty < off) {
-            uint64_t a = red[ty][tx], b = red[ty + off][tx], r;
-            if (OP == RED_ADD_U64) r = a + b;
-            else if (OP == RED_ADD_F64) r = f64_bits(as_f64(a) + as_f64(b));
-            else if (OP == RED_OR) r = a | b;
-            else if (OP == RED_MIN_I64) r = (int64_t)a < (int64_t)b ? a : b;
-            else if (OP == RED_MAX_I64) r = (int64_t)a > (int64_t)b ? a : b;
-            else if (OP == RED_MIN_U64) r = a < b ? a : b;
-            else r = a > b ? a : b;
-            red[ty][tx] = r;
-        }
+        if (ty < off) red[ty][tx] = fold_word(op, red[ty][tx], red[ty + off][tx]);
         __syncthreads();
     }
     uint64_t out = red[0][tx];
     __syncthreads();
     return out;
+}
+
+N1K_DEV void atomic_fold_word(uint32_t op, unsigned long long* w, uint64_t v) {
+    switch (op) {
+        case FOLD_ADD_U64: atomicAdd(w, (unsigned long long)v); break;
+        case FOLD_ADD_F64: atomicAdd((double*)w, as_f64(v)); break;
+        case FOLD_OR: atomicOr(w, (unsigned long long)v); break;
+        case FOLD_MIN_I64: atomicMin((long long*)w, (long long)v); break;
+        case FOLD_MAX_I64: atomicMax((long long*)w, (long long)v); break;
+        case FOLD_MIN_U64: atomicMin(w, (unsigned long long)v); break;
+        default: atomicMax(w, (unsigned long long)v); break;
+    }
+}
+
+template <uint32_t KIND, int UNROLL>
+N1K_DEV void merge_slabs_agg(uint64_t (*red)[64], const uint64_t* l, uint32_t S, size_t slab_words, uint32_t nblocks, unsigned long long* w) {
+    uint64_t acc[kFoldMaxWords];
+    fold_init(KIND, acc);
+#pragma unroll UNROLL
+    for (uint32_t b = 0; b < nblocks; b++) {
+        const uint64_t* lb = l + b * slab_words;
+        uint64_t x[kFoldMaxWords];
+#pragma unroll
+        for (uint32_t i = 0; i < fold_slab_words(KIND); i++) x[i] = lb[i * (size_t)S];
+        fold_slab(KIND, acc, x);
+    }
+#pragma unroll
+    for (uint32_t i = 0; i < fold_acc_words(KIND); i++) acc[i] = reduce_over_y(red, acc[i], fold_word_op(KIND, i));
+    if (!w) return;
+    const uint64_t fl = acc[fold_flags_word(KIND)];
+#pragma unroll
+    for (uint32_t i = 0; i < fold_acc_words(KIND); i++)
+        if (fold_word_live(KIND, i, fl)) atomic_fold_word(fold_word_op(KIND, i), &w[i], acc[i]);
 }
 
 __global__ __launch_bounds__(1024) void merge_slabs_kernel(const Program P, const FastArgs F, const GlobalTable G,
@@ -1356,7 +1377,7 @@
     uint64_t touched = 0;
 #pragma unroll 8
     for (uint32_t b = 0; b < nblocks; b++) touched |= base[b * slab_words] ^ kEmptyKey;
-    touched = reduce_over_y<RED_OR>(red, touched);
+    touched = reduce_over_y(red, touched, FOLD_OR);
     const bool leader = threadIdx.y == 0 && in_range && touched != 0;
     long long g = -1;
     if (leader) g = global_find_or_insert(G, fast_slot_key(F, s), F.err_flags, ngroups);
@@ -1368,74 +1389,11 @@
         unsigned long long* w = grow ? (unsigned long long*)(grow + ag.glob_off) : nullptr;
         switch (ag.kind) {
             case AGG_COUNT:
-            case AGG_COUNTN: {
-                unsigned long long c = 0;
-#pragma unroll 8
-                for (uint32_t b = 0; b < nblocks; b++) c += l[b * slab_words];
-                c = reduce_over_y<RED_ADD_U64>(red, c);
-                if (w && c) atomicAdd(&w[0], c);
-                break;
-            }
-            case AGG_SUM:
-            case AGG_AVG: {
-                unsigned long long lo = 0, hi = 0, fl = 0, n = 0;
-                double fs = 0.0;
-                const bool avg = ag.kind == AGG_AVG;
-#pragma unroll 4
-                for (uint32_t b = 0; b < nblocks; b++) {
-                    const uint64_t* lb = l + b * slab_words;
-                    int64_t x = (int64_t)lb[0];
-                    double f = as_f64(lb[(size_t)S]);
-                    fl |= lb[2 * (size_t)S];
-                    lo += (unsigned long long)(uint32_t)x;
-                    hi += (unsigned long long)(x >> 32);
-                    fs += f;
-                    if (avg) n += lb[3 * (size_t)S];
-                }
-                lo = reduce_over_y<RED_ADD_U64>(red, lo);
-                hi = reduce_over_y<RED_ADD_U64>(red, hi);
-                fs = as_f64(reduce_over_y<RED_ADD_F64>(red, f64_bits(fs)));
-                fl = reduce_over_y<RED_OR>(red, fl);
-                if (avg) n = reduce_over_y<RED_ADD_U64>(red, n);
-                if (!w || !fl) break;
-                if (fl & (SF_NONNEG_INT | SF_NEG_INT)) { atomicAdd(&w[0], lo); atomicAdd(&w[1], hi); }
-                if (fl & SF_FLOAT) atomicAdd((double*)&w[2], fs);
-                atomicOr(&w[3], fl);
-                if (avg) atomicAdd(&w[4], n);
-                break;
-            }
-            default: {
-                const bool mn = ag.kind == AGG_MIN;
-                unsigned long long fl = 0;
-                long long iv = mn ? INT64_MAX : INT64_MIN;
-                unsigned long long fv = mn ? ~0ull : 0ull, sv = mn ? ~0ull : 0ull;
-#pragma unroll 4
-                for (uint32_t b = 0; b < nblocks; b++) {
-                    const uint64_t* lb = l + b * slab_words;
-                    fl |= lb[0];
-                    long long x = (long long)lb[(size_t)S];
-                    unsigned long long yv = lb[2 * (size_t)S], z = lb[3 * (size_t)S];
-                    iv = mn ? (x < iv ? x : iv) : (x > iv ? x : iv);
-                    fv = mn ? (yv < fv ? yv : fv) : (yv > fv ? yv : fv);
-                    sv = mn ? (z < sv ? z : sv) : (z > sv ? z : sv);
-                }
-                fl = reduce_over_y<RED_OR>(red, fl);
-                if (mn) {
-                    iv = (long long)reduce_over_y<RED_MIN_I64>(red, (uint64_t)iv);
-                    fv = reduce_over_y<RED_MIN_U64>(red, fv);
-                    sv = reduce_over_y<RED_MIN_U64>(red, sv);
-                } else {
-                    iv = (long long)reduce_over_y<RED_MAX_I64>(red, (uint64_t)iv);
-                    fv = reduce_over_y<RED_MAX_U64>(red, fv);
-                    sv = reduce_over_y<RED_MAX_U64>(red, sv);
-                }
-                if (!w || !fl) break;
-                atomicOr(&w[0], fl);
-                if (fl & MM_INT) { if (mn) atomicMin((long long*)&w[1], iv); else atomicMax((long long*)&w[1], iv); }
-                if (fl & MM_FLOAT) { if (mn) atomicMin(&w[2], fv); else atomicMax(&w[2], fv); }
-                if (fl & MM_STRING) { if (mn) atomicMin(&w[3], sv); else atomicMax(&w[3], sv); }
-                break;
-            }
+            case AGG_COUNTN: merge_slabs_agg<AGG_COUNT, 8>(red, l, S, slab_words, nblocks, w); break;
+            case AGG_SUM: merge_slabs_agg<AGG_SUM, 4>(red, l, S, slab_words, nblocks, w); break;
+            case AGG_AVG: merge_slabs_agg<AGG_AVG, 4>(red, l, S, slab_words, nblocks, w); break;
+            case AGG_MIN: merge_slabs_agg<AGG_MIN, 4>(red, l, S, slab_words, nblocks, w); break;
+            default: merge_slabs_agg<AGG_MAX, 4>(red, l, S, slab_words, nblocks, w); break;
         }
     }
 }
@@ -1753,7 +1711,6 @@
     }
 }
 
-constexpr uint32_t kFinalizeSmallMax = 8192;
 __global__ __launch_bounds__(1024) void finalize_small_kernel(const Program P, const GlobalTable G, OutValue* out_keys, OutValue* out_aggs,
                                                              OutPartial* out_parts, uint64_t* out_rep, unsigned long long* counters,
                                                              unsigned long long* host_counters, uint64_t max_out, uint32_t* err_flags,
@@ -1812,6 +1769,173 @@
     if (G.capacity > kFinalizeSmallMax) return hipErrorInvalidValue;
     hipLaunchKernelGGL(finalize_small_kernel, dim3(1), dim3(1024), 0, st, P, G, out_keys, out_aggs, out_parts, out_rep, counters,
                        host_counters, max_out, err_flags, clear ? 1u : 0u);
+    return hipGetLastError();
+}
+
+#ifndef N1K_FOLD_SLOTS
+#define N1K_FOLD_SLOTS 16
+#endif
+#ifndef N1K_FOLD_CHUNK
+#define N1K_FOLD_CHUNK 6
+#endif
+constexpr uint32_t kFoldSlots = N1K_FOLD_SLOTS, kFoldChunk = N1K_FOLD_CHUNK;
+constexpr uint32_t kFoldStage = kFoldMaxWords + 1;
+static_assert(kFoldSlots == 4 || kFoldSlots == 8 || kFoldSlots == 16 || kFoldSlots == 32, "slots of a workgroup share a wave");
+
+template <uint32_t KIND, uint32_t SLOTS, bool KEY>
+N1K_DEV void fold_rows_agg(const uint64_t* key0, const uint64_t* l, uint32_t S, size_t slab_words, uint32_t nslabs, uint32_t bl,
+                           uint64_t* acc, uint64_t& touched) {
+    constexpr uint32_t LANES = 1024 / SLOTS, NW = fold_slab_words(KIND), CH = NW <= 3 || kFoldChunk < 4 ? kFoldChunk : 4;
+    fold_init(KIND, acc);
+    for (uint32_t b0 = 0; b0 < nslabs; b0 += LANES * CH) {
+        uint64_t x[CH][kFoldMaxWords], k[CH];
+#pragma unroll
+        for (uint32_t c = 0; c < CH; c++) {
+            const uint32_t b = b0 + c * LANES + bl;
+            const size_t at = (size_t)(b < nslabs ? b : 0u) * slab_words;
+            k[c] = KEY ? key0[at] : kEmptyKey;
+#pragma unroll
+            for (uint32_t i = 0; i < NW; i++) x[c][i] = l[at + i * (size_t)S];
+        }
+#pragma unroll
+        for (uint32_t c = 0; c < CH; c++) {
+            const bool valid = b0 + c * LANES + bl < nslabs;
+#pragma unroll
+            for (uint32_t i = 0; i < NW; i++) x[c][i] = valid ? x[c][i] : fold_slab_identity(KIND, i);
+            touched |= valid ? (k[c] ^ kEmptyKey) : 0ull;
+            fold_slab(KIND, acc, x[c]);
+        }
+    }
+    for (uint32_t off = SLOTS; off < 64; off <<= 1) {
+        uint64_t other[kFoldMaxWords];
+#pragma unroll
+        for (uint32_t i = 0; i < fold_acc_words(KIND); i++) other[i] = (uint64_t)__shfl_xor((unsigned long long)acc[i], (int)off, 64);
+        fold_join(KIND, acc, other);
+        if (KEY) touched |= (uint64_t)__shfl_xor((unsigned long long)touched, (int)off, 64);
+    }
+}
+
+template <uint32_t SLOTS, bool KEY>
+N1K_DEV void fold_rows_kind(uint32_t kind, const uint64_t* key0, const uint64_t* l, uint32_t S, size_t slab_words, uint32_t nslabs,
+                            uint32_t bl, uint64_t* acc, uint64_t& touched) {
+    switch (kind) {
+        case AGG_COUNT:
+        case AGG_COUNTN: fold_rows_agg<AGG_COUNT, SLOTS, KEY>(key0, l, S, slab_words, nslabs, bl, acc, touched); break;
+        case AGG_SUM: fold_rows_agg<AGG_SUM, SLOTS, KEY>(key0, l, S, slab_words, nslabs, bl, acc, touched); break;
+        case AGG_AVG: fold_rows_agg<AGG_AVG, SLOTS, KEY>(key0, l, S, slab_words, nslabs, bl, acc, touched); break;
+        case AGG_MIN: fold_rows_agg<AGG_MIN, SLOTS, KEY>(key0, l, S, slab_words, nslabs, bl, acc, touched); break;
+        default: fold_rows_agg<AGG_MAX, SLOTS, KEY>(key0, l, S, slab_words, nslabs, bl, acc, touched); break;
+    }
+}
+
+template <uint32_t SLOTS>
+__global__ __launch_bounds__(1024) void fold_rows_kernel(const Program P, const FastArgs F, const GlobalTable G, uint32_t nslabs,
+                                                        OutValue* out_keys, OutValue* out_aggs, OutPartial* out_parts,
+                                                        uint64_t* out_rep, unsigned long long* counters, uint32_t ticket_word,
+                                                        unsigned long long* host_counters, uint64_t max_out) {
+    __shared__ uint64_t stage[16][SLOTS][kFoldStage];
+    __shared__ uint64_t accs[SLOTS][kMaxAggs][kFoldMaxWords];
+    __shared__ uint64_t rows[SLOTS][kMaxAggs * kFoldMaxWords];
+    __shared__ uint64_t touched_s[SLOTS];
+    const uint32_t tid = threadIdx.x, lane = tid & 63, wave = tid >> 6, sx = tid % SLOTS, bl = tid / SLOTS;
+    const uint32_t S = F.lds_slots;
+    const uint32_t s = blockIdx.x * SLOTS + sx;
+    const size_t slab_words = (size_t)P.lds_words * S;
+    const uint64_t* key0 = F.slabs + (s < S ? s : S - 1);
+    unsigned long long in_table = 0, sel = 0;
+    if (wave == 0) {
+        in_table = __hip_atomic_load(&counters[1], __ATOMIC_RELAXED, __HIP_MEMORY_SCOPE_AGENT);
+        const uint32_t per = (nslabs + gridDim.x - 1) / gridDim.x, lo = blockIdx.x * per, hi = lo + per < nslabs ? lo + per : nslabs;
+        for (uint32_t b = lo + lane; b < hi; b += 64) sel += F.block_selected[b];
+    }
+    for (uint32_t a = 0; a < P.naggs; a++) {
+        const AggSpec& ag = P.aggs[a];
+        const uint64_t* l = key0 + (size_t)ag.lds_off * S;
+        uint64_t acc[kFoldMaxWords], touched = 0;
+        const bool first = a == 0;
+        if (first) fold_rows_kind<SLOTS, true>(ag.kind, key0, l, S, slab_words, nslabs, bl, acc, touched);
+        else fold_rows_kind<SLOTS, false>(ag.kind, key0, l, S, slab_words, nslabs, bl, acc, touched);
+        const uint32_t na = fold_acc_words(ag.kind);
+        if (lane < SLOTS) {
+#pragma unroll
+            for (uint32_t i = 0; i < kFoldMaxWords; i++)
+                if (i < na) stage[wave][sx][i] = acc[i];
+            if (first) stage[wave][sx][kFoldMaxWords] = touched;
+        }
+        __syncthreads();
+        if (tid < SLOTS * kFoldStage && (bl < na || (first && bl == kFoldMaxWords))) {
+            const uint32_t op = bl == kFoldMaxWords ? (uint32_t)FOLD_OR : fold_word_op(ag.kind, bl);
+            uint64_t v = stage[0][sx][bl];
+            for (uint32_t w = 1; w < 16; w++) v = fold_word(op, v, stage[w][sx][bl]);
+            if (bl == kFoldMaxWords) touched_s[sx] = v;
+            else accs[sx][a][bl] = v;
+        }
+        __syncthreads();
+    }
+    if (wave != 0) return;
+    for (int off = 32; off > 0; off >>= 1) sel += __shfl_xor(sel, off, 64);
+    if (lane == 0 && sel) atomicAdd(&counters[0], sel);
+    {
+        const bool used = tid < SLOTS && s < S && touched_s[tid % SLOTS] != 0;
+        const unsigned long long m = __ballot(used);
+        unsigned long long first = 0;
+        if (tid == 0 && m) first = atomicAdd(&counters[2], (unsigned long long)__popcll(m));
+        first = __shfl(first, 0, 64);
+        const unsigned long long idx = first + (uint32_t)__popcll(m & ((1ull << lane) - 1ull));
+        if (used && idx < max_out) {
+            uint64_t* g = rows[tid % SLOTS];
+            const uint64_t key = fast_slot_key(F, s);
+            if (in_table) {
+                const uint64_t mask = G.capacity - 1;
+                uint64_t at = mix64(key) & mask;
+                for (uint64_t probe = 0; probe < G.capacity; probe++, at = (at + 1) & mask) {
+                    const uint64_t cur = G.keys[at];
+                    if (cur == kEmptyKey) break;
+                    if (cur != key) continue;
+                    for (uint32_t a = 0; a < P.naggs; a++)
+                        fold_join(P.aggs[a].kind, accs[tid % SLOTS][a], &G.acc[at * P.glob_words + P.aggs[a].glob_off]);
+                    break;
+                }
+            }
+            for (uint32_t a = 0; a < P.naggs; a++) fold_row(P.aggs[a].kind, accs[tid % SLOTS][a], g + P.aggs[a].glob_off);
+            for (uint32_t k = 0; k < P.nkeys; k++) {
+                const KeySpec& ks = P.keys[k];
+                uint64_t field = ks.bits >= 64 ? key : ((key >> ks.shift) & ((1ull << ks.bits) - 1ull));
+                uint32_t tag;
+                uint64_t p;
+                unpack_key_field(P, ks.mode, field, tag, p);
+                put_value(&out_keys[idx * P.nkeys + k], tag, p);
+            }
+            for (uint32_t a = 0; a < P.naggs; a++)
+                finalize_agg(P, P.aggs[a], g, &out_aggs[idx * P.naggs + a], &out_parts[idx * P.naggs + a], F.err_flags);
+            if (out_rep) out_rep[idx] = P.emit_packed_key ? key : ~0ull;
+        }
+    }
+    uint32_t last = 0;
+    __threadfence();
+    if (lane == 0) last = atomicAdd(&counters[ticket_word], 1ull) == (unsigned long long)gridDim.x - 1ull ? 1u : 0u;
+    if (!__shfl(last, 0, 64)) return;
+    __threadfence();
+    unsigned long long v = __hip_atomic_load(&counters[lane % kCounters], __ATOMIC_RELAXED, __HIP_MEMORY_SCOPE_AGENT);
+    const unsigned long long nrows_out = __shfl(v, 2, 64);
+    in_table = __shfl(v, 1, 64);
+    if (lane == 1 || lane == 2) v = nrows_out;
+    if (lane == ticket_word) v = in_table;
+    if (lane < kCounters) {
+        host_counters[lane] = v;
+        counters[lane] = 0;
+    }
+}
+
+hipError_t launch_fold_rows(const Program& P, const FastArgs& F, const GlobalTable& G, uint32_t nslabs, OutValue* out_keys,
+                            OutValue* out_aggs, OutPartial* out_parts, uint64_t* out_rep, unsigned long long* counters,
+                            uint32_t ticket_word, unsigned long long* host_counters, uint64_t max_out, hipStream_t st) {
+    if (!G.capacity || (G.capacity & (G.capacity - 1)) || !F.slabs || !F.block_selected || !nslabs || !F.lds_slots || F.hashed) return hipErrorInvalidValue;
+    if (ticket_word < 3 || ticket_word >= kCounters || P.naggs == 0) return hipErrorInvalidValue;
+    for (uint32_t a = 0; a < P.naggs; a++)
+        if (P.aggs[a].distinct || P.aggs[a].kind > AGG_MAX) return hipErrorInvalidValue;
+    hipLaunchKernelGGL(fold_rows_kernel<kFoldSlots>, dim3((F.lds_slots + kFoldSlots - 1) / kFoldSlots), dim3(1024), 0, st, P, F, G,
+                       nslabs, out_keys, out_aggs, out_parts, out_rep, counters, ticket_word, host_counters, max_out);
     return hipGetLastError();
 }
 
diff --git a/query_amd/csrc/n1k_scan.cpp b/query_amd/csrc/n1k_scan.cpp
--- a/query_amd/csrc/n1k_scan.cpp
+++ b/query_amd/csrc/n1k_scan.cpp
@@ -252,7 +252,7 @@
     return c;
 }
 
-static n1k_status launch_chunk(n1k_handle* h, const ScanChoice& c, const Program& P, FastArgs& F, const WordLogArgs& L, uint64_t off, uint64_t n) {
+static n1k_status launch_chunk(n1k_handle* h, const ScanChoice& c, const Program& P, FastArgs& F, const WordLogArgs& L, uint64_t off, uint64_t n, bool only_chunk) {
     unsigned long long* ngroups = h->groups.counters.p + CTR_GROUPS;
     auto launch = [&](uint32_t g, bool wide) {
         if (c.kernel.spec) return c.kernel.spec->launch(P, F, h->groups.table, ngroups, g, c.fblock, wide, L, h->stream);
@@ -277,7 +277,11 @@
         F.block_selected = h->groups.block_sel.p;
     }
     HIP_TRY(h, launch(g, wide));
-    if (F.slabs) HIP_TRY(h, launch_merge_slabs(P, F, h->groups.table, g, ngroups, h->stream, h->opt.merge_chunks));
+    if (F.slabs && &P == &h->prog && slabs_to_rows(h, F, g, only_chunk, n_main == n)) {
+        h->groups.pending.grid = g;
+        h->groups.pending.F = F;
+    } else if (F.slabs)
+        HIP_TRY(h, launch_merge_slabs(P, F, h->groups.table, g, ngroups, h->stream, h->opt.merge_chunks));
     F.slabs = nullptr;
     if (n_main < n) {
         advance_cols(F.cols, F.ncols, n_main);
@@ -310,7 +314,7 @@
     if (e0) (void)hipEventRecord(e0, h->stream);
     const uint64_t chunk = 1ull << 31;
     for (uint64_t off = 0; off < nrows; off += chunk) {
-        n1k_status st = launch_chunk(h, c, P, F, L, off, std::min<uint64_t>(chunk, nrows - off));
+        n1k_status st = launch_chunk(h, c, P, F, L, off, std::min<uint64_t>(chunk, nrows - off), nrows <= chunk);
         if (st != N1K_OK) return st;
     }
     if (e1) (void)hipEventRecord(e1, h->stream);
@@ -500,6 +504,7 @@
 
 n1k_status push_device(n1k_handle* h, const n1k_batch* b) {
     if (h->stop_flag.load()) return fail(h, N1K_STOPPED, "operator was stopped");
+    h->groups.pending.clean_at_push = h->device_clean && h->row_base == 0 && h->groups.merged_bound == 0 && !h->groups.pending.grid;
     h->device_clean = false;
     n1k_status st = ensure_device(h);
     if (st != N1K_OK) return st;
@@ -546,6 +551,7 @@
         groups_est = std::min<uint64_t>(b->nrows, h->part.sticky.groups_est * b->nrows / std::max<uint64_t>(h->part.sticky.rows, 1) + 1024);
     }
     if (decide) {
+        h->groups.pending.clean_at_push = false;
         st = ensure_table(h, head);
         if (st != N1K_OK) return st;
         unsigned long long before = 0, after = 0;
```

New measurement: 341.5 billion rows/s (median of 6 runs). 1.05x the previous value.
